# lxa9867/ControlVAR

Hardware: AMD Instinct MI355X
Metric: images/sec (256^2 autoregressive_infer_cfg, d24) (higher is better)
Workload: dtype bf16; 1 GPU; ControlVAR d24 autoregressive_infer_cfg 256^2 (control+image), CFG=4.0, top_k=900, top_p=0.96, incl. 2 VQVAE decodes; synthetic weights/labels; batch_per_gpu=512, global_batch=512, seq_len=1360, parallelism=dp1 (sample-sharded, no collective)

## Files before the change

### controlvar_amd/_lib.py

```python
from __future__ import annotations

import ctypes as C
import os
import threading

HERE = os.path.dirname(os.path.abspath(__file__))
LIB_PATH = os.environ.get('CVAR_LIB') or os.path.join(HERE, 'libcvar_hip.so')
ABI_VERSION = 21

CVAR_F32, CVAR_BF16 = 0, 1
ACT_NONE, ACT_GELU_TANH, ACT_GELU_GRAD = 0, 1, 2

c_p = C.c_void_p
c_i = C.c_int
c_l = C.c_int64
c_f = C.c_float


class GemmDesc(C.Structure):
    _fields_ = [
        ('M', c_i), ('N', c_i), ('K', c_i), ('dtype', c_i),
        ('A', c_p), ('lda', c_l), ('W', c_p), ('ldw', c_l),
        ('batch', c_i),
        ('strideA', c_l), ('strideW', c_l), ('strideC', c_l), ('strideR', c_l),
        ('conv', c_i), ('Hin', c_i), ('Win', c_i), ('Cin', c_i), ('Hout', c_i), ('Wout', c_i), ('stride', c_i), ('up', c_i),
        ('alpha', c_f), ('bias', c_p), ('act', c_i),
        ('gate', c_p), ('ldg', c_l), ('gate_rows', c_i),
        ('residual', c_p), ('res_dtype', c_i), ('ldr', c_l),
        ('C', c_p), ('out_dtype', c_i), ('ldc', c_l),
        ('remap_l', c_i), ('remap_L', c_i), ('remap_off', c_i),
        ('pre_act', c_p), ('aux', c_p), ('gate_scale', c_p),
        ('ws', c_p), ('ws_bytes', c_l), ('tile_cfg', c_i), ('stagger', c_i), ('group_m', c_i),
        ('C_split', c_p), ('split_n', c_i), ('ld_split', c_l), ('split_alpha', c_f),
        ('ln_out', c_p), ('ln_out_dtype', c_i), ('ln_scale', c_p), ('ln_shift', c_p), ('ld_ln', c_l), ('ln_rows', c_i), ('ln_eps', c_f),
        ('gn_part', c_p),
    ]


SIGNATURES = {
    'cvar_abi_version': (c_i, []),
    'cvar_status_str': (C.c_char_p, [c_i]),
    'cvar_gemm': (c_i, [C.POINTER(GemmDesc), c_p]),
    'cvar_resample_u8': (c_i, [c_p, c_i, c_i, c_i, c_i, c_i, c_p, c_p, c_i, c_p, c_p]),
    'cvar_crop_flip_normalize': (c_i, [c_p, c_i, c_i, c_i, c_i, c_i, c_i, c_i, c_i, c_p, c_p]),
    'cvar_sumsq_multi': (c_i, [c_p, c_i, c_p, c_p]),
    'cvar_adamw_multi': (c_i, [c_p, c_i, C.POINTER(c_f), C.POINTER(c_f), c_i, c_f, c_f, c_f, c_i, c_p, c_f, c_p]),
    'cvar_rle_paint': (c_i, [c_p, c_p, c_p, c_i, c_i, c_i, c_p, c_p]),
    'cvar_ignore_mask': (c_i, [c_p, c_i, c_i, c_i, C.POINTER(c_i), c_i, c_i, c_i, c_p, c_i, c_p]),
    'cvar_ln_modulate': (c_i, [c_p, c_p, c_p, c_l, c_i, c_p, c_i, c_i, c_i, c_f, c_p]),
    'cvar_silu_cast': (c_i, [c_p, c_p, c_i, c_l, c_p]),
    'cvar_attention': (c_i, [c_p, c_p, c_i, c_i, c_i, c_i, c_i, c_i, c_f, C.POINTER(c_i), c_i, C.POINTER(c_i), c_p, c_p, c_p]),
    'cvar_attention_rowwise': (c_i, [c_p, c_p, c_i, c_i, c_i, c_i, c_i, c_i, c_f, C.POINTER(c_i), c_i, C.POINTER(c_i), c_p, c_p, c_p]),
    'cvar_attention_v1': (c_i, [c_p, c_p, c_i, c_i, c_i, c_i, c_i, c_i, c_f, C.POINTER(c_i), c_i, C.POINTER(c_i), c_p, c_p, c_p]),
    'cvar_attention_prescaled': (c_i, [c_p, c_p, c_i, c_i, c_i, c_i, c_i, c_i, C.POINTER(c_i), c_i, C.POINTER(c_i), c_p, c_p, c_p]),
    'cvar_attention_bwd': (c_i, [c_p, c_i, c_p, c_p, c_p, c_i, c_i, c_i, c_i, c_i, c_f, C.POINTER(c_i), c_i, C.POINTER(c_i), c_p, c_p, c_p]),
    'cvar_attention_bwd_rowwise': (c_i, [c_p, c_i, c_p, c_p, c_p, c_i, c_i, c_i, c_i, c_i, c_f, C.POINTER(c_i), c_i, C.POINTER(c_i), c_p, c_p, c_p]),
    'cvar_cos_qk_norm': (c_i, [c_p, c_p, c_i, c_i, c_i, c_i, c_i, c_i, c_p, c_p, c_f, c_p]),
    'cvar_cos_qk_norm_bwd': (c_i, [c_p, c_p, c_i, c_i, c_i, c_i, c_i, c_p, c_p, c_p, c_p]),
    'cvar_cfg_sample': (c_i, [c_p, c_i, c_i, c_i, c_i, C.POINTER(c_f), c_i, c_f, C.c_uint64, c_p, c_i, c_i, c_p, c_p, c_p, c_p, c_i, c_p, c_i, c_f, c_f, c_p, c_p, c_p]),
    'cvar_ms_next_input': (c_i, [c_p, c_p, c_p, c_p, c_p, c_p, c_p, c_p, c_i, c_i, c_i, c_i, c_i, c_i, c_p]),
    'cvar_ms_encode': (c_i, [c_p, c_p, c_i, c_p, c_p, C.POINTER(c_i), C.POINTER(c_i), c_i, c_p, c_p, c_p, c_p, c_p, c_i, c_i, c_i, c_p]),
    'cvar_word_embed': (c_i, [c_p, c_p, c_p, c_p, c_p, c_i, c_i, c_i, c_i, c_i, c_i, c_i, c_p]),
    'cvar_first_tokens': (c_i, [c_p, c_p, c_p, c_p, c_p, c_p, c_p, c_p, c_i, c_i, c_i, c_i, c_p]),
    'cvar_groupnorm_ws_bytes': (c_l, [c_i, c_i, c_i]),
    'cvar_groupnorm_silu': (c_i, [c_p, c_i, c_p, c_p, c_p, c_i, c_i, c_i, c_i, c_f, c_i, c_p, c_p]),
    'cvar_groupnorm_silu_partials': (c_i, [c_p, c_i, c_p, c_p, c_p, c_i, c_i, c_i, c_i, c_f, c_i, c_p, c_i, c_i, c_p, c_p]),
    'cvar_split3': (c_i, [c_p, c_l, c_p, c_l, c_i, c_i, c_p]),
    'cvar_groupnorm_silu_split3': (c_i, [c_p, c_p, c_p, c_p, c_i, c_i, c_i, c_i, c_f, c_i, c_p, c_p]),
    'cvar_conv3x3_gn_partials': (c_i, [c_i, c_i, c_i, c_i, c_i, c_i, c_i, c_i, C.POINTER(c_i), C.POINTER(c_i)]),
    'cvar_softmax_rows': (c_i, [c_p, c_p, c_i, c_i, c_i, c_p]),
    'cvar_gemm_tn': (c_i, [c_p, c_l, c_p, c_l, c_p, c_l, c_i, c_i, c_i, c_p, c_l, c_p, c_p]),
    'cvar_embed_rows': (c_i, [c_p, c_p, c_i, c_p, c_l, c_i, c_p]),
    'cvar_resample_sep': (c_i, [c_p, c_p, c_p, c_p, c_i, c_i, c_i, c_i, c_i, c_i, c_p]),
    'cvar_transpose': (c_i, [c_p, c_p, c_i, c_i, c_i, c_i, c_l, c_l, c_p]),
    'cvar_nchw_to_nhwc': (c_i, [c_p, c_p, c_i, c_i, c_i, c_i, c_i, c_p]),
    'cvar_nhwc_to_nchw': (c_i, [c_p, c_i, c_l, c_p, c_i, c_i, c_i, c_f, c_f, c_f, c_f, c_p]),
    'cvar_gate_residual': (c_i, [c_p, c_p, c_i, c_p, c_l, c_i, c_p, c_l, c_i, c_p]),
    'cvar_train_ws_floats': (c_l, [c_l, c_i, c_i]),
    'cvar_gated_grad': (c_i, [c_p, c_p, c_i, c_p, c_l, c_p, c_p, c_p, c_l, c_i, c_i, c_i, c_p, c_l, c_p]),
    'cvar_gelu': (c_i, [c_p, c_p, c_i, c_l, c_p]),
    'cvar_gelu_bwd': (c_i, [c_p, c_p, c_i, c_l, c_p]),
    'cvar_ln_modulate_bwd': (c_i, [c_p, c_p, c_i, c_p, c_l, c_i, c_p, c_p, c_p, c_p, c_l, c_i, c_i, c_f, c_p, c_l, c_p]),
    'cvar_colsum': (c_i, [c_p, c_i, c_l, c_p, c_l, c_i, c_i, c_p, c_p]),
    'cvar_wordembed_grad_ws_bytes': (c_l, [c_l, c_i]),
    'cvar_wordembed_grad': (c_i, [c_p, c_l, c_i, c_i, c_p, c_i, c_i, c_i, c_i, c_p, c_p, c_p, c_p]),
    'cvar_rowsum': (c_i, [c_p, c_i, c_l, c_p, c_i, c_i, c_i, c_p]),
    'cvar_ce_fwd_bwd': (c_i, [c_p, c_p, c_p, c_f, c_p, c_p, c_i, c_l, c_i, c_p]),
    'cvar_scatter_add_rows': (c_i, [c_p, c_l, c_p, c_p, c_i, c_i, c_p]),
    'cvar_silu_bwd': (c_i, [c_p, c_p, c_p, c_l, c_p]),
    'cvar_adamw': (c_i, [c_p, c_p, c_p, c_p, c_l, c_f, c_f, c_f, c_f, c_f, c_i, c_p, c_f, c_p]),
    'cvar_sumsq': (c_i, [c_p, c_l, c_p, c_p]),
    'cvar_clip_coef': (c_i, [c_p, c_l, c_f, c_f, c_p, c_p]),
    'cvar_lora_down': (c_i, [c_p, c_l, c_p, c_l, c_p, c_l, c_p, c_l, c_i, c_i, c_i, c_i, c_f, c_f, C.c_uint64, C.c_uint32, c_p]),
    'cvar_lora_dx': (c_i, [c_p, c_l, c_i, c_p, c_l, c_p, c_l, c_p, c_l, c_i, c_i, c_i, c_i, c_f, c_f, C.c_uint64, C.c_uint32, c_p]),
    'cvar_lora_wgrad_ws_floats': (c_l, [c_i, c_i]),
    'cvar_lora_wgrad': (c_i, [c_p, c_l, c_p, c_l, c_i, c_i, c_i, c_i, c_f, c_f, C.c_uint64, C.c_uint32, c_p, c_l, c_p, c_l, c_l, c_p]),
    'cvar_lora_dropout_mask': (c_i, [c_p, c_i, c_i, c_f, C.c_uint64, C.c_uint32, c_p]),
    'cvar_probe_mfma_bf16': (c_i, [c_p, c_l, c_i, c_p, c_p]),
    'cvar_probe_mfma_bf16_32x32': (c_i, [c_p, c_l, c_i, c_p, c_p]),
    'cvar_probe_mfma_flops': (C.c_double, [c_i]),
}

_lib = None
_lock = threading.Lock()


class CvarError(RuntimeError):
    pass


def load(path: str = LIB_PATH) -> C.CDLL:
    global _lib
    with _lock:
        if _lib is not None:
            return _lib
        if not os.path.exists(path):
            raise CvarError(f'{path} not found - build it with `python -m controlvar_amd.build` (hipcc, gfx950); '
                            'there is no fallback path')
        try:
            import torch
        except Exception:
            pass
        lib = C.CDLL(path, mode=C.RTLD_GLOBAL)
        for name, (res, args) in SIGNATURES.items():
            fn = getattr(lib, name)
            fn.restype = res
            fn.argtypes = args
        v = lib.cvar_abi_version()
        if v != ABI_VERSION:
            raise CvarError(f'libcvar_hip.so ABI {v} != expected {ABI_VERSION}; rebuild')
        _lib = lib
        return lib


def check(status: int, what: str):
    if status != 0:
        msg = load().cvar_status_str(status).decode()
        raise CvarError(f'{what}: {msg} ({status})')
```

### controlvar_amd/csrc/conv_halo.hip

```cpp
#include "cvar_common.h"

typedef __attribute__((address_space(3))) void* lptr_t;

#ifndef CH_EPI_LDS
#define CH_EPI_LDS 1
#endif

struct ConvHaloParams {
    const bf16_t* X; const bf16_t* Wt; const float* bias; const bf16_t* res; void* out;
    int B, H, W, Cin, Cout, tiles_x, tiles_y, nchunk;
    int up, Hin, Win;
    float* gn_part;
};


template <int CH_NB, typename TO, int TW = 16>
__global__ __launch_bounds__(TW * 16, 2) void conv3x3_halo_bf16_kernel(const ConvHaloParams p) {
    constexpr int NW = TW / 4;
    constexpr int CH_HROW = TW + 4;
    constexpr int CH_HALO_PIECES = (18 * CH_HROW * 64 + 1023) / 1024;
    constexpr int CH_HALO_BYTES = CH_HALO_PIECES * 1024;
    constexpr int H_PER_WAVE = (CH_HALO_PIECES + NW - 1) / NW;
    constexpr int CH_W_BYTES = CH_NB * 2048;
    constexpr int W_PIECES = CH_NB * 2;
    constexpr int W_PER_WAVE = (W_PIECES + NW - 1) / NW;
    __shared__ __attribute__((aligned(1024))) char smem[2 * CH_HALO_BYTES + 3 * CH_W_BYTES];
    const int tid = threadIdx.x, lane = tid & 63;
    const int wave = __builtin_amdgcn_readfirstlane(tid >> 6);
    const int lrow = lane & 31, hi = lane >> 5;
    int t_ = blockIdx.x;
    const int tx = t_ % p.tiles_x; t_ /= p.tiles_x;
    const int ty = t_ % p.tiles_y;
    const int b = t_ / p.tiles_y;
    const int ty0 = ty * 16, tx0 = tx * TW;
    const int cout0 = blockIdx.y * (32 * CH_NB);
    const bf16_t* ximg = p.X + (long)b * p.Hin * p.Win * p.Cin;
    const __amdgpu_buffer_rsrc_t x_rsrc = __builtin_amdgcn_make_buffer_rsrc((void*)ximg, 0, p.Hin * p.Win * p.Cin * 2, 0x00020000);
    const __amdgpu_buffer_rsrc_t w_rsrc = __builtin_amdgcn_make_buffer_rsrc((void*)(p.Wt + (long)cout0 * 9 * p.Cin), 0, min(32 * CH_NB, p.Cout - cout0) * 9 * p.Cin * 2, 0x00020000);

    unsigned h_off[H_PER_WAVE], w_off[W_PER_WAVE];
#pragma unroll
    for (int jj = 0; jj < H_PER_WAVE; ++jj) {
        const int q = (wave + NW * jj) * 64 + lane;
        const int hp = q >> 2;
        const int hy = hp / CH_HROW, hx = hp - hy * CH_HROW;
        const int lc = (q & 3) ^ ((hx >> 2) & 3);
        const int gy = ty0 - 1 + hy, gx = tx0 - 1 + hx;
        const bool ok = hy < 18 && hx < TW + 2 && gy >= 0 && gy < p.H && gx >= 0 && gx < p.W;
        const int sy = p.up ? gy >> 1 : gy, sx = p.up ? gx >> 1 : gx;
        h_off[jj] = ok ? (unsigned)(((sy * p.Win + sx) * p.Cin + lc * 8) * 2) : 0x80000000u;
    }
#pragma unroll
    for (int jj = 0; jj < W_PER_WAVE; ++jj) {
        const int q = (wave + NW * jj) * 64 + lane;
        const int n = q >> 2, lc = (q & 3) ^ ((n >> 2) & 3);
        w_off[jj] = (n < 32 * CH_NB && cout0 + n < p.Cout) ? (unsigned)((n * 9 * p.Cin + lc * 8) * 2) : 0x80000000u;
    }
    auto issue_halo = [&](int c, int jj) -> int {
        const int j = wave + NW * jj;
        if (j >= CH_HALO_PIECES) return 0;
        __builtin_amdgcn_raw_ptr_buffer_load_lds(x_rsrc, (lptr_t)(smem + (c & 1) * CH_HALO_BYTES + j * 1024), 16, (int)h_off[jj], c * 64, 0, 0);
        return 1;
    };
    auto issue_w = [&](int c, int t) -> int {
        int n = 0;
#pragma unroll
        for (int jj = 0; jj < W_PER_WAVE; ++jj) {
            const int j = wave + NW * jj;
            if (j < W_PIECES) {
                __builtin_amdgcn_raw_ptr_buffer_load_lds(w_rsrc, (lptr_t)(smem + 2 * CH_HALO_BYTES + (t % 3) * CH_W_BYTES + j * 1024), 16,
                                                         (int)w_off[jj], (t * p.Cin + c * 32) * 2, 0, 0);
                ++n;
            }
        }
        return n;
    };
    auto wait_vm = [&](int n) {
        if (n >= 4) asm volatile("s_waitcnt vmcnt(4)" ::: "memory");
        else if (n == 3) asm volatile("s_waitcnt vmcnt(3)" ::: "memory");
        else if (n == 2) asm volatile("s_waitcnt vmcnt(2)" ::: "memory");
        else if (n == 1) asm volatile("s_waitcnt vmcnt(1)" ::: "memory");
        else asm volatile("s_waitcnt vmcnt(0)" ::: "memory");
    };

    constexpr int RPI = 32 / TW;
    const int px = lrow & (TW - 1), py0 = 2 * RPI * wave + lrow / TW;
    const int hpb = py0 * CH_HROW + px;
    const int swb = (lrow >> 2) & 3;
    const int b_lane = lrow * 64;

    f32x16_t acc[2][CH_NB];
#pragma unroll
    for (int i = 0; i < 2; ++i)
#pragma unroll
        for (int j = 0; j < CH_NB; ++j)
#pragma unroll
            for (int r = 0; r < 16; ++r) acc[i][j][r] = 0.f;

#pragma unroll
    for (int jj = 0; jj < H_PER_WAVE; ++jj) issue_halo(0, jj);
    issue_w(0, 0);
    issue_w(0, 1);
    asm volatile("s_waitcnt vmcnt(0)" ::: "memory");
    __builtin_amdgcn_s_barrier();

    bf16x8_t af[2][2][2];
    auto read_a = [&](int set, const char* hbuf, int d) {
        const int sw = ((px + d % CH_HROW) >> 2) & 3;
#pragma unroll
        for (int i = 0; i < 2; ++i) {
            const int hp = hpb + RPI * CH_HROW * i + d;
            const char* ap = hbuf + hp * 64;
#pragma unroll
            for (int ks = 0; ks < 2; ++ks) af[set][i][ks] = *(const bf16x8_t*)(ap + (((2 * ks + hi) ^ sw) << 4));
        }
    };
    read_a(0, smem, 0);
    for (int c = 0; c < p.nchunk; ++c) {
        const char* hb = smem + (c & 1) * CH_HALO_BYTES;
        const char* hb_next = smem + ((c + 1) & 1) * CH_HALO_BYTES;
#pragma unroll
        for (int t = 0; t < 9; ++t) {
            int issued = 0;
            if (t < H_PER_WAVE && c + 1 < p.nchunk) issued += issue_halo(c + 1, t);
            {
                const int c2 = t + 2 >= 9 ? c + 1 : c, t2 = t + 2 >= 9 ? t + 2 - 9 : t + 2;
                if (c2 < p.nchunk) issued += issue_w(c2, t2);
            }
            const char* wb = smem + 2 * CH_HALO_BYTES + (t % 3) * CH_W_BYTES + b_lane;
            bf16x8_t w[2][CH_NB];
#pragma unroll
            for (int ks = 0; ks < 2; ++ks)
#pragma unroll
                for (int j = 0; j < CH_NB; ++j) w[ks][j] = *(const bf16x8_t*)(wb + j * 2048 + (((2 * ks + hi) ^ swb) << 4));
            if (t < 8) read_a((t + 1) & 1, hb, ((t + 1) / 3) * CH_HROW + ((t + 1) % 3));
            else read_a(1, hb_next, 0);
#pragma unroll
            for (int ks = 0; ks < 2; ++ks)
#pragma unroll
                for (int j = 0; j < CH_NB; ++j)
#pragma unroll
                    for (int i = 0; i < 2; ++i) acc[i][j] = __builtin_amdgcn_mfma_f32_32x32x16_bf16(w[ks][j], af[t & 1][i][ks], acc[i][j], 0, 0, 0);
            wait_vm(issued);
            __builtin_amdgcn_s_barrier();
        }
#pragma unroll
        for (int i = 0; i < 2; ++i)
#pragma unroll
            for (int ks = 0; ks < 2; ++ks) af[0][i][ks] = af[1][i][ks];
    }

    float gs[8], gq[8], gpiv[8];
#pragma unroll
    for (int i = 0; i < 2; ++i) {
        const int yy = py0 + RPI * i, xx = px;
        const long gpix = ((long)b * p.H + ty0 + yy) * p.W + tx0 + xx;
        if constexpr (CH_NB == 1) {
            TO* op = (TO*)p.out + gpix * p.Cout + cout0;
#pragma unroll
            for (int g = 0; g < 4; ++g)
#pragma unroll
                for (int e = 0; e < 4; ++e) {
                    const int co = 8 * g + 4 * hi + e;
                    if (cout0 + co < p.Cout) {
                        const float v = acc[i][0][4 * g + e] + (p.bias ? p.bias[cout0 + co] : 0.f);
                        if constexpr (sizeof(TO) == 4) op[co] = v;
                        else op[co] = f32_to_bf16(v);
                    }
                }
        } else if constexpr (CH_NB == 5 && sizeof(TO) == 4) {
            float* op = (float*)p.out + gpix * p.Cout + cout0 + 4 * hi;
            const float* rp = p.res ? (const float*)p.res + gpix * p.Cout + cout0 + 4 * hi : nullptr;
            const float* bp = p.bias ? p.bias + cout0 + 4 * hi : nullptr;
#pragma unroll
            for (int j = 0; j < CH_NB; ++j) {
                f32x4_t rq[4];
                if (rp) {
#pragma unroll
                    for (int g = 0; g < 4; ++g) rq[g] = *(const f32x4_t*)(rp + 32 * j + 8 * g);
                }
#pragma unroll
                for (int g = 0; g < 4; ++g) {
                    const int co = 32 * j + 8 * g;
                    f32x4_t bq = {0.f, 0.f, 0.f, 0.f};
                    if (bp) bq = *(const f32x4_t*)(bp + co);
                    f32x4_t v;
#pragma unroll
                    for (int e = 0; e < 4; ++e) v[e] = acc[i][j][4 * g + e] + bq[e];
                    if (rp) {
#pragma unroll
                        for (int e = 0; e < 4; ++e) v[e] += rq[g][e];
                    }
                    *(f32x4_t*)(op + co) = v;
                }
            }
        } else if constexpr (CH_EPI_LDS != 0 && CH_NB == 5) {
            constexpr int PS = 336;
            constexpr int SLICE = (2 * CH_HALO_BYTES + 3 * CH_W_BYTES) / NW / 64 * 64;
            static_assert(32 * PS + 512 + 3 * 20 * 64 <= SLICE, "GroupNorm partials need the slack behind the staged rows");
            char* stg = smem + wave * SLICE;
            const float* bp = p.bias ? p.bias + cout0 + 4 * hi : nullptr;
            const long img = (long)b * p.H * p.W * p.Cout;
            auto chunk = [&](int k, int& go, int& lo) {
                const int q = k * 64 + lane, pq = q / 20, part = q - pq * 20;
                go = ((ty0 + 2 * RPI * wave + RPI * i + pq / TW) * p.W + tx0 + (pq & (TW - 1))) * p.Cout + cout0 + part * 8;
                lo = pq * PS + part * 16;
            };
            if (p.res) {
                const bf16_t* rimg = p.res + img;
#pragma unroll
                for (int h = 0; h < 2; ++h) {
                    bf16x8_t rr[5];
                    int lo[5];
#pragma unroll
                    for (int k = 0; k < 5; ++k) { int go; chunk(5 * h + k, go, lo[k]); rr[k] = *(const bf16x8_t*)(rimg + go); }
#pragma unroll
                    for (int k = 0; k < 5; ++k) *(bf16x8_t*)(stg + lo[k]) = rr[k];
                }
            }
            char* mine = stg + lrow * PS + 8 * hi;
#pragma unroll
            for (int j = 0; j < CH_NB; ++j)
#pragma unroll
                for (int g = 0; g < 4; ++g) {
                    const int co = 32 * j + 8 * g;
                    f32x4_t bq = {0.f, 0.f, 0.f, 0.f};
                    if (bp) bq = *(const f32x4_t*)(bp + co);
                    float v[4];
#pragma unroll
                    for (int e = 0; e < 4; ++e) v[e] = acc[i][j][4 * g + e] + bq[e];
                    if (p.res) {
                        const bf16x4_t rq = *(const bf16x4_t*)(mine + co * 2);
#pragma unroll
                        for (int e = 0; e < 4; ++e) v[e] += bf16_to_f32((bf16_t)rq[e]);
                    }
                    *(bf16x4_t*)(mine + co * 2) = pack_bf16x4(v);
                }
#pragma unroll
            for (int k = 0; k < 10; ++k) { int go, lo; chunk(k, go, lo); *(bf16x8_t*)((bf16_t*)p.out + img + go) = *(const bf16x8_t*)(stg + lo); }
            if (p.gn_part) {
                char* pv = smem + 32 * PS;
                if (i == 0) {
                    __builtin_amdgcn_wave_barrier();
                    if (wave == 0 && lane < 20) *(bf16x8_t*)(pv + lane * 16) = *(const bf16x8_t*)(stg + lane * 16);
                    __syncthreads();
                    if (lane < 60) {
                        const bf16x8_t pq8 = *(const bf16x8_t*)(pv + (lane % 20) * 16);
#pragma unroll
                        for (int e = 0; e < 8; ++e) { gpiv[e] = bf16_to_f32((bf16_t)pq8[e]); gs[e] = 0.f; gq[e] = 0.f; }
                    }
                }
                if (lane < 60) {
                    const int cc = lane % 20, pg = lane / 20;
#pragma unroll
                    for (int it = 0; it < 11; ++it) {
                        const int pp = pg + 3 * it;
                        if (pp < 32) {
                            const bf16x8_t y8 = *(const bf16x8_t*)(stg + pp * PS + cc * 16);
#pragma unroll
                            for (int e = 0; e < 8; ++e) { const float f = bf16_to_f32((bf16_t)y8[e]) - gpiv[e]; gs[e] += f; gq[e] = __builtin_fmaf(f, f, gq[e]); }
                        }
                    }
                }
                __builtin_amdgcn_wave_barrier();
            }
        } else {
            bf16_t* op = (bf16_t*)p.out + gpix * p.Cout + cout0 + 4 * hi;
            const bf16_t* rp = p.res ? p.res + gpix * p.Cout + cout0 + 4 * hi : nullptr;
            const float* bp = p.bias ? p.bias + cout0 + 4 * hi : nullptr;
            bf16x4_t rq[CH_NB][4];
            if (rp) {
#pragma unroll
                for (int j = 0; j < CH_NB; ++j)
#pragma unroll
                    for (int g = 0; g < 4; ++g) rq[j][g] = *(const bf16x4_t*)(rp + 32 * j + 8 * g);
            }
#pragma unroll
            for (int j = 0; j < CH_NB; ++j)
#pragma unroll
                for (int g = 0; g < 4; ++g) {
                    const int co = 32 * j + 8 * g;
                    f32x4_t bq = {0.f, 0.f, 0.f, 0.f};
                    if (bp) bq = *(const f32x4_t*)(bp + co);
                    float v[4];
#pragma unroll
                    for (int e = 0; e < 4; ++e) v[e] = acc[i][j][4 * g + e] + bq[e];
                    if (rp) {
#pragma unroll
                        for (int e = 0; e < 4; ++e) v[e] += bf16_to_f32((bf16_t)rq[j][g][e]);
                    }
                    *(bf16x4_t*)(op + co) = pack_bf16x4(v);
                }
        }
    }
    if constexpr (CH_NB == 5 && CH_EPI_LDS != 0 && sizeof(TO) == 2) {
        if (p.gn_part) {
            constexpr int PS = 336, SLICE = (2 * CH_HALO_BYTES + 3 * CH_W_BYTES) / NW / 64 * 64, RED = 32 * PS + 512;
            if (lane < 60) {
                float* rd = (float*)(smem + wave * SLICE + RED) + lane * 16;
#pragma unroll
                for (int e = 0; e < 8; e += 4) {
                    *(f32x4_t*)(rd + e) = f32x4_t{gs[e], gs[e + 1], gs[e + 2], gs[e + 3]};
                    *(f32x4_t*)(rd + 8 + e) = f32x4_t{gq[e], gq[e + 1], gq[e + 2], gq[e + 3]};
                }
            }
            __syncthreads();
            if (tid < 160) {
                const int cc = tid >> 3, e = tid & 7;
                float S = 0.f, Q = 0.f;
#pragma unroll
                for (int w = 0; w < NW; ++w)
#pragma unroll
                    for (int pg = 0; pg < 3; ++pg) {
                        const float* rd = (const float*)(smem + w * SLICE + RED) + (pg * 20 + cc) * 16;
                        S += rd[e]; Q += rd[8 + e];
                    }
                const float piv = bf16_to_f32(*(const bf16_t*)(smem + 32 * PS + tid * 2));
                float* gp = p.gn_part + ((((long)b * p.tiles_y + ty) * p.tiles_x + tx) * p.Cout + cout0 + tid) * 3;
                gp[0] = S; gp[1] = Q; gp[2] = piv;
            }
        }
    }
}

int cvar_conv3x3_halo_bf16(const void* X, const void* Wt, const float* bias, const void* residual, void* out, int out_f32, int B, int H, int W, int Cin,
                           int Cout, int up, float* gn_part, hipStream_t st) {
    ConvHaloParams p;
    p.X = (const bf16_t*)X; p.Wt = (const bf16_t*)Wt; p.bias = bias; p.res = (const bf16_t*)residual; p.out = out;
    p.B = B; p.H = H; p.W = W; p.Cin = Cin; p.Cout = Cout; p.tiles_x = W / 16; p.tiles_y = H / 16; p.nchunk = Cin / 32;
    p.up = up ? 1 : 0; p.Hin = up ? H / 2 : H; p.Win = up ? W / 2 : W;
    p.gn_part = gn_part;
    if (gn_part && !(Cout % 160 == 0 && !out_f32)) return CVAR_EUNSUPPORTED;
    const long tiles = (long)B * p.tiles_x * p.tiles_y;
    if (tiles <= 0 || tiles > 0x7fffffffL) return CVAR_EINVAL;
    if (Cout % 160 == 0 && out_f32) {
        if ((((uintptr_t)out | (uintptr_t)residual) & 15) != 0 || (long)H * W * Cout >= 0x7fffffffL) return CVAR_EUNSUPPORTED;
        hipLaunchKernelGGL((conv3x3_halo_bf16_kernel<5, float>), dim3((unsigned)tiles, Cout / 160), dim3(256), 0, st, p);
    } else if (Cout % 160 == 0 && !out_f32) {
        if ((((uintptr_t)out | (uintptr_t)residual) & 15) != 0 || (long)H * W * Cout >= 0x7fffffffL) return CVAR_EUNSUPPORTED;
        hipLaunchKernelGGL((conv3x3_halo_bf16_kernel<5, bf16_t>), dim3((unsigned)tiles, Cout / 160), dim3(256), 0, st, p);
    } else if (Cout <= 32 && !residual) {
        if (out_f32) hipLaunchKernelGGL((conv3x3_halo_bf16_kernel<1, float>), dim3((unsigned)tiles, 1), dim3(256), 0, st, p);
        else hipLaunchKernelGGL((conv3x3_halo_bf16_kernel<1, bf16_t>), dim3((unsigned)tiles, 1), dim3(256), 0, st, p);
    } else {
        return CVAR_EUNSUPPORTED;
    }
    CVAR_CHECK_LAUNCH();
    return CVAR_OK;
}
```

### controlvar_amd/csrc/cvar_common.h

```cpp
#pragma once
#include <hip/hip_runtime.h>
#include <stdint.h>
#include "../../include/cvar.h"

typedef __attribute__((ext_vector_type(8))) short bf16x8_t;
typedef __attribute__((ext_vector_type(4))) short bf16x4_t;
typedef __attribute__((ext_vector_type(4))) float f32x4_t;
typedef __attribute__((ext_vector_type(16))) float f32x16_t;
typedef unsigned short bf16_t;

#define CVAR_CHECK_LAUNCH()                                      \
    do {                                                         \
        hipError_t e__ = hipGetLastError();                      \
        if (e__ != hipSuccess) return CVAR_ELAUNCH;              \
    } while (0)

__device__ __forceinline__ float bf16_to_f32(bf16_t b) { return __uint_as_float(((unsigned)b) << 16); }

typedef __attribute__((ext_vector_type(2))) float f32x2_t;
typedef __attribute__((ext_vector_type(2))) __bf16 bf16x2n_t;
typedef __attribute__((ext_vector_type(4))) unsigned u32x4_t;
__device__ __forceinline__ bf16_t f32_to_bf16(float f) {
    const __bf16 b = (__bf16)f;
    return __builtin_bit_cast(unsigned short, b);
}
__device__ __forceinline__ unsigned pack_bf16x2(float lo, float hi) {
    const f32x2_t v = {lo, hi};
    const bf16x2n_t r = __builtin_convertvector(v, bf16x2n_t);
    return __builtin_bit_cast(unsigned, r);
}
__device__ __forceinline__ bf16x8_t pack_bf16x8(const float* v) {
    const u32x4_t u = {pack_bf16x2(v[0], v[1]), pack_bf16x2(v[2], v[3]), pack_bf16x2(v[4], v[5]), pack_bf16x2(v[6], v[7])};
    return __builtin_bit_cast(bf16x8_t, u);
}
__device__ __forceinline__ bf16x4_t pack_bf16x4(const float* v) {
    typedef __attribute__((ext_vector_type(2))) unsigned u32x2_t;
    const u32x2_t u = {pack_bf16x2(v[0], v[1]), pack_bf16x2(v[2], v[3])};
    return __builtin_bit_cast(bf16x4_t, u);
}

template <typename T> struct Elem;
template <> struct Elem<float> {
    static constexpr int kDtype = CVAR_F32;
    __device__ static __forceinline__ float ld(const float* p) { return *p; }
    __device__ static __forceinline__ void st(float* p, float v) { *p = v; }
};
template <> struct Elem<bf16_t> {
    static constexpr int kDtype = CVAR_BF16;
    __device__ static __forceinline__ float ld(const bf16_t* p) { return bf16_to_f32(*p); }
    __device__ static __forceinline__ void st(bf16_t* p, float v) { *p = f32_to_bf16(v); }
};

__device__ __forceinline__ float ld_any(const void* p, int dtype, int64_t i) {
    return dtype == CVAR_BF16 ? bf16_to_f32(((const bf16_t*)p)[i]) : ((const float*)p)[i];
}
__device__ __forceinline__ void st_any(void* p, int dtype, int64_t i, float v) {
    if (dtype == CVAR_BF16) ((bf16_t*)p)[i] = f32_to_bf16(v);
    else ((float*)p)[i] = v;
}

__device__ __forceinline__ float wave_sum(float v) {
#pragma unroll
    for (int o = 32; o > 0; o >>= 1) v += __shfl_xor(v, o, 64);
    return v;
}
__device__ __forceinline__ float wave_max(float v) {
#pragma unroll
    for (int o = 32; o > 0; o >>= 1) v = fmaxf(v, __shfl_xor(v, o, 64));
    return v;
}

__device__ __forceinline__ float gelu_tanh_f(float t) {
    const float k2 = 2.0f * 0.7978845608028654f;
    const float u2 = k2 * (t + 0.044715f * t * t * t);
    return t / (1.0f + __expf(-u2));
}

__device__ __forceinline__ float gelu_tanh_fast(float t) {
    const float c1 = -2.0f * 0.7978845608028654f * 1.4426950408889634f, c3 = c1 * 0.044715f;
    const float t2 = t * t;
    const float arg = t * (c1 + c3 * t2);
    return t * __builtin_amdgcn_rcpf(1.0f + __builtin_amdgcn_exp2f(arg));
}

__device__ __forceinline__ float gelu_tanh_grad(float t) {
    const float k2 = 2.0f * 0.7978845608028654f;
    const float u2 = k2 * (t + 0.044715f * t * t * t);
    const float sg = 1.0f / (1.0f + __expf(-u2));
    return sg + t * sg * (1.0f - sg) * k2 * (1.0f + 0.134145f * t * t);
}

static inline hipStream_t as_stream(void* s) { return (hipStream_t)s; }
static inline int cdiv(int64_t a, int64_t b) { return (int)((a + b - 1) / b); }

int cvar_conv3x3_halo_bf16(const void* X, const void* Wt, const float* bias, const void* residual, void* out, int out_f32, int B, int H, int W, int Cin,
                           int Cout, int up, float* gn_part, hipStream_t st);
int cvar_conv3x3_c8_bf16(const void* X, const void* Wt, const float* bias, void* out, int B, int H, int W, int Cout, float* gn_part, hipStream_t st);
```

### controlvar_amd/csrc/gemm.hip

```cpp
#include "cvar_common.h"
#include "gemm_params.h"
#if defined(CVAR_GEMM_CONV_TU)
#define CVAR_TU_CONV 1
#define CVAR_TU_PLAIN 0
#elif defined(CVAR_GEMM_F32_TU)
#define CVAR_TU_CONV 1
#define CVAR_TU_PLAIN 1
#else
#define CVAR_TU_CONV 0
#define CVAR_TU_PLAIN 1
#endif
#include <type_traits>

static __device__ __attribute__((aligned(16))) unsigned int cvar_zero_chunk[4] = {0u, 0u, 0u, 0u};
#if defined(CVAR_GEMM_TIMING) && defined(CVAR_GEMM_F32_TU)
#undef CVAR_GEMM_TIMING
#endif
#ifdef CVAR_GEMM_TIMING
__device__ unsigned long long cvar_gemm_dbg[64 * 8 * 8];
__device__ unsigned long long cvar_gemm_dbg_tot[8];
#define CVAR_DBG_WG_MAX 16384
__device__ unsigned long long cvar_gemm_dbg_wg[CVAR_DBG_WG_MAX * 5];
extern "C" int cvar_gemm_dbg_wg_read(unsigned long long* host, int n) { return (int)hipMemcpyFromSymbol(host, HIP_SYMBOL(cvar_gemm_dbg_wg), sizeof(unsigned long long) * 5 * (size_t)(n < CVAR_DBG_WG_MAX ? n : CVAR_DBG_WG_MAX)); }
extern "C" int cvar_gemm_dbg_tot_read(unsigned long long* host, int reset) { int rc = (int)hipMemcpyFromSymbol(host, HIP_SYMBOL(cvar_gemm_dbg_tot), 64); if (reset) { unsigned long long z[8] = {0}; rc |= (int)hipMemcpyToSymbol(HIP_SYMBOL(cvar_gemm_dbg_tot), z, 64); } return rc; }
// ... 788 lines not shown
            if (!lane_on || rr >= 16 || m >= p.M) continue;
            float v[8];
            {
                const float* sg = stg;
                const f32x4_t a0 = *(const f32x4_t*)(sg + (rr + srow_half * half) * EROW + ecol);
                const f32x4_t a1 = *(const f32x4_t*)(sg + (rr + srow_half * half) * EROW + ecol + 4);
#pragma unroll
                for (int e = 0; e < 4; ++e) { v[e] = a0[e] * p.alpha; v[4 + e] = a1[e] * p.alpha; }
            }
            long orow = m;
            if (p.remap_l > 0) {
                const int sq = fast_div(m, p.remap_magic, p.remap_shift);
                orow = (long)sq * p.remap_L + p.remap_off + (m - sq * p.remap_l);
            }
            const float* grow = p.gate ? p.gate + (long)fast_div(m, p.gate_magic, p.gate_shift) * p.ldg : nullptr;
            void* Cdst = Cb;
            long cbase = cz + orow * p.ldc + n;
            bool scale_split = false;
            if (p.split_n > 0) {
                if (n < p.split_n) { Cdst = p.Cs; cbase = (long)m * p.ld_split + n; scale_split = p.split_alpha != 1.0f; }
                else cbase -= p.split_n;
            }
            if (vec_ok) {
#pragma unroll
                for (int e = 0; e < 8; ++e) v[e] += bias8[e];
                if (p.C2) {
#pragma unroll
                    for (int e = 0; e < 8; ++e) st_any(p.C2, ES == 2 ? CVAR_BF16 : CVAR_F32, cz + (long)m * p.ldc + n + e, v[e]);
                }
                if (scale_split) {
#pragma unroll
                    for (int e = 0; e < 8; ++e) v[e] *= p.split_alpha;
                }
                if (p.act == CVAR_ACT_GELU_TANH) {
#pragma unroll
                    for (int e = 0; e < 8; ++e) v[e] = (ES == 2) ? gelu_tanh_fast(v[e]) : gelu_tanh_f(v[e]);
                } else if (p.act == CVAR_ACT_GELU_GRAD) {
#pragma unroll
                    for (int e = 0; e < 8; ++e) v[e] *= gelu_tanh_grad(ld_any(p.aux, p.out_dtype, cz + (long)m * p.ldc + n + e));
                }
                if (grow) {
                    const f32x4_t g0 = *(const f32x4_t*)(grow + n), g1 = *(const f32x4_t*)(grow + n + 4);
                    const float gs = p.gate_scale ? p.gate_scale[fast_div(m, p.gate_magic, p.gate_shift)] : 1.0f;
#pragma unroll
                    for (int e = 0; e < 4; ++e) { v[e] *= g0[e] * gs; v[4 + e] *= g1[e] * gs; }
                }
                if (p.residual) {
                    if (p.res_dtype == CVAR_BF16) {
                        const bf16x8_t rv = *(const bf16x8_t*)((const bf16_t*)p.residual + rz + (long)m * p.ldr + n);
#pragma unroll
                        for (int e = 0; e < 8; ++e) v[e] += bf16_to_f32((bf16_t)rv[e]);
                    } else {
                        const float* rp = (const float*)p.residual + rz + (long)m * p.ldr + n;
                        const f32x4_t r0 = *(const f32x4_t*)rp, r1 = *(const f32x4_t*)(rp + 4);
#pragma unroll
                        for (int e = 0; e < 4; ++e) { v[e] += r0[e]; v[4 + e] += r1[e]; }
                    }
                }
                if (p.out_dtype == CVAR_BF16) {
                    *(bf16x8_t*)((bf16_t*)Cdst + cbase) = pack_bf16x8(v);
                } else {
                    float* cp = (float*)Cdst + cbase;
                    const f32x4_t o0 = {v[0], v[1], v[2], v[3]}, o1 = {v[4], v[5], v[6], v[7]};
                    *(f32x4_t*)cp = o0; *(f32x4_t*)(cp + 4) = o1;
                }
            } else {
                for (int e = 0; e < 8; ++e) {
                    if (n + e >= p.N) break;
                    float x = v[e];
                    if (p.bias) x += p.bias[n + e];
                    if (p.C2) st_any(p.C2, ES == 2 ? CVAR_BF16 : CVAR_F32, cz + (long)m * p.ldc + n + e, x);
                    if (p.act == CVAR_ACT_GELU_TANH) x = gelu_tanh_f(x);
                    else if (p.act == CVAR_ACT_GELU_GRAD) x *= gelu_tanh_grad(ld_any(p.aux, p.out_dtype, cz + (long)m * p.ldc + n + e));
                    if (grow) x *= grow[n + e] * (p.gate_scale ? p.gate_scale[fast_div(m, p.gate_magic, p.gate_shift)] : 1.0f);
                    if (p.residual) x += ld_any(p.residual, p.res_dtype, rz + (long)m * p.ldr + n + e);
                    st_any(Cdst, p.out_dtype, cbase + e, x);
                }
            }
        }
    }
    }
#ifdef CVAR_GEMM_TIMING
    if (lane == 0 && wave == 0 && (int)blockIdx.x < CVAR_DBG_WG_MAX && blockIdx.y == 0 && blockIdx.z == 0) {
        asm volatile("s_waitcnt vmcnt(0)" ::: "memory");
        unsigned hwid, xcc;
        asm volatile("s_getreg_b32 %0, hwreg(HW_REG_HW_ID)" : "=s"(hwid));
        asm volatile("s_getreg_b32 %0, hwreg(HW_REG_XCC_ID)" : "=s"(xcc));
        unsigned long long* o = cvar_gemm_dbg_wg + (size_t)blockIdx.x * 5;
        o[0] = dbg_rt_entry; o[1] = dbg_rt_loop; o[2] = dbg_rt_loop_end; o[3] = __builtin_amdgcn_s_memrealtime(); o[4] = (unsigned long long)hwid | ((unsigned long long)xcc << 32);
    }
    if (lane == 0 && blockIdx.x < 64) {
        const unsigned long long dbg_t2 = __builtin_amdgcn_s_memtime();
        unsigned long long* o = cvar_gemm_dbg + (blockIdx.x * 8 + wave) * 8;
        o[0] = dbg_comp; o[1] = dbg_vm; o[2] = dbg_bar; o[3] = dbg_t1 - dbg_t0; o[4] = dbg_t2 - dbg_t1; o[5] = nk - kt_lo; o[6] = dbg_t0; o[7] = dbg_t2;
    }
    if (lane == 0 && wave == 0) {
        const unsigned long long dbg_t2 = __builtin_amdgcn_s_memtime();
        atomicAdd(&cvar_gemm_dbg_tot[0], dbg_t1 - dbg_t0); atomicAdd(&cvar_gemm_dbg_tot[1], dbg_t2 - dbg_t1); atomicAdd(&cvar_gemm_dbg_tot[2], 1ULL);
        atomicAdd(&cvar_gemm_dbg_tot[6], dbg_ew); atomicAdd(&cvar_gemm_dbg_tot[3], dbg_vm); atomicAdd(&cvar_gemm_dbg_tot[4], dbg_bar); atomicAdd(&cvar_gemm_dbg_tot[5], dbg_comp);
    }
#endif
}

template <typename T, int BM, int BN, int WM, int WN, bool CONV, int NSTAGE = 2, bool FAST = false, bool CUP = false>
__global__ __launch_bounds__(WM * WN * 64) void cvar_gemm_kernel(const GemmParams p) {
    cvar_gemm_tile<T, BM, BN, WM, WN, CONV, NSTAGE, FAST, CUP>(p, (int)blockIdx.x);
}

__device__ __forceinline__ void splitk_finish_quad(const GemmParams& p, const float* __restrict__ part, int nsplit, int m, int n) {
    f32x4_t v;
    const float* const q0 = part + (long)m * p.N + n;
    const long sstride = (long)p.M * p.N;
    {
        v = *(const f32x4_t*)q0;
        for (int s0 = 1; s0 < nsplit; s0 += 8) {
            f32x4_t w[8];
#pragma unroll
            for (int u = 0; u < 8; ++u)
                if (s0 + u < nsplit) w[u] = *(const f32x4_t*)(q0 + (long)(s0 + u) * sstride);
#pragma unroll
            for (int u = 0; u < 8; ++u)
                if (s0 + u < nsplit) {
#pragma unroll
                    for (int e = 0; e < 4; ++e) v[e] += w[u][e];
                }
        }
    }
    gemm_epilogue_quad(p, m, n, v);
}

template <typename K>
static void set_max_lds_once(K kfn, size_t lds, unsigned char* done) {
    int dev = 0;
    (void)hipGetDevice(&dev);
    if (dev < 0 || dev >= 64 || !done[dev]) {
        (void)hipFuncSetAttribute((const void*)kfn, hipFuncAttributeMaxDynamicSharedMemorySize, (int)lds);
        if (dev >= 0 && dev < 64) done[dev] = 1;
    }
}

template <typename T, int BM, int BN, int WM, int WN, int NSTAGE = 2, bool CONVFAST = false, bool CUP = false>
static int launch_cfg(const GemmParams& gp, int batch, hipStream_t st) {
    GemmParams p = gp;
    p.tiles_m = (p.M + BM - 1) / BM;
    p.tiles_n = (p.N + BN - 1) / BN;
    if (p.group_m <= 0) p.group_m = (!p.conv && ((long)p.K * (long)sizeof(T) >= 8192 || p.out_dtype == CVAR_F32)) ? 4 : 8;
    if (p.conv) { const int kt_e = 128 / (int)sizeof(T); p.cv_adv = kt_e / p.Cin; p.cv_rem = kt_e % p.Cin; }
    const size_t lds = NSTAGE * (BM + BN) * 128 + ((sizeof(T) == 2 && BM == 256 && BN == 256 && WM == 2 && WN == 4 && NSTAGE == 2 && !CONVFAST) ? 32768 : 0);
    const int nk_all = (p.K + (128 / (int)sizeof(T)) - 1) / (128 / (int)sizeof(T));
    const int splits = p.split_tiles > 0 ? (nk_all + p.split_tiles - 1) / p.split_tiles : 1;
    const bool plain_fast = !p.conv && p.K % (128 / (int)sizeof(T)) == 0 && (long)(BM - 1) * p.lda * (long)sizeof(T) + (long)p.K * (long)sizeof(T) < (1L << 31) &&
                            (long)(BN - 1) * p.ldw * (long)sizeof(T) + (long)p.K * (long)sizeof(T) < (1L << 31);
    dim3 grid((unsigned)(p.tiles_m * p.tiles_n), (unsigned)splits, (unsigned)batch), block(WM * WN * 64);
    constexpr bool WITH_CONV = CVAR_TU_CONV || sizeof(T) == 4, WITH_PLAIN = CVAR_TU_PLAIN || sizeof(T) == 4;
    if constexpr (CONVFAST) {
        if (!p.conv) return CVAR_EINVAL;
        if constexpr (WITH_CONV) {
            auto kfn = cvar_gemm_kernel<T, BM, BN, WM, WN, true, NSTAGE, true, CUP>;
            static unsigned char lds_set[64] = {0};
            set_max_lds_once(kfn, lds, lds_set);
            hipLaunchKernelGGL(kfn, grid, block, lds, st, p);
            CVAR_CHECK_LAUNCH();
            return CVAR_OK;
        } else return CVAR_EUNSUPPORTED;
    } else if (p.conv) {
        if constexpr (WITH_CONV) {
            auto kfn = cvar_gemm_kernel<T, BM, BN, WM, WN, true, NSTAGE>;
            static unsigned char lds_set[64] = {0};
            set_max_lds_once(kfn, lds, lds_set);
            hipLaunchKernelGGL(kfn, grid, block, lds, st, p);
        } else return CVAR_EUNSUPPORTED;
    } else if constexpr (!WITH_PLAIN) {
        return CVAR_EUNSUPPORTED;
    } else if (plain_fast) {
        auto kfn = cvar_gemm_kernel<T, BM, BN, WM, WN, false, NSTAGE, true>;
        static unsigned char lds_set[64] = {0};
        set_max_lds_once(kfn, lds, lds_set);
        hipLaunchKernelGGL(kfn, grid, block, lds, st, p);
    } else {
        auto kfn = cvar_gemm_kernel<T, BM, BN, WM, WN, false, NSTAGE>;
        static unsigned char lds_set[64] = {0};
        set_max_lds_once(kfn, lds, lds_set);
        hipLaunchKernelGGL(kfn, grid, block, lds, st, p);
    }
    CVAR_CHECK_LAUNCH();
    return CVAR_OK;
}

static int gemm_cfg_override(const GemmParams& p) {
    return p.tile_cfg == 1 ? 0 : (p.tile_cfg == 2 || p.tile_cfg == 7 || p.tile_cfg == 28) ? 1 : (p.tile_cfg == 3 || p.tile_cfg == 8) ? 3 : p.tile_cfg == 4 ? 4 : -1;
}

template <typename T>
static int launch_typed(const GemmParams& p, int batch, hipStream_t st) {
    if (p.M <= 64) return launch_cfg<T, 64, 128, 1, 4>(p, batch, st);
    auto launch_128 = [&](const GemmParams& q, int nb, hipStream_t s) -> int {
#if CVAR_TU_PLAIN && !CVAR_TU_CONV
        if constexpr (sizeof(T) == 2) {
            if (CVAR_GEMM_128_W8 && !q.conv && q.tile_cfg != 26) return launch_cfg<T, 128, 128, 2, 4>(q, nb, s);
        }
#endif
        return launch_cfg<T, 128, 128, 2, 2>(q, nb, s);
    };
    if constexpr (sizeof(T) == 2) {
        if (p.conv && p.N <= 32 && p.M >= 4096 && p.stride == 1 && !p.up && p.Cin % 32 == 0 && p.split_tiles == 0 && gemm_cfg_override(p) != 0) {
            const long in_bytes = (long)(p.M / (p.Hout * p.Wout)) * p.Hin * p.Win * p.Cin * (long)sizeof(T);
            if (in_bytes < (1L << 31)) {
                GemmParams q = p;
                q.conv_bytes = (unsigned)in_bytes;
                return launch_cfg<T, 256, 32, 4, 1, 2, true>(q, batch, st);
            }
        }
    }
    if (p.N % 160 == 0 && (p.N % 128 != 0 || p.conv) && p.M >= 4096) {
        const long in_bytes = p.conv ? (long)(p.M / (p.Hout * p.Wout)) * p.Hin * p.Win * p.Cin * (long)sizeof(T) : 0;
        if constexpr (sizeof(T) == 2) {
            if (p.conv && (p.stride == 1 || (p.stride == 2 && !p.up)) && p.Cin % 32 == 0 && p.split_tiles == 0 && in_bytes < (1L << 31) &&
                (long)159 * p.ldw * 2 + (long)p.K * 2 + 256 < (1L << 31) && gemm_cfg_override(p) != 0 &&
                (!p.up || (p.Hout == 2 * p.Hin && p.Wout == 2 * p.Win))) {
                GemmParams q = p;
                q.conv_bytes = (unsigned)in_bytes;
                const int ovc = gemm_cfg_override(p);
                if (!p.up && p.stride == 1 && ovc != 3 && (ovc == 4 || (long)p.K * (long)sizeof(T) <= 4096)) return launch_cfg<T, 256, 160, 8, 1, 2, true>(q, batch, st);
                return p.up ? launch_cfg<T, 256, 160, 4, 1, 2, true, true>(q, batch, st) : launch_cfg<T, 256, 160, 4, 1, 2, true>(q, batch, st);
            }
        }
        return launch_cfg<T, 128, 160, 4, 1>(p, batch, st);
    }
#if CVAR_TU_PLAIN && !CVAR_TU_CONV
    if constexpr (sizeof(T) == 2) {
        if (p.tile_cfg == 27 && !p.conv && p.split_tiles == 0) return launch_cfg<T, 256, 192, 4, 2>(p, batch, st);
    }
#endif
    const int ov = gemm_cfg_override(p);
    const bool n_ok = p.N % 256 == 0 || (p.N % 128 == 0 && p.N >= 1536);
    if (sizeof(T) == 2 && (ov == 3 || (ov != 0 && ov != 1 && p.split_tiles > 0)) && (p.M >= 2048 || (p.split_tiles > 0 && p.M > 1024)) && n_ok)
        return launch_cfg<T, 256, 256, 2, 2>(p, batch, st);
    if (ov == -1 && sizeof(T) == 2 && p.split_tiles == 0 && batch == 1 && n_ok && p.M >= 2048) {
        const long t256 = (long)((p.M + 255) / 256) * ((p.N + 255) / 256), t128 = (long)((p.M + 127) / 128) * ((p.N + 127) / 128);
        const double c256 = (double)((t256 + 255) / 256), c128 = CVAR_GEMM_C128 * (double)((t128 + 511) / 512);
#if CVAR_TU_PLAIN && !CVAR_TU_CONV
        if constexpr (sizeof(T) == 2) {
            if (CVAR_GEMM_T192 && !p.conv && p.N % 192 == 0) {
                const long t192 = (long)((p.M + 255) / 256) * (p.N / 192);
                const double c192 = CVAR_GEMM_C192 * (double)((t192 + 255) / 256);
                if (c192 < 0.95 * c256 && c192 < c128) return launch_cfg<T, 256, 192, 4, 2>(p, batch, st);
            }
        }
#endif
        if (c128 < 0.97 * c256) {
#if CVAR_TU_PLAIN && !CVAR_TU_CONV
            if constexpr (sizeof(T) == 2) {
                if (p.tile_cfg == 12 && !p.conv && t128 <= 256 && p.K >= 6 * 64) return launch_cfg<T, 128, 128, 2, 4, 3>(p, batch, st);
            }
#endif
            return launch_128(p, batch, st);
        }
    }
    if (ov != 0 && (p.M >= 2048 || (p.split_tiles > 0 && p.M > 1024)) && n_ok) return launch_cfg<T, 256, 256, 2, 4>(p, batch, st);
#if CVAR_TU_PLAIN && !CVAR_TU_CONV
    if constexpr (sizeof(T) == 2) {
        if (p.tile_cfg == 13 && !p.conv) return launch_cfg<T, 128, 128, 2, 4, 3>(p, batch, st);
        if (p.tile_cfg == 14 && !p.conv) return launch_cfg<T, 128, 128, 2, 2, 4>(p, batch, st);
        if (p.tile_cfg == 12 && !p.conv && batch == 1 && p.split_tiles == 0 && p.K >= 6 * 64 &&
            (long)((p.M + 127) / 128) * ((p.N + 127) / 128) <= 256) return launch_cfg<T, 128, 128, 2, 4, 3>(p, batch, st);
    }
#endif
    return launch_128(p, batch, st);
}

int cvar_gemm_skinny_plan(int M, int N, int K, long lda, long ldw, int want_rowfin, int have_ws, int* mt, int* nt, int* slices);
int cvar_gemm_skinny_launch(const GemmParams& p, int mt, int nt, int slices, hipStream_t st);
int cvar_splitk_rowfin_ok(const GemmParams& p, const cvar_gemm_desc* d);
int cvar_splitk_rowfin_launch(const float* part, int nsplit, const GemmParams& p, const cvar_gemm_desc* d, hipStream_t st);
int cvar_gemm_launch_f32(const GemmParams& p, int batch, hipStream_t st);
int cvar_gemm_launch_conv_bf16(const GemmParams& p, int batch, hipStream_t st);
#if defined(CVAR_GEMM_F32_TU)
int cvar_gemm_launch_f32(const GemmParams& p, int batch, hipStream_t st) { return launch_typed<float>(p, batch, st); }
#elif defined(CVAR_GEMM_CONV_TU)
int cvar_gemm_launch_conv_bf16(const GemmParams& p, int batch, hipStream_t st) { return launch_typed<bf16_t>(p, batch, st); }
#else

__global__ __launch_bounds__(256) void cvar_splitk_epilogue_kernel(const float* __restrict__ part, int nsplit, const GemmParams p) {
    const long nvec = (long)p.M * (p.N / 4);
    for (long i = (long)blockIdx.x * 256 + threadIdx.x; i < nvec; i += (long)gridDim.x * 256)
        splitk_finish_quad(p, part, nsplit, (int)(i / (p.N / 4)), (int)(i % (p.N / 4)) * 4);
}


extern "C" int cvar_conv3x3_gn_partials(int dtype, int stride, int Cin, int Cout, int Hin, int Win, int Hout, int Wout, int* tiles_per_image, int* pixels_per_tile) {
#ifndef CVAR_NO_CONV_C8
    const bool c8 = Cin == 8 && Hin == Hout && Win == Wout;
#else
    const bool c8 = false;
#endif
    const bool ok = dtype == CVAR_BF16 && stride == 1 && Cin > 0 && (Cin % 32 == 0 || c8) && Cout > 0 && Cout % 160 == 0 && Hout > 0 && Wout > 0 && Hout % 16 == 0 && Wout % 16 == 0 &&
                    (long)Hin * Win * Cin * 2 < 0x7fffffffL && (long)Hout * Wout * Cout < 0x7fffffffL;
    if (!ok) return 0;
    if (tiles_per_image) *tiles_per_image = (Hout / 16) * (Wout / 16);
    if (pixels_per_tile) *pixels_per_tile = 256;
    return 1;
}

extern "C" int cvar_gemm(const cvar_gemm_desc* d, void* stream) {
    if (!d || !d->A || !d->W || !d->C) return CVAR_EINVAL;
    if (d->M <= 0 || d->N <= 0 || d->K <= 0 || d->batch < 1) return CVAR_EINVAL;
    if (d->dtype != CVAR_F32 && d->dtype != CVAR_BF16) return CVAR_EUNSUPPORTED;
    const int es = d->dtype == CVAR_BF16 ? 2 : 4, kch = 16 / es;
    if (d->K % kch) return CVAR_EUNSUPPORTED;
    if (((uintptr_t)d->A & 15) || ((uintptr_t)d->W & 15)) return CVAR_EINVAL;
    if ((d->ldw % kch) || (d->strideW % kch) || (d->strideA % kch)) return CVAR_EUNSUPPORTED;
    if (d->conv) {
        if (d->Cin % kch || d->K != 9 * d->Cin) return CVAR_EUNSUPPORTED;
        if (d->stride != 1 && d->stride != 2) return CVAR_EUNSUPPORTED;
        if (d->stride == 2 && d->up) return CVAR_EUNSUPPORTED;
        if (d->stride == 1 && (d->Hout != (d->up ? 2 : 1) * d->Hin || d->Wout != (d->up ? 2 : 1) * d->Win)) return CVAR_EINVAL;
        if (d->stride == 2 && (d->Hout != d->Hin / 2 || d->Wout != d->Win / 2)) return CVAR_EINVAL;
        if (d->M % (d->Hout * d->Wout)) return CVAR_EINVAL;
    } else if (d->lda % kch) {
        return CVAR_EUNSUPPORTED;
    }
    if (d->gn_part && !d->conv) return CVAR_EINVAL;
    if (d->gate && d->gate_rows <= 0) return CVAR_EINVAL;
    if (d->act == CVAR_ACT_GELU_GRAD && !d->aux) return CVAR_EINVAL;
    if (d->pre_act && d->act == CVAR_ACT_GELU_GRAD) return CVAR_EINVAL;
    if (d->gate_scale && !d->gate) return CVAR_EINVAL;
    if ((d->pre_act || d->aux) && d->remap_l > 0) return CVAR_EUNSUPPORTED;
    if (d->split_n < 0 || d->split_n >= d->N) return CVAR_EINVAL;
    if (d->split_n > 0) {
        if (!d->C_split || d->ld_split < d->split_n) return CVAR_EINVAL;
        if (d->remap_l <= 0 || d->conv || d->batch != 1 || d->residual || d->gate || d->act != CVAR_ACT_NONE) return CVAR_EUNSUPPORTED;
        if ((d->split_n & 7) || (d->N & 7) || (d->ld_split & 7) || (d->ldc & 7) || ((uintptr_t)d->C_split & 15) || ((uintptr_t)d->C & 15)) return CVAR_EUNSUPPORTED;
    }
    GemmParams p;
    p.M = d->M; p.N = d->N; p.K = d->K;
    p.A = (const char*)d->A; p.lda = d->lda; p.W = (const char*)d->W; p.ldw = d->ldw;
    p.strideA = d->strideA; p.strideW = d->strideW; p.strideC = d->strideC; p.strideR = d->strideR;
    p.conv = d->conv; p.Hin = d->Hin; p.Win = d->Win; p.Cin = d->Cin; p.Hout = d->Hout; p.Wout = d->Wout;
    p.stride = d->stride; p.up = d->up;
    p.alpha = d->alpha; p.bias = d->bias; p.act = d->act;
    p.gate = d->gate; p.ldg = d->ldg; p.gate_rows = d->gate_rows;
    p.residual = d->residual; p.res_dtype = d->res_dtype; p.ldr = d->ldr;
    p.C = d->C; p.out_dtype = d->out_dtype; p.ldc = d->ldc;
    p.C2 = d->pre_act; p.aux = d->aux; p.gate_scale = d->gate_scale; p.in_dtype = d->dtype;
    p.remap_l = d->remap_l; p.remap_L = d->remap_L; p.remap_off = d->remap_off;
    p.Cs = d->C_split; p.split_n = d->split_n; p.ld_split = d->ld_split; p.split_alpha = d->split_alpha == 0.0f ? 1.0f : d->split_alpha;
    p.tiles_m = p.tiles_n = 0;
    p.cv_adv = p.cv_rem = 0; p.conv_bytes = 0;
    make_fast_div(p.remap_l, &p.remap_magic, &p.remap_shift);
    make_fast_div(p.gate ? p.gate_rows : 1, &p.gate_magic, &p.gate_shift);
    p.split_tiles = 0; p.split_stride = 0;
    p.tile_cfg = d->tile_cfg; p.stagger = d->stagger > 0 ? d->stagger : 0; p.group_m = d->group_m > 0 ? d->group_m : 0;
    p.nt = ((long)d->M * d->N * (d->out_dtype == CVAR_F32 ? 4 : 2) >= (128L << 20)) ? 1 : 0;
    float* const g_splitk_ws = (d->ws && d->ws_bytes > 0 && (((uintptr_t)d->ws & 15) == 0)) ? (float*)d->ws : nullptr;
    const size_t g_splitk_ws_bytes = g_splitk_ws ? (size_t)d->ws_bytes : 0;
    hipStream_t st = as_stream(stream);
    if (d->ln_out) {
        if (!d->ln_scale || !d->ln_shift || d->ln_rows <= 0 || (d->N % 4) || d->N > 2048 || (d->ld_ln % 4) || d->out_dtype != CVAR_F32 || d->ldc != d->N ||
            d->remap_l > 0 || d->split_n > 0 || d->conv || d->batch != 1 || (d->ln_out_dtype != CVAR_BF16 && d->ln_out_dtype != CVAR_F32)) return CVAR_EUNSUPPORTED;
    }
    auto ln_after = [&](int rc) -> int {
        if (rc != CVAR_OK || !d->ln_out) return rc;
        return cvar_ln_modulate((const float*)d->C, d->ln_scale, d->ln_shift, d->ld_ln, d->ln_rows, d->ln_out, d->ln_out_dtype, d->M, d->N, d->ln_eps, stream);
    };
    const bool rowfin = g_splitk_ws && cvar_splitk_rowfin_ok(p, d);
    auto finish_slices = [&](int splits) -> int {
        if (rowfin) return cvar_splitk_rowfin_launch(g_splitk_ws, splits, p, d, st);
        const long nvec = (long)d->M * (d->N / 4);
        hipLaunchKernelGGL(cvar_splitk_epilogue_kernel, dim3((unsigned)min((long)2048, (nvec + 255) / 256)), dim3(256), 0, st, g_splitk_ws, splits, p);
        CVAR_CHECK_LAUNCH();
        return ln_after(CVAR_OK);
    };
    if (!d->conv && d->batch == 1 && d->dtype == CVAR_BF16 && d->tile_cfg == 12 && !d->pre_act && !d->aux) {
        int mt = 0, nt = 0, sl = 0;
        if (cvar_gemm_skinny_plan(d->M, d->N, d->K, d->lda, d->ldw, rowfin ? 1 : 0, g_splitk_ws ? 1 : 0, &mt, &nt, &sl)) {
            if (sl > 1 && (size_t)sl * d->M * d->N * sizeof(float) <= g_splitk_ws_bytes) {
                GemmParams ps = p;
                ps.C = g_splitk_ws; ps.out_dtype = CVAR_F32; ps.ldc = d->N;
                ps.split_tiles = (d->K >> 5) / sl; ps.split_stride = (long)d->M * d->N;
                const int rc = cvar_gemm_skinny_launch(ps, mt, nt, sl, st);
                if (rc != CVAR_OK) return rc;
                return finish_slices(sl);
            }
            if (sl == 1) return ln_after(cvar_gemm_skinny_launch(p, mt, nt, 1, st));
        }
    }
    const int kt_elems = 128 / es;
    const int nk_all = (d->K + kt_elems - 1) / kt_elems;
    const int tm = d->M <= 64 ? (d->M + 63) / 64 : (d->M + 127) / 128, tn = (d->N + 127) / 128;
    int long_k_splits = 0;
    const int t256 = ((d->M + 255) / 256) * ((d->N + 255) / 256);
    if (!d->conv && d->batch == 1 && d->dtype == CVAR_BF16 && d->M > 1024 && d->M % 128 == 0 && d->N % 128 == 0 && d->N >= 1536 && g_splitk_ws &&
        (nk_all >= 128 || (nk_all >= 24 && t256 <= 64 && !d->remap_l))) {
        const int tiles = t256;
        if (tiles < 256) {
            double best = 1e30;
            for (int sp = 1; sp <= 8; ++sp) {
                const double cost = (double)((tiles * sp + 255) / 256) / sp + 0.01 * sp;
                if (nk_all / sp < 6) break;
                if (cost < best && (size_t)sp * d->M * d->N * sizeof(float) <= g_splitk_ws_bytes) { best = cost; long_k_splits = sp; }
            }
            if (long_k_splits < 2) long_k_splits = 0;
        }
    }
    const bool three = d->tile_cfg == 12 && !d->conv && d->batch == 1 && d->dtype == CVAR_BF16 && d->M > 64 && d->M <= 1024 && (d->N % 4) == 0 && tm * tn <= 256 &&
                       nk_all >= 6 && !d->pre_act && !d->aux;
    int three_splits = 1;
    if (three && g_splitk_ws) {
        three_splits = min(16, max(1, 256 / (tm * tn)));
        while (three_splits > 1 && nk_all / three_splits < 4) --three_splits;
    }
    if (three) p.tile_cfg = 13;
    if (long_k_splits || (three && three_splits > 1) ||
        (!three && !d->conv && d->batch == 1 && d->M <= 1024 && (d->N % 4) == 0 && tm * tn < 128 && nk_all >= 8 && g_splitk_ws)) {
        int splits = long_k_splits ? long_k_splits : three ? three_splits : min(16, max(2, 320 / (tm * tn)));
        int per = (nk_all + splits - 1) / splits;
        if (per < 2) per = 2;
        splits = (nk_all + per - 1) / per;
        const size_t need = (size_t)splits * d->M * d->N * sizeof(float);
        if (splits > 1 && need <= g_splitk_ws_bytes) {
            GemmParams ps = p;
            ps.alpha = 1.0f; ps.bias = nullptr; ps.act = CVAR_ACT_NONE; ps.gate = nullptr; ps.residual = nullptr; ps.C2 = nullptr; ps.aux = nullptr; ps.gate_scale = nullptr;
            ps.C = g_splitk_ws; ps.out_dtype = CVAR_F32; ps.ldc = d->N; ps.remap_l = 0; ps.split_n = 0; ps.Cs = nullptr; ps.strideC = 0;
            ps.split_tiles = per; ps.split_stride = (long)d->M * d->N;
            const int rc = d->dtype == CVAR_BF16 ? launch_typed<bf16_t>(ps, 1, st) : cvar_gemm_launch_f32(ps, 1, st);
            if (rc != CVAR_OK) return rc;
            return finish_slices(splits);
        }
    }
#ifndef CVAR_NO_CONV_C8
    if (d->conv && d->dtype == CVAR_BF16 && d->stride == 1 && !d->up && d->batch == 1 && (d->tile_cfg == 0 || d->tile_cfg == 6) && d->Cin == 8 && d->N % 160 == 0 &&
        d->Hout % 16 == 0 && d->Wout % 16 == 0 && d->act == CVAR_ACT_NONE && !d->gate && d->alpha == 1.0f && !d->residual && !d->pre_act && !d->aux && !d->gate_scale &&
        d->remap_l == 0 && d->split_n == 0 && d->strideC == 0 && d->ldc == d->N && d->ldw == d->K && d->out_dtype == CVAR_BF16 &&
        ((((uintptr_t)d->C | (uintptr_t)d->bias) & 15) == 0) && (long)d->Hout * d->Wout * d->N < 0x7fffffffL)
        return cvar_conv3x3_c8_bf16(d->A, d->W, d->bias, d->C, d->M / (d->Hout * d->Wout), d->Hout, d->Wout, d->N, d->gn_part, st);
#endif
    if (d->conv && d->dtype == CVAR_BF16 && d->stride == 1 && d->batch == 1 && (d->tile_cfg == 0 || d->tile_cfg == 6 || d->tile_cfg == 9 || d->tile_cfg == 10) &&
        d->Cin % 32 == 0 && d->Hout % 16 == 0 && d->Wout % 16 == 0 && d->act == CVAR_ACT_NONE && !d->gate && d->alpha == 1.0f &&
        !d->pre_act && !d->aux && !d->gate_scale && d->remap_l == 0 && d->split_n == 0 && d->strideC == 0 && d->ldc == d->N &&
        d->ldw == d->K &&
        (!d->bias || (((uintptr_t)d->bias & 15) == 0)) && (long)d->Hin * d->Win * d->Cin * 2 < 0x7fffffffL) {
        const bool wide = d->N % 160 == 0 && d->out_dtype == CVAR_BF16 && (((uintptr_t)d->C & 15) == 0) &&
                          (!d->residual || (d->res_dtype == CVAR_BF16 && d->ldr == d->N && (((uintptr_t)d->residual & 15) == 0))) &&
                          (long)d->Hout * d->Wout * d->N < 0x7fffffffL;
        const bool narrow = d->N <= 32 && !d->residual && (d->out_dtype == CVAR_BF16 || d->out_dtype == CVAR_F32) && ((long)d->Hout * d->Wout >= 65536 || d->tile_cfg == 6);
        if (d->gn_part && !wide) return CVAR_EUNSUPPORTED;
        const bool wide32 = d->N % 160 == 0 && d->out_dtype == CVAR_F32 && (((uintptr_t)d->C & 15) == 0) && !d->up &&
                            (!d->residual || (d->res_dtype == CVAR_F32 && d->ldr == d->N && (((uintptr_t)d->residual & 15) == 0))) &&
                            (long)d->Hout * d->Wout * d->N < 0x7fffffffL;
        if (wide || narrow || wide32)
            return cvar_conv3x3_halo_bf16(d->A, d->W, d->bias, d->residual, d->C, d->out_dtype == CVAR_F32, d->M / (d->Hout * d->Wout), d->Hout, d->Wout, d->Cin,
                                          d->N, d->up, d->gn_part, st);
    }
    if (d->gn_part) return CVAR_EUNSUPPORTED;
    if (d->dtype == CVAR_BF16) return d->conv ? cvar_gemm_launch_conv_bf16(p, d->batch, st) : ln_after(launch_typed<bf16_t>(p, d->batch, st));
    return ln_after(cvar_gemm_launch_f32(p, d->batch, st));
}
#endif
```

### controlvar_amd/csrc/ops.hip

```cpp
#include "cvar_common.h"

template <typename TO, int NV, bool TAIL>
__global__ __launch_bounds__(256) void ln_modulate_kernel(const float* __restrict__ x, const float* __restrict__ scale,
                                                         const float* __restrict__ shift, long ld_ada, int rows_per,
                                                         TO* __restrict__ out, int M, int C, float eps) {
    const int lane = threadIdx.x & 63;
    const int row = blockIdx.x * 4 + (threadIdx.x >> 6);
    if (row >= M) return;
    const float* xr = x + (long)row * C;
    const long g = row / rows_per;
    const float* sc = scale + g * ld_ada;
    const float* sh = shift + g * ld_ada;
    f32x4_t v[NV], a[NV], b[NV];
    const f32x4_t zero4 = {0.f, 0.f, 0.f, 0.f};
#pragma unroll
    for (int i = 0; i < NV; ++i) {
        const int c = (i * 64 + lane) * 4;
        const bool ok = !(TAIL && i == NV - 1) || c < C;
        v[i] = ok ? *(const f32x4_t*)(xr + c) : zero4;
        a[i] = ok ? *(const f32x4_t*)(sc + c) : zero4;
        b[i] = ok ? *(const f32x4_t*)(sh + c) : zero4;
    }
    float s = 0.f;
#pragma unroll
// ... 42 lines not shown
        case 1: ln_launch<TO, 1>(tail, grid, st, x, scale, shift, ld_ada, rows_per, out, M, C, eps); break;
        case 2: ln_launch<TO, 2>(tail, grid, st, x, scale, shift, ld_ada, rows_per, out, M, C, eps); break;
        case 3: ln_launch<TO, 3>(tail, grid, st, x, scale, shift, ld_ada, rows_per, out, M, C, eps); break;
        case 4: ln_launch<TO, 4>(tail, grid, st, x, scale, shift, ld_ada, rows_per, out, M, C, eps); break;
        case 5: ln_launch<TO, 5>(tail, grid, st, x, scale, shift, ld_ada, rows_per, out, M, C, eps); break;
        case 6: ln_launch<TO, 6>(tail, grid, st, x, scale, shift, ld_ada, rows_per, out, M, C, eps); break;
        case 7: ln_launch<TO, 7>(tail, grid, st, x, scale, shift, ld_ada, rows_per, out, M, C, eps); break;
        case 8: ln_launch<TO, 8>(tail, grid, st, x, scale, shift, ld_ada, rows_per, out, M, C, eps); break;
        default: return CVAR_EUNSUPPORTED;
    }
    CVAR_CHECK_LAUNCH();
    return CVAR_OK;
}

extern "C" int cvar_ln_modulate(const float* x, const float* scale, const float* shift, int64_t ld_ada, int rows_per,
                                void* out, int out_dtype, int M, int C, float eps, void* stream) {
    if (!x || !scale || !shift || !out || M <= 0 || rows_per <= 0) return CVAR_EINVAL;
    if (C % 4 || C > 2048 || ld_ada % 4) return CVAR_EUNSUPPORTED;
    if (out_dtype == CVAR_BF16) return ln_dispatch<bf16_t>(x, scale, shift, (long)ld_ada, rows_per, (bf16_t*)out, M, C, eps, as_stream(stream));
    if (out_dtype == CVAR_F32) return ln_dispatch<float>(x, scale, shift, (long)ld_ada, rows_per, (float*)out, M, C, eps, as_stream(stream));
    return CVAR_EUNSUPPORTED;
}

template <typename TO>
__global__ void silu_cast_kernel(const float* __restrict__ x, TO* __restrict__ out, long n) {
    long i = (long)blockIdx.x * blockDim.x + threadIdx.x;
    const long stride = (long)gridDim.x * blockDim.x;
    for (; i < n; i += stride) {
        const float v = x[i];
        Elem<TO>::st(out + i, v / (1.0f + __expf(-v)));
    }
}

extern "C" int cvar_silu_cast(const float* x, void* out, int out_dtype, int64_t n, void* stream) {
    if (!x || !out || n <= 0) return CVAR_EINVAL;
    dim3 grid((unsigned)min((int64_t)2048, (n + 255) / 256)), block(256);
    if (out_dtype == CVAR_BF16) hipLaunchKernelGGL(silu_cast_kernel<bf16_t>, grid, block, 0, as_stream(stream), x, (bf16_t*)out, (long)n);
    else if (out_dtype == CVAR_F32) hipLaunchKernelGGL(silu_cast_kernel<float>, grid, block, 0, as_stream(stream), x, (float*)out, (long)n);
    else return CVAR_EUNSUPPORTED;
    CVAR_CHECK_LAUNCH();
    return CVAR_OK;
}

template <typename T>
__global__ __launch_bounds__(256) void cos_qk_norm_kernel(T* __restrict__ qkv, T* __restrict__ qs, int R, int H, int Lmax, int q_off, int l,
                                                         const float* __restrict__ scale_mul, float* __restrict__ norms, float q_mul) {
    const int lane = threadIdx.x & 63;
    const long item = (long)blockIdx.x * 4 + (threadIdx.x >> 6);
    const long total = (long)R * l * H * 2;
    if (item >= total) return;
    const int which = (int)(item & 1);
    const int h = (int)((item >> 1) % H);
    const long rt = (item >> 1) / H;
    const int t = (int)(rt % l);
    const long r = rt / l;
    T* p;
    if (qs) p = (which == 0 ? qs + (r * l + t) * (long)(H * 64) : qkv + (r * Lmax + q_off + t) * 2 * (long)(H * 64)) + h * 64 + lane;
    else p = qkv + ((r * Lmax + q_off + t) * 3 + which) * (long)(H * 64) + h * 64 + lane;
    const float v = Elem<T>::ld(p);
    const float nrm = fmaxf(sqrtf(wave_sum(v * v)), 1e-12f);
    float o = v / nrm;
    if (which == 0) o *= __expf(fminf(scale_mul[h], 4.605170185988092f)) * q_mul;
    Elem<T>::st(p, o);
    if (norms && lane == 0) norms[item] = nrm;
}

extern "C" int cvar_cos_qk_norm(void* qkv, void* q, int dtype, int R, int H, int Lmax, int q_off, int l, const float* scale_mul,
                                float* norms, float q_mul, void* stream) {
    if (!qkv || !scale_mul || R <= 0 || H <= 0 || l <= 0) return CVAR_EINVAL;
    const long total = (long)R * l * H * 2;
    dim3 grid(cdiv(total, 4)), block(256);
    if (dtype == CVAR_BF16) hipLaunchKernelGGL(cos_qk_norm_kernel<bf16_t>, grid, block, 0, as_stream(stream), (bf16_t*)qkv, (bf16_t*)q, R, H, Lmax, q_off, l, scale_mul, norms, q_mul);
    else if (dtype == CVAR_F32) hipLaunchKernelGGL(cos_qk_norm_kernel<float>, grid, block, 0, as_stream(stream), (float*)qkv, (float*)q, R, H, Lmax, q_off, l, scale_mul, norms, q_mul);
    else return CVAR_EUNSUPPORTED;
    CVAR_CHECK_LAUNCH();
    return CVAR_OK;
}

template <typename T>
__global__ __launch_bounds__(256) void cos_qk_norm_bwd_kernel(const T* __restrict__ qkv, T* __restrict__ dqkv, int R, int H, int Lmax, int l,
                                                             const float* __restrict__ scale_mul, const float* __restrict__ norms,
                                                             float* __restrict__ dsm_tok ) {
    const int lane = threadIdx.x & 63;
    const long item = (long)blockIdx.x * 4 + (threadIdx.x >> 6);
    const long total = (long)R * l * H * 2;
    if (item >= total) return;
    const int which = (int)(item & 1);
    const int h = (int)((item >> 1) % H);
    const long rt = (item >> 1) / H;
    const int t = (int)(rt % l);
    const long r = rt / l;
    const long off = ((r * Lmax + t) * 3 + which) * (long)(H * 64) + h * 64 + lane;
    const float sm = __expf(fminf(scale_mul[h], 4.605170185988092f));
    const float xh = Elem<T>::ld(qkv + off);
    const float g = Elem<T>::ld(dqkv + off);
    const float nrm = norms[item];
    const float xt = which == 0 ? xh / sm : xh;
    const float gp = which == 0 ? g * sm : g;
    const float dot = wave_sum(xt * gp);
    Elem<T>::st(dqkv + off, (gp - xt * dot) / nrm);
    if (which == 0) {
        const float ds = wave_sum(g * xt);
        if (lane == 0) dsm_tok[rt * H + h] = scale_mul[h] < 4.605170185988092f ? ds * sm : 0.f;
    }
}

extern "C" int cvar_cos_qk_norm_bwd(const void* qkv, void* dqkv, int dtype, int R, int H, int Lmax, int l, const float* scale_mul,
                                    const float* norms, float* dsm_tok, void* stream) {
    if (!qkv || !dqkv || !scale_mul || !norms || !dsm_tok || R <= 0 || H <= 0 || l <= 0) return CVAR_EINVAL;
    const long total = (long)R * l * H * 2;
    dim3 grid(cdiv(total, 4)), block(256);
    if (dtype == CVAR_BF16) hipLaunchKernelGGL(cos_qk_norm_bwd_kernel<bf16_t>, grid, block, 0, as_stream(stream), (const bf16_t*)qkv, (bf16_t*)dqkv, R, H, Lmax, l, scale_mul, norms, dsm_tok);
    else if (dtype == CVAR_F32) hipLaunchKernelGGL(cos_qk_norm_bwd_kernel<float>, grid, block, 0, as_stream(stream), (const float*)qkv, (float*)dqkv, R, H, Lmax, l, scale_mul, norms, dsm_tok);
    else return CVAR_EUNSUPPORTED;
    CVAR_CHECK_LAUNCH();
    return CVAR_OK;
}

constexpr int WE_TOK = 64;
__global__ __launch_bounds__(256) void word_embed_kernel(const float* __restrict__ tok, const float* __restrict__ W,
                                                        const float* __restrict__ bias, const float* __restrict__ lvl_pos,
                                                        float* __restrict__ x, int nb, int nrep, int l, int Cvae, int C,
                                                        int x_rows, int x_off, int tpb) {
    __shared__ __attribute__((aligned(16))) float tk[WE_TOK * 64];
    const long ntok = (long)nb * l;
    const long bt0 = (long)blockIdx.x * tpb;
    const int nt = (int)min((long)tpb, ntok - bt0);
    for (int i = threadIdx.x; i < nt * Cvae; i += 256) tk[i] = tok[bt0 * Cvae + i];
    __syncthreads();
    const int c = blockIdx.y * 256 + threadIdx.x;
    if (c >= C) return;
    f32x4_t wv[16];
#pragma unroll
    for (int k4 = 0; k4 < 16; ++k4) {
        const f32x4_t z = {0.f, 0.f, 0.f, 0.f};
        wv[k4] = 4 * k4 < Cvae ? *(const f32x4_t*)(W + (long)c * Cvae + 4 * k4) : z;
    }
    const float bc = bias[c];
    for (int i = 0; i < nt; ++i) {
        const long bt = bt0 + i;
        const int t = (int)(bt % l);
        const long b = bt / l;
        const float* tv = tk + i * Cvae;
        float acc = 0.f;
#pragma unroll
        for (int k4 = 0; k4 < 16; ++k4) {
            if (4 * k4 < Cvae) {
                const f32x4_t q = *(const f32x4_t*)(tv + 4 * k4);
                acc = fmaf(q[0], wv[k4][0], acc); acc = fmaf(q[1], wv[k4][1], acc);
                acc = fmaf(q[2], wv[k4][2], acc); acc = fmaf(q[3], wv[k4][3], acc);
            }
        }
        const float v = (acc + bc) + lvl_pos[(long)t * C + c];
        for (int rep = 0; rep < nrep; ++rep) x[(((long)rep * nb + b) * x_rows + x_off + t) * C + c] = v;
    }
}

extern "C" int cvar_word_embed(const float* tok, const float* W, const float* bias, const float* lvl_pos, float* x,
                               int nb, int nrep, int l, int Cvae, int C, int x_rows, int x_off, void* stream) {
    if (!tok || !W || !bias || !lvl_pos || !x || nb <= 0 || nrep <= 0 || l <= 0) return CVAR_EINVAL;
    if (x_rows < x_off + l || x_off < 0) return CVAR_EINVAL;
    if (Cvae > 64 || Cvae % 4) return CVAR_EUNSUPPORTED;
    const long ntok = (long)nb * l;
    int tpb = WE_TOK;
    while (tpb > 4 && ((ntok + tpb - 1) / tpb) * cdiv(C, 256) < 512) tpb >>= 1;
    hipLaunchKernelGGL(word_embed_kernel, dim3((unsigned)((ntok + tpb - 1) / tpb), (unsigned)cdiv(C, 256)), dim3(256), 0, as_stream(stream), tok, W,
                       bias, lvl_pos, x, nb, nrep, l, Cvae, C, x_rows, x_off, tpb);
    CVAR_CHECK_LAUNCH();
    return CVAR_OK;
}

__global__ void first_tokens_kernel(const float* __restrict__ class_emb, const float* __restrict__ cond_embed,
                                    const int* __restrict__ labels, const int* __restrict__ types,
                                    const float* __restrict__ pos_start, const float* __restrict__ lvl_pos,
                                    float* __restrict__ x, float* __restrict__ cond, int R, int first_l, int C, int x_rows) {
    const int r = blockIdx.x;
    const float* ce = class_emb + (long)labels[r] * C;
    for (int c = threadIdx.x; c < C; c += blockDim.x) {
        const float cls = ce[c];
        cond[(long)r * C + c] = cls;
        if (first_l == 2) {
            const float ct = cond_embed[(long)types[r] * C + c];
            x[((long)r * x_rows + 0) * C + c] = (ct + pos_start[c]) + lvl_pos[c];
            x[((long)r * x_rows + 1) * C + c] = (cls + pos_start[C + c]) + lvl_pos[C + c];
        } else {
            x[(long)r * x_rows * C + c] = (cls + pos_start[c]) + lvl_pos[c];
        }
    }
}

extern "C" int cvar_first_tokens(const float* class_emb, const float* cond_embed, const int32_t* labels, const int32_t* types,
                                 const float* pos_start, const float* lvl_pos, float* x, float* cond, int R, int first_l,
                                 int C, int x_rows, void* stream) {
    if (!class_emb || !labels || !pos_start || !lvl_pos || !x || !cond || R <= 0) return CVAR_EINVAL;
    if (first_l != 1 && first_l != 2) return CVAR_EUNSUPPORTED;
    if (x_rows < first_l) return CVAR_EINVAL;
    if (first_l == 2 && (!cond_embed || !types)) return CVAR_EINVAL;
    hipLaunchKernelGGL(first_tokens_kernel, dim3(R), dim3(256), 0, as_stream(stream), class_emb, cond_embed, labels, types, pos_start, lvl_pos, x, cond, R, first_l, C, x_rows);
    CVAR_CHECK_LAUNCH();
    return CVAR_OK;
}

template <typename T>
__global__ __launch_bounds__(256) void gn_stats_kernel(const T* __restrict__ x, float* __restrict__ partial, int HW, int C, int pix_per_block) {
    constexpr int VEC = 16 / sizeof(T);
    extern __shared__ float sred[];
    const int b = blockIdx.y, chunk = blockIdx.x, nchunk = gridDim.x;
    const int ncg = C / VEC;
    const int PL = 256 / ncg;
    const int pl = threadIdx.x / ncg, cg = threadIdx.x % ncg;
    if (pl < PL) {
        float s[VEC], q[VEC];
#pragma unroll
        for (int e = 0; e < VEC; ++e) { s[e] = 0.f; q[e] = 0.f; }
        const int p0 = chunk * pix_per_block;
        const int p1 = min(p0 + pix_per_block, HW);
        float piv[VEC];
        {
            const T* src = x + (long)b * HW * C + cg * VEC;
            if constexpr (sizeof(T) == 2) {
                const bf16x8_t v = *(const bf16x8_t*)src;
#pragma unroll
                for (int e = 0; e < VEC; ++e) piv[e] = bf16_to_f32((bf16_t)v[e]);
            } else {
                const f32x4_t v = *(const f32x4_t*)src;
#pragma unroll
                for (int e = 0; e < VEC; ++e) piv[e] = v[e];
            }
        }
#pragma unroll 4
        for (int p = p0 + pl; p < p1; p += PL) {
            const T* src = x + ((long)b * HW + p) * C + cg * VEC;
            if constexpr (sizeof(T) == 2) {
                const bf16x8_t v = *(const bf16x8_t*)src;
#pragma unroll
                for (int e = 0; e < VEC; ++e) { const float f = bf16_to_f32((bf16_t)v[e]) - piv[e]; s[e] += f; q[e] += f * f; }
            } else {
                const f32x4_t v = *(const f32x4_t*)src;
#pragma unroll
                for (int e = 0; e < VEC; ++e) { const float f = v[e] - piv[e]; s[e] += f; q[e] += f * f; }
            }
        }
#pragma unroll
        for (int e = 0; e < VEC; ++e) {
            float2 sq; sq.x = s[e]; sq.y = q[e];
            *(float2*)(sred + ((long)(e * PL + pl) * ncg + cg) * 2) = sq;
        }
    }
    __syncthreads();
    for (int i = threadIdx.x; i < 2 * C; i += 256) {
        const int c = i >> 1, which = i & 1, cg2 = c / VEC, e = c % VEC;
        float a = 0.f;
        for (int k = 0; k < PL; ++k) a += sred[((long)(e * PL + k) * ncg + cg2) * 2 + which];
        partial[(((long)b * nchunk + chunk) * C) * 2 + i] = a;
    }
}

template <typename T>
__global__ __launch_bounds__(64) void gn_finalize_kernel(const float* __restrict__ partial, int nchunk, const T* __restrict__ x, const float* __restrict__ weight,
                                                        const float* __restrict__ bias, float* __restrict__ coef, int HW, int C, int groups, float eps) {
    const int b = blockIdx.y, g = blockIdx.x, lane = threadIdx.x;
    const int cpg = C / groups;
    double s = 0.0;
    const int items = cpg * nchunk;
    for (int it = lane; it < items; it += 64) {
        const int k = it / cpg, cc = g * cpg + it % cpg;
        s += (double)partial[(((long)b * nchunk + k) * C + cc) * 2];
    }
    for (int cc = g * cpg + lane; cc < (g + 1) * cpg; cc += 64) s += (double)HW * (double)Elem<T>::ld(x + (long)b * HW * C + cc);
#pragma unroll
    for (int o = 32; o > 0; o >>= 1) s += __shfl_xor(s, o, 64);
    const double n = (double)HW * cpg;
    const double mean = s / n;
    double q = 0.0;
    for (int it = lane; it < items; it += 64) {
        const int k = it / cpg, cc = g * cpg + it % cpg;
        const double d = (double)Elem<T>::ld(x + (long)b * HW * C + cc) - mean;
        q += (double)partial[(((long)b * nchunk + k) * C + cc) * 2 + 1] + 2.0 * d * (double)partial[(((long)b * nchunk + k) * C + cc) * 2];
    }
    for (int cc = g * cpg + lane; cc < (g + 1) * cpg; cc += 64) {
        const double d = (double)Elem<T>::ld(x + (long)b * HW * C + cc) - mean;
        q += (double)HW * d * d;
    }
#pragma unroll
    for (int o = 32; o > 0; o >>= 1) q += __shfl_xor(q, o, 64);
    double var = q / n;
    if (var < 0.0) var = 0.0;
    const float rstd = (float)(1.0 / sqrt(var + (double)eps));
    for (int cc = g * cpg + lane; cc < (g + 1) * cpg; cc += 64) {
        const float a = rstd * weight[cc];
        coef[((long)b * C + cc) * 2] = a;
        coef[((long)b * C + cc) * 2 + 1] = bias[cc] - (float)mean * a;
    }
}

template <typename T>
__global__ __launch_bounds__(256) void gn_apply_kernel(const T* __restrict__ x, const float* __restrict__ coef, T* __restrict__ out,
                                                      int HW, int C, int ppb, int silu) {
    constexpr int VEC = 16 / sizeof(T);
    const int ncg = C / VEC, PL = 256 / ncg;
    const int b = blockIdx.y, chunk = blockIdx.x;
    const int cg = threadIdx.x % ncg, pl = threadIdx.x / ncg;
    if (pl >= PL) return;
    float a[VEC], d[VEC];
    {
        const float* cf = coef + ((long)b * C + cg * VEC) * 2;
#pragma unroll
        for (int e = 0; e < VEC; ++e) { a[e] = cf[2 * e]; d[e] = cf[2 * e + 1]; }
    }
    const int p0 = chunk * ppb, p1 = min(HW, p0 + ppb);
    const long base = (long)b * HW * C + cg * VEC;
#pragma unroll 4
    for (int p = p0 + pl; p < p1; p += PL) {
        const long off = base + (long)p * C;
        float y[VEC];
        if constexpr (sizeof(T) == 2) {
            const bf16x8_t v = *(const bf16x8_t*)(x + off);
#pragma unroll
            for (int e = 0; e < VEC; ++e) y[e] = bf16_to_f32((bf16_t)v[e]) * a[e] + d[e];
        } else {
            const f32x4_t v = *(const f32x4_t*)(x + off);
#pragma unroll
            for (int e = 0; e < VEC; ++e) y[e] = v[e] * a[e] + d[e];
        }
        if (silu) {
#pragma unroll
            for (int e = 0; e < VEC; ++e) {
                if constexpr (sizeof(T) == 2) y[e] = y[e] * __builtin_amdgcn_rcpf(1.0f + __builtin_amdgcn_exp2f(-1.4426950408889634f * y[e]));
                else y[e] = y[e] / (1.0f + __expf(-y[e]));
            }
        }
        if constexpr (sizeof(T) == 2) {
            *(bf16x8_t*)(out + off) = pack_bf16x8(y);
        } else {
            f32x4_t o = {y[0], y[1], y[2], y[3]};
            *(f32x4_t*)(out + off) = o;
        }
    }
}

__global__ __launch_bounds__(64) void gn_finalize_tiles_kernel(const float* __restrict__ part, int ntile, int npix, const float* __restrict__ weight,
                                                              const float* __restrict__ bias, float* __restrict__ coef, int HW, int C, int groups, float eps) {
    const int b = blockIdx.y, g = blockIdx.x, lane = threadIdx.x;
    const int cpg = C / groups;
    const int items = cpg * ntile;
    const double n = (double)npix;
    double s = 0.0;
    for (int it = lane; it < items; it += 64) {
        const int k = it / cpg, cc = g * cpg + it % cpg;
        const float* q = part + (((long)b * ntile + k) * C + cc) * 3;
        s += n * (double)q[2] + (double)q[0];
    }
#pragma unroll
    for (int o = 32; o > 0; o >>= 1) s += __shfl_xor(s, o, 64);
    const double cnt = (double)HW * cpg;
    const double mean = s / cnt;
    double v = 0.0;
    for (int it = lane; it < items; it += 64) {
        const int k = it / cpg, cc = g * cpg + it % cpg;
        const float* q = part + (((long)b * ntile + k) * C + cc) * 3;
        const double d = (double)q[2] - mean;
        v += (double)q[1] + 2.0 * d * (double)q[0] + n * d * d;
    }
#pragma unroll
    for (int o = 32; o > 0; o >>= 1) v += __shfl_xor(v, o, 64);
    double var = v / cnt;
    if (var < 0.0) var = 0.0;
    const float rstd = (float)(1.0 / sqrt(var + (double)eps));
    for (int cc = g * cpg + lane; cc < (g + 1) * cpg; cc += 64) {
        const float a = rstd * weight[cc];
        coef[((long)b * C + cc) * 2] = a;
        coef[((long)b * C + cc) * 2 + 1] = bias[cc] - (float)mean * a;
    }
}

static inline int gn_pix_per_block(int HW) { return HW >= 16384 ? 512 : (HW >= 1024 ? 128 : 32); }

extern "C" int64_t cvar_groupnorm_ws_bytes(int B, int HW, int C) {
    const int64_t nchunk = cdiv(HW, gn_pix_per_block(HW));
    return ((int64_t)B * nchunk * C * 2 + (int64_t)B * C * 2) * (int64_t)sizeof(float);
}

template <typename T>
static int groupnorm_typed(const T* x, const float* weight, const float* bias, T* out, int B, int HW, int C, int groups,
                           float eps, int silu, void* ws, hipStream_t st) {
    constexpr int VEC = 16 / sizeof(T);
    if (C % VEC || C % groups || C / VEC > 256) return CVAR_EUNSUPPORTED;
    const int ppb = gn_pix_per_block(HW);
    const int nchunk = cdiv(HW, ppb);
    float* partial = (float*)ws;
    float* coef = partial + (size_t)B * nchunk * C * 2;
    const int PL = 256 / (C / VEC);
    hipLaunchKernelGGL(gn_stats_kernel<T>, dim3(nchunk, B), dim3(256), (size_t)PL * C * 2 * sizeof(float), st, x, partial, HW, C, ppb);
    hipLaunchKernelGGL(gn_finalize_kernel<T>, dim3(groups, B), dim3(64), 0, st, partial, nchunk, x, weight, bias, coef, HW, C, groups, eps);
    hipLaunchKernelGGL(gn_apply_kernel<T>, dim3(nchunk, B), dim3(256), 0, st, x, coef, out, HW, C, ppb, silu);
    CVAR_CHECK_LAUNCH();
    return CVAR_OK;
}

extern "C" int cvar_groupnorm_silu_partials(const void* x, int dtype, const float* weight, const float* bias, void* out, int B, int HW, int C, int groups, float eps,
                                            int silu, const float* gn_part, int tiles_per_image, int pixels_per_tile, void* ws, void* stream) {
    if (!x || !weight || !bias || !out || !ws || !gn_part || B <= 0 || HW <= 0 || C <= 0 || groups <= 0 || tiles_per_image <= 0 || pixels_per_tile <= 0) return CVAR_EINVAL;
    if ((long)tiles_per_image * pixels_per_tile != HW) return CVAR_EINVAL;
    if (dtype != CVAR_BF16) return CVAR_EUNSUPPORTED;
    constexpr int VEC = 8;
    if (C % VEC || C % groups || C / VEC > 256) return CVAR_EUNSUPPORTED;
    hipStream_t st = as_stream(stream);
    const int ppb = gn_pix_per_block(HW);
    const int nchunk = cdiv(HW, ppb);
    float* coef = (float*)ws + (size_t)B * nchunk * C * 2;
    hipLaunchKernelGGL(gn_finalize_tiles_kernel, dim3(groups, B), dim3(64), 0, st, gn_part, tiles_per_image, pixels_per_tile, weight, bias, coef, HW, C, groups, eps);
    hipLaunchKernelGGL(gn_apply_kernel<bf16_t>, dim3(nchunk, B), dim3(256), 0, st, (const bf16_t*)x, coef, (bf16_t*)out, HW, C, ppb, silu);
    CVAR_CHECK_LAUNCH();
    return CVAR_OK;
}

extern "C" int cvar_groupnorm_silu(const void* x, int dtype, const float* weight, const float* bias, void* out,
                                   int B, int HW, int C, int groups, float eps, int silu, void* ws, void* stream) {
    if (!x || !weight || !bias || !out || !ws || B <= 0 || HW <= 0 || C <= 0 || groups <= 0) return CVAR_EINVAL;
    if (dtype == CVAR_BF16) return groupnorm_typed<bf16_t>((const bf16_t*)x, weight, bias, (bf16_t*)out, B, HW, C, groups, eps, silu, ws, as_stream(stream));
    if (dtype == CVAR_F32) return groupnorm_typed<float>((const float*)x, weight, bias, (float*)out, B, HW, C, groups, eps, silu, ws, as_stream(stream));
    return CVAR_EUNSUPPORTED;
}

__device__ __forceinline__ void split3_store(bf16_t* __restrict__ o, const float* y, int C) {
    float hi[4], lo[4];
#pragma unroll
    for (int e = 0; e < 4; ++e) { const bf16_t h = f32_to_bf16(y[e]); hi[e] = bf16_to_f32(h); lo[e] = y[e] - hi[e]; }
    const bf16x4_t H = pack_bf16x4(hi), L = pack_bf16x4(lo);
    *(bf16x4_t*)(o) = H;
    *(bf16x4_t*)(o + C) = L;
    *(bf16x4_t*)(o + 2 * C) = H;
}

__global__ __launch_bounds__(256) void split3_kernel(const float* __restrict__ x, long ldx, bf16_t* __restrict__ out, long M, int C, int Cpad) {
    const int nq = C / 4, npad = (Cpad - 3 * C) / 4;
    const long total = M * (nq + npad);
    for (long i = (long)blockIdx.x * 256 + threadIdx.x; i < total; i += (long)gridDim.x * 256) {
        const long m = i / (nq + npad);
        const int q = (int)(i % (nq + npad));
        if (q < nq) {
            const f32x4_t v = *(const f32x4_t*)(x + m * ldx + q * 4);
            const float y[4] = {v[0], v[1], v[2], v[3]};
            split3_store(out + m * Cpad + q * 4, y, C);
        } else {
            const bf16x4_t z = {0, 0, 0, 0};
            *(bf16x4_t*)(out + m * Cpad + 3 * C + (q - nq) * 4) = z;
        }
    }
}

extern "C" int cvar_split3(const float* x, int64_t ldx, void* out, int64_t M, int C, int Cpad, void* stream) {
    if (!x || !out || M <= 0 || C <= 0) return CVAR_EINVAL;
    if (C % 4 || ldx % 4 || Cpad < 3 * C || Cpad % 4 || (((uintptr_t)x | (uintptr_t)out) & 15)) return CVAR_EUNSUPPORTED;
    const long total = M * (long)(Cpad - 2 * C) / 4;
    const int blocks = (int)std::min<long>(cdiv(total, 256L), 256L * 32);
    hipLaunchKernelGGL(split3_kernel, dim3(blocks), dim3(256), 0, as_stream(stream), x, (long)ldx, (bf16_t*)out, (long)M, C, Cpad);
    CVAR_CHECK_LAUNCH();
    return CVAR_OK;
}

__global__ __launch_bounds__(256) void gn_apply_split3_kernel(const float* __restrict__ x, const float* __restrict__ coef, bf16_t* __restrict__ out,
                                                             int HW, int C, int ppb, int silu) {
    const int ncg = C / 4, PL = 256 / ncg;
    const int b = blockIdx.y, chunk = blockIdx.x;
    const int cg = threadIdx.x % ncg, pl = threadIdx.x / ncg;
    if (pl >= PL) return;
    float a[4], d[4];
    {
        const float* cf = coef + ((long)b * C + cg * 4) * 2;
#pragma unroll
        for (int e = 0; e < 4; ++e) { a[e] = cf[2 * e]; d[e] = cf[2 * e + 1]; }
    }
    const int p0 = chunk * ppb, p1 = min(HW, p0 + ppb);
#pragma unroll 4
    for (int p = p0 + pl; p < p1; p += PL) {
        const long row = (long)b * HW + p;
        const f32x4_t v = *(const f32x4_t*)(x + row * C + cg * 4);
        float y[4];
#pragma unroll
        for (int e = 0; e < 4; ++e) y[e] = v[e] * a[e] + d[e];
        if (silu) {
#pragma unroll
            for (int e = 0; e < 4; ++e) y[e] = y[e] / (1.0f + __expf(-y[e]));
        }
        split3_store(out + row * 3 * C + cg * 4, y, C);
    }
}

extern "C" int cvar_groupnorm_silu_split3(const float* x, const float* weight, const float* bias, void* out, int B, int HW, int C, int groups, float eps, int silu,
                                          void* ws, void* stream) {
    if (!x || !weight || !bias || !out || !ws || B <= 0 || HW <= 0 || C <= 0 || groups <= 0) return CVAR_EINVAL;
    if (C % 4 || C % groups || C / 4 > 256 || (((uintptr_t)x | (uintptr_t)out) & 15)) return CVAR_EUNSUPPORTED;
    hipStream_t st = as_stream(stream);
    const int ppb = gn_pix_per_block(HW);
    const int nchunk = cdiv(HW, ppb);
    float* partial = (float*)ws;
    float* coef = partial + (size_t)B * nchunk * C * 2;
    const int PL = 256 / (C / 4);
    hipLaunchKernelGGL(gn_stats_kernel<float>, dim3(nchunk, B), dim3(256), (size_t)PL * C * 2 * sizeof(float), st, x, partial, HW, C, ppb);
    hipLaunchKernelGGL(gn_finalize_kernel<float>, dim3(groups, B), dim3(64), 0, st, partial, nchunk, x, weight, bias, coef, HW, C, groups, eps);
    hipLaunchKernelGGL(gn_apply_split3_kernel, dim3(nchunk, B), dim3(256), 0, st, x, coef, (bf16_t*)out, HW, C, ppb, silu);
    CVAR_CHECK_LAUNCH();
    return CVAR_OK;
}

template <typename TO>
__global__ __launch_bounds__(256) void softmax_rows_kernel(const float* __restrict__ s, TO* __restrict__ p, int rows, int cols) {
    const int lane = threadIdx.x & 63;
    const long row = (long)blockIdx.x * 4 + (threadIdx.x >> 6);
    if (row >= rows) return;
    const float* sr = s + row * cols;
    float v[16];
    float mx = -INFINITY;
#pragma unroll
    for (int i = 0; i < 16; ++i) {
        const int c = i * 64 + lane;
        v[i] = c < cols ? sr[c] : -INFINITY;
        mx = fmaxf(mx, v[i]);
    }
    mx = wave_max(mx);
    float sum = 0.f;
#pragma unroll
    for (int i = 0; i < 16; ++i) { v[i] = __expf(v[i] - mx); sum += v[i]; }
    sum = wave_sum(sum);
    const float inv = 1.0f / sum;
#pragma unroll
    for (int i = 0; i < 16; ++i) {
        const int c = i * 64 + lane;
        if (c < cols) Elem<TO>::st(p + row * cols + c, v[i] * inv);
    }
}

extern "C" int cvar_softmax_rows(const float* s, void* p, int out_dtype, int rows, int cols, void* stream) {
    if (!s || !p || rows <= 0 || cols <= 0) return CVAR_EINVAL;
    if (cols > 1024) return CVAR_EUNSUPPORTED;
    dim3 grid(cdiv(rows, 4)), block(256);
    if (out_dtype == CVAR_BF16) hipLaunchKernelGGL(softmax_rows_kernel<bf16_t>, grid, block, 0, as_stream(stream), s, (bf16_t*)p, rows, cols);
    else if (out_dtype == CVAR_F32) hipLaunchKernelGGL(softmax_rows_kernel<float>, grid, block, 0, as_stream(stream), s, (float*)p, rows, cols);
    else return CVAR_EUNSUPPORTED;
    CVAR_CHECK_LAUNCH();
    return CVAR_OK;
}

template <typename T>
__global__ __launch_bounds__(256) void transpose_kernel(const T* __restrict__ in, T* __restrict__ out, int n, int c, long ld_in, long ld_out) {
    constexpr int VEC = 16 / sizeof(T);
    constexpr int TS = 64;
    constexpr int TPR = TS / VEC;
    constexpr int RPP = 256 / TPR;
    __shared__ T tile[TS][TS + 2 * VEC / VEC + (sizeof(T) == 2 ? 2 : 1)];
    const long b = blockIdx.z;
    const int n0 = blockIdx.x * TS, c0 = blockIdx.y * TS;
    const int tr = threadIdx.x / TPR, tv = (threadIdx.x % TPR) * VEC;
    const bool vec_in = ((ld_in % VEC) == 0) && ((((uintptr_t)in) & 15) == 0);
    const bool vec_out = ((ld_out % VEC) == 0) && ((((uintptr_t)out) & 15) == 0);
    for (int r = tr; r < TS; r += RPP) {
        const int nn = n0 + r, cc = c0 + tv;
        if (nn < n) {
            const T* src = in + (b * n + nn) * ld_in + cc;
            if (vec_in && cc + VEC <= c) {
                T tmp[VEC];
                *(u32x4_t*)tmp = *(const u32x4_t*)src;
#pragma unroll
                for (int e = 0; e < VEC; ++e) tile[r][tv + e] = tmp[e];
            } else {
                for (int e = 0; e < VEC; ++e) if (cc + e < c) tile[r][tv + e] = src[e];
            }
        }
    }
    __syncthreads();
    for (int r = tr; r < TS; r += RPP) {
        const int cidx = c0 + r, nn = n0 + tv;
        if (cidx < c) {
            T* dst = out + (b * c + cidx) * ld_out + nn;
            if (vec_out && nn + VEC <= n) {
                T tmp[VEC];
#pragma unroll
                for (int e = 0; e < VEC; ++e) tmp[e] = tile[tv + e][r];
                *(u32x4_t*)dst = *(const u32x4_t*)tmp;
            } else {
                for (int e = 0; e < VEC; ++e) if (nn + e < n) dst[e] = tile[tv + e][r];
            }
        }
    }
}

extern "C" int cvar_transpose(const void* in, void* out, int dtype, int B, int n, int c, int64_t ld_in, int64_t ld_out, void* stream) {
    if (!in || !out || B <= 0 || n <= 0 || c <= 0 || ld_out < n) return CVAR_EINVAL;
    dim3 grid(cdiv(n, 64), cdiv(c, 64), B), block(256);
    if (dtype == CVAR_BF16) hipLaunchKernelGGL(transpose_kernel<bf16_t>, grid, block, 0, as_stream(stream), (const bf16_t*)in, (bf16_t*)out, n, c, (long)ld_in, (long)ld_out);
    else if (dtype == CVAR_F32) hipLaunchKernelGGL(transpose_kernel<float>, grid, block, 0, as_stream(stream), (const float*)in, (float*)out, n, c, (long)ld_in, (long)ld_out);
    else return CVAR_EUNSUPPORTED;
    CVAR_CHECK_LAUNCH();
    return CVAR_OK;
}

template <typename T>
__global__ __launch_bounds__(256) void rowsum_kernel(const T* __restrict__ A, long lda, float* __restrict__ out, int nrows, int ncols, int accumulate) {
    constexpr int VEC = 16 / sizeof(T);
    const int lane = threadIdx.x & 63;
    const int row = blockIdx.x * 4 + (threadIdx.x >> 6);
    if (row >= nrows) return;
    const T* ar = A + (long)row * lda;
    float acc = 0.f;
    const int nv = ncols / VEC;
    for (int i = lane; i < nv; i += 64) {
        T tmp[VEC];
        *(u32x4_t*)tmp = *(const u32x4_t*)(ar + (long)i * VEC);
#pragma unroll
        for (int e = 0; e < VEC; ++e) acc += Elem<T>::ld(tmp + e);
    }
    for (int j = nv * VEC + lane; j < ncols; j += 64) acc += Elem<T>::ld(ar + j);
    acc = wave_sum(acc);
    if (lane == 0) out[row] = accumulate ? out[row] + acc : acc;
}
extern "C" int cvar_rowsum(const void* A, int dtype, int64_t lda, float* out, int nrows, int ncols, int accumulate, void* stream) {
    if (!A || !out || nrows <= 0 || ncols <= 0) return CVAR_EINVAL;
    const int es = dtype == CVAR_BF16 ? 2 : 4;
    if ((lda * es) % 16 || ((uintptr_t)A & 15)) return CVAR_EUNSUPPORTED;
    dim3 grid(cdiv(nrows, 4)), block(256);
    if (dtype == CVAR_BF16) hipLaunchKernelGGL(rowsum_kernel<bf16_t>, grid, block, 0, as_stream(stream), (const bf16_t*)A, (long)lda, out, nrows, ncols, accumulate);
    else if (dtype == CVAR_F32) hipLaunchKernelGGL(rowsum_kernel<float>, grid, block, 0, as_stream(stream), (const float*)A, (long)lda, out, nrows, ncols, accumulate);
    else return CVAR_EUNSUPPORTED;
    CVAR_CHECK_LAUNCH();
    return CVAR_OK;
}

template <typename TO>
__global__ void nchw_to_nhwc_kernel(const float* __restrict__ in, TO* __restrict__ out, int C, int HW, int Cpad, long total) {
    long i = (long)blockIdx.x * blockDim.x + threadIdx.x;
    const long stride = (long)gridDim.x * blockDim.x;
    for (; i < total; i += stride) {
        const int c = (int)(i % Cpad);
        const long bp = i / Cpad;
        const long p = bp % HW, b = bp / HW;
        Elem<TO>::st(out + i, c < C ? in[(b * C + c) * HW + p] : 0.f);
    }
}

extern "C" int cvar_nchw_to_nhwc(const float* in, void* out, int dtype, int B, int C, int HW, int Cpad, void* stream) {
    if (!in || !out || B <= 0 || C <= 0 || HW <= 0 || Cpad < C) return CVAR_EINVAL;
    const long total = (long)B * HW * Cpad;
    dim3 grid((unsigned)min((long)4096, (total + 255) / 256)), block(256);
    if (dtype == CVAR_BF16) hipLaunchKernelGGL(nchw_to_nhwc_kernel<bf16_t>, grid, block, 0, as_stream(stream), in, (bf16_t*)out, C, HW, Cpad, total);
    else if (dtype == CVAR_F32) hipLaunchKernelGGL(nchw_to_nhwc_kernel<float>, grid, block, 0, as_stream(stream), in, (float*)out, C, HW, Cpad, total);
    else return CVAR_EUNSUPPORTED;
    CVAR_CHECK_LAUNCH();
    return CVAR_OK;
}

template <typename TI>
__global__ void nhwc_to_nchw_kernel(const TI* __restrict__ in, long ld_in, float* __restrict__ out, int C, int HW, long total,
                                    float lo, float hi, float mul, float add) {
    long i = (long)blockIdx.x * blockDim.x + threadIdx.x;
    const long stride = (long)gridDim.x * blockDim.x;
    for (; i < total; i += stride) {
        const long p = i % HW;
        const long bc = i / HW;
        const int c = (int)(bc % C);
        const long b = bc / C;
        float v = Elem<TI>::ld(in + (b * HW + p) * ld_in + c);
        v = fminf(fmaxf(v, lo), hi);
        out[i] = v * mul + add;
    }
}

extern "C" int cvar_nhwc_to_nchw(const void* in, int dtype, int64_t ld_in, float* out, int B, int C, int HW,
                                 float lo, float hi, float mul, float add, void* stream) {
    if (!in || !out || B <= 0 || C <= 0 || HW <= 0) return CVAR_EINVAL;
    const long total = (long)B * C * HW;
    dim3 grid((unsigned)min((long)4096, (total + 255) / 256)), block(256);
    if (dtype == CVAR_BF16) hipLaunchKernelGGL(nhwc_to_nchw_kernel<bf16_t>, grid, block, 0, as_stream(stream), (const bf16_t*)in, (long)ld_in, out, C, HW, total, lo, hi, mul, add);
    else if (dtype == CVAR_F32) hipLaunchKernelGGL(nhwc_to_nchw_kernel<float>, grid, block, 0, as_stream(stream), (const float*)in, (long)ld_in, out, C, HW, total, lo, hi, mul, add);
    else return CVAR_EUNSUPPORTED;
    CVAR_CHECK_LAUNCH();
    return CVAR_OK;
}

extern "C" int cvar_abi_version(void) { return 21; }
extern "C" const char* cvar_status_str(int status) {
    switch (status) {
        case CVAR_OK: return "ok";
        case CVAR_EINVAL: return "invalid argument";
        case CVAR_EUNSUPPORTED: return "unsupported shape or dtype";
        case CVAR_ELAUNCH: return "kernel launch failed";
        default: return "unknown status";
    }
}
```

### controlvar_amd/models.py

```python
from __future__ import annotations

import math
from typing import Any, Dict, List, Optional, Sequence, Tuple, Union

import numpy as np
import torch
import torch.nn as nn

from . import ops
from ._lib import CvarError
from ._lib import ACT_GELU_TANH
from .pyramid import packed_tables
from .spec import DEFAULT_PATCH_NUMS, VaeConfig, VarConfig, attention_levels, vae_state_shapes, var_state_shapes
from .synth import synth_vae_state, synth_var_state


class _Tree(nn.Module):
    """plain container so that dotted state_dict keys map onto nested attributes"""


def _register_tree(root: nn.Module, shapes, values: Dict[str, torch.Tensor], requires_grad: bool):
    for key, (shape, kind) in shapes.items():
        parts = key.split('.')
        m = root
        for p in parts[:-1]:
            if p not in m._modules:
                m.add_module(p, _Tree())
            m = m._modules[p]
        t = values[key]
        assert tuple(t.shape) == tuple(shape), key
        if kind == 'param':
            m.register_parameter(parts[-1], nn.Parameter(t, requires_grad=requires_grad and t.is_floating_point()))
        else:
            m.register_buffer(parts[-1], t)


def _tensor_sig(module: nn.Module):
    return tuple((t.data_ptr(), t._version) for t in list(module.parameters(recurse=True)) + list(module.buffers(recurse=True)))


def _check_index_range(t: torch.Tensor, lo: int, hi: int, what: str):
    if t.numel() == 0:
        return
    if t.is_cuda and torch.cuda.is_current_stream_capturing():
        return
    mn, mx = (int(v) for v in torch.stack((t.min(), t.max())).tolist())
    if mn < lo or mx > hi:
        raise IndexError(f'{what}: index out of range (got [{mn}, {mx}], valid [{lo}, {hi}])')


def _compute_dtype(d) -> torch.dtype:
    if isinstance(d, torch.dtype):
        return d
    return {'bf16': torch.bfloat16, 'bfloat16': torch.bfloat16, 'fp32': torch.float32, 'f32': torch.float32, 'float32': torch.float32}[d]


class VQVAE(nn.Module):

    def __init__(self, vocab_size=4096, z_channels=32, ch=128, dropout=0.0, beta=0.25, using_znorm=False, quant_conv_ks=3,
                 quant_resi=0.5, share_quant_resi=4, default_qresi_counts=0, v_patch_nums=DEFAULT_PATCH_NUMS, test_mode=True,
                 compute_dtype=torch.bfloat16, init_seed: int = 0, decode_chunk: int = 128, encoder_precision: Optional[str] = None):
        super().__init__()
        if using_znorm or quant_conv_ks != 3 or abs(quant_resi - 0.5) > 1e-9 or share_quant_resi != 4 or dropout != 0.0:
            raise NotImplementedError('only the shipped VQVAE configuration (vqvae.py:18-27 defaults, share_quant_resi=4) is built')
        self.cfg = VaeConfig(vocab=vocab_size, z_channels=z_channels, ch=ch, share_quant_resi=share_quant_resi,
                             patch_nums=tuple(v_patch_nums))
        self.test_mode = test_mode
        self.V = self.vocab_size = vocab_size
        self.Cvae = z_channels
        self.downsample = 2 ** (len(self.cfg.ch_mult) - 1)
        self.compute_dtype = _compute_dtype(compute_dtype)
        ep = encoder_precision or ('bf16' if self.compute_dtype == torch.bfloat16 else 'fp32')
        if ep not in ('bf16', 'bf16x3', 'fp32') or (self.compute_dtype == torch.float32 and ep != 'fp32'):
            raise ValueError(f'encoder_precision={encoder_precision!r}: one of bf16 / bf16x3 / fp32 (an fp32 model encodes in fp32)')
        self.encoder_precision = ep
        self.decode_chunk = decode_chunk
        _register_tree(self, vae_state_shapes(self.cfg), synth_vae_state(self.cfg, init_seed), requires_grad=not test_mode)
        self._packed = None
        if test_mode:
            self.eval()

    def load_state_dict(self, state_dict: Dict[str, Any], strict=True, assign=False):
        key = 'quantize.ema_vocab_hit_SV'
        if key in state_dict and state_dict[key].shape[0] != self.quantize.ema_vocab_hit_SV.shape[0]:
            state_dict = dict(state_dict)
            state_dict[key] = self.quantize.ema_vocab_hit_SV
        self._packed = None
        return super().load_state_dict(state_dict, strict=strict, assign=assign)

    def _apply(self, fn, *a, **k):
        self._packed = None
        return super()._apply(fn, *a, **k)

    @property
    def device(self):
        return self.quant_conv.weight.device

    def _state_sig(self):
        return _tensor_sig(self)

    def _pack(self, check: bool = False):
        if self._packed is not None and (not check or self._packed_sig == self._state_sig()):
            return self._packed
        dev, T = self.device, self.compute_dtype
        if dev.type != 'cuda':
            raise RuntimeError('controlvar_amd.VQVAE computes on the GPU only; call .to("cuda") first')
        kch = 8 if T == torch.bfloat16 else 4
        sd = {k: v.detach() for k, v in self.state_dict().items()}
        P: Dict[str, Any] = {'conv': {}, 'norm': {}}
        for k, v in sd.items():
            if k.endswith('.weight') and v.dim() == 4 and not k.startswith('quantize.'):
                name = k[:-len('.weight')]
                fp32_only = name in ('quant_conv', 'post_quant_conv')
                Tw = torch.float32 if fp32_only else T
                kc = 4 if fp32_only else kch
                cout, cin, ks, _ = v.shape
                if ks == 3:
                    cin_p = (cin + kc - 1) // kc * kc
                    w = torch.zeros(cout, 3, 3, cin_p, device=dev, dtype=torch.float32)
                    w[..., :cin] = v.permute(0, 2, 3, 1)
                    w = w.reshape(cout, 9 * cin_p)
                else:
                    cin_p = cin
                    w = v.reshape(cout, cin)
                P['conv'][name] = dict(w=w.to(Tw).contiguous(), b=sd[name + '.bias'].float().contiguous(), cin=cin_p, cout=cout, ks=ks)
                if name.startswith('encoder.') and T == torch.bfloat16 and self.encoder_precision != 'bf16':
                    P.setdefault('enc', {})[name] = self._pack_encoder_conv(v, sd[name + '.bias'], dev)
            elif '.norm' in k and k.endswith('.weight'):
                name = k[:-len('.weight')]
                P['norm'][name] = (v.float().contiguous(), sd[name + '.bias'].float().contiguous())
        P['E'] = sd['quantize.embedding.weight'].float().contiguous()
        nphi = self.cfg.share_quant_resi
        pw = torch.stack([sd[f'quantize.quant_resi.qresi_ls.{k}.weight'] for k in range(nphi)])
        P['phi_w'] = pw.permute(0, 2, 3, 4, 1).reshape(nphi, self.Cvae, 9, self.Cvae).float().contiguous()
        P['phi_b'] = torch.stack([sd[f'quantize.quant_resi.qresi_ls.{k}.bias'] for k in range(nphi)]).float().contiguous()
        r = float(self.cfg.quant_resi)
        pf = pw.float() * r
        pf[:, torch.arange(self.Cvae), torch.arange(self.Cvae), 1, 1] += 1.0 - r
        P['phi_fold_w'] = pf.permute(0, 1, 3, 4, 2).reshape(nphi, self.Cvae, 9 * self.Cvae).contiguous()
        P['phi_fold_b'] = (P['phi_b'] * r).contiguous()
        up, down, offs = packed_tables(self.cfg.patch_nums)
        P['up'] = torch.from_numpy(up).to(dev)
        P['down'] = torch.from_numpy(down).to(dev)
        P['tab_off'] = [int(o) for o in offs]
        P['phi_map'] = self.cfg.phi_map
        self._packed = P
        self._packed_sig = self._state_sig()
        return P

    def _pack_encoder_conv(self, v, bias, dev):
        cout, cin, ks, _ = v.shape
        cin_p = (cin + 3) // 4 * 4
        w = torch.zeros(cout, ks, ks, cin_p, device=dev, dtype=torch.float32)
        w[..., :cin] = v.permute(0, 2, 3, 1).float()
        b = bias.float().contiguous()
        if self.encoder_precision == 'fp32':
            return dict(w=w.reshape(cout, ks * ks * cin_p).contiguous(), b=b, cin=cin_p, cout=cout, ks=ks)
        hi = w.to(torch.bfloat16)
        lo = (w - hi.float()).to(torch.bfloat16)
        cin3 = (3 * cin_p + 7) // 8 * 8
        w3 = torch.zeros(cout, ks, ks, cin3, device=dev, dtype=torch.bfloat16)
        w3[..., :cin_p], w3[..., cin_p:2 * cin_p], w3[..., 2 * cin_p:3 * cin_p] = hi, hi, lo
        return dict(w=w3.reshape(cout, ks * ks * cin3).contiguous(), b=b, cin=cin_p, cin3=cin3, cout=cout, ks=ks)

    GN_FROM_CONV = True

    def _conv(self, x, name, B, Hin, Win, *, stride=1, up=0, residual=None, out_dtype=None):
        c = self._pack()['conv'][name]
        T = c['w'].dtype
        if c['ks'] == 1:
            M = B * Hin * Win
            out = torch.empty(M, c['cout'], device=x.device, dtype=out_dtype or T)
            ops.gemm(x, c['w'], out, M=M, N=c['cout'], K=c['cin'], bias=c['b'], residual=residual, split_k=False)
            return out, Hin, Win
        Hout = Hin * 2 if up else (Hin // 2 if stride == 2 else Hin)
        Wout = Win * 2 if up else (Win // 2 if stride == 2 else Win)
        M = B * Hout * Wout
        out = torch.empty(M, c['cout'], device=x.device, dtype=out_dtype or T)
        geo = ops.conv_gn_partials(T, stride, c['cin'], c['cout'], Hin, Win, Hout, Wout) if (self.GN_FROM_CONV and out.dtype == T) else None
        part = torch.empty(B, geo[0], c['cout'], 3, device=x.device, dtype=torch.float32) if geo else None
        cv = dict(Hin=Hin, Win=Win, Cin=c['cin'], Hout=Hout, Wout=Wout, stride=stride, up=up)
        try:
            ops.gemm(x, c['w'], out, M=M, N=c['cout'], K=9 * c['cin'], bias=c['b'], residual=residual, conv=cv, gn_part=part)
        except CvarError as e:
            if part is None or 'unsupported' not in str(e).lower():
                raise
            geo, part = None, None
            ops.gemm(x, c['w'], out, M=M, N=c['cout'], K=9 * c['cin'], bias=c['b'], residual=residual, conv=cv)
        if geo:
            out._gn_part = (part, geo[0], geo[1])
        return out, Hout, Wout

    def _gn(self, x, name, B, HW, C, silu=True):
        w, b = self._pack()['norm'][name]
        ws = torch.empty(ops.groupnorm_ws_bytes(B, HW, C), device=x.device, dtype=torch.uint8)
        out = torch.empty_like(x)
        gp = getattr(x, '_gn_part', None)
        if gp is not None and gp[0].shape[0] == B and gp[0].shape[2] == C and gp[1] * gp[2] == HW:
            return ops.groupnorm_silu_partials(x, w, b, out, B, HW, C, self.cfg.gn_groups, self.cfg.gn_eps, silu, gp[0], gp[1], gp[2], ws)
        return ops.groupnorm_silu(x, w, b, out, B, HW, C, self.cfg.gn_groups, self.cfg.gn_eps, silu, ws)

    def _resblock(self, x, name, B, H, W, cin, cout):
        h = self._gn(x, name + '.norm1', B, H * W, cin)
        h, _, _ = self._conv(h, name + '.conv1', B, H, W)
        h = self._gn(h, name + '.norm2', B, H * W, cout)
        if cin != cout:
            x, _, _ = self._conv(x, name + '.nin_shortcut', B, H, W)
        h, _, _ = self._conv(h, name + '.conv2', B, H, W, residual=x)
        return h

    def _attnblock(self, x, name, B, HW, C):
        T = x.dtype
        n = self._gn(x, name + '.norm', B, HW, C, silu=False)
        qkv, _, _ = self._conv(n, name + '.qkv', B, HW, 1)
        kch = 16 // x.element_size()
        HWp = -(-HW // kch) * kch
        vT = torch.empty(B, C, HW, device=x.device, dtype=T) if HWp == HW else torch.zeros(B, C, HWp, device=x.device, dtype=T)
        ops.transpose(qkv, vT, B, HW, C, 3 * C, in_off=2 * C, ld_out=HWp)
        s = torch.empty(B, HW, HW, device=x.device, dtype=torch.float32)
        ops.gemm(qkv, qkv, s, M=HW, N=HW, K=C, lda=3 * C, ldw=3 * C, w_off=C, alpha=float(int(C) ** -0.5), batch=B,
                 strideA=HW * 3 * C, strideW=HW * 3 * C, strideC=HW * HW)
        p = torch.empty(B, HW, HW, device=x.device, dtype=T)
        ops.softmax_rows(s, p, B * HW, HW)
        if HWp != HW:
            pp = torch.zeros(B, HW, HWp, device=x.device, dtype=T)
            pp[:, :, :HW] = p
            p = pp
        o = torch.empty(B * HW, C, device=x.device, dtype=T)
        ops.gemm(p, vT, o, M=HW, N=C, K=HWp, batch=B, strideA=HW * HWp, strideW=C * HWp, strideC=HW * C)
        y, _, _ = self._conv(o, name + '.proj_out', B, HW, 1, residual=x)
        return y

    def _encode_f(self, img: torch.Tensor) -> torch.Tensor:
        P = self._pack()
        if self.encoder_precision != ('bf16' if self.compute_dtype == torch.bfloat16 else 'fp32'):
            return self._encode_f_hiprec(img)
        B, _, H, W = img.shape
        T = self.compute_dtype
        cfg = self.cfg
        cin_p = P['conv']['encoder.conv_in']['cin']
        x = torch.empty(B * H * W, cin_p, device=img.device, dtype=T)
        ops.nchw_to_nhwc(img.contiguous().float(), x, B, 3, H * W, cin_p)
        h, H, W = self._conv(x, 'encoder.conv_in', B, H, W)
        nlev = len(cfg.ch_mult)
        in_mult = (1,) + tuple(cfg.ch_mult)
        cur = cfg.ch
        for lv in range(nlev):
            cout = cfg.ch * cfg.ch_mult[lv]
            for b in range(cfg.num_res_blocks):
                h = self._resblock(h, f'encoder.down.{lv}.block.{b}', B, H, W, cur, cout)
                cur = cout
                if lv == nlev - 1:
                    h = self._attnblock(h, f'encoder.down.{lv}.attn.{b}', B, H * W, cur)
            if lv != nlev - 1:
                h, H, W = self._conv(h, f'encoder.down.{lv}.downsample.conv', B, H, W, stride=2)
        h = self._resblock(h, 'encoder.mid.block_1', B, H, W, cur, cur)
        h = self._attnblock(h, 'encoder.mid.attn_1', B, H * W, cur)
        h = self._resblock(h, 'encoder.mid.block_2', B, H, W, cur, cur)
        h = self._gn(h, 'encoder.norm_out', B, H * W, cur)
        z, _, _ = self._conv(h, 'encoder.conv_out', B, H, W, out_dtype=torch.float32)
        f, _, _ = self._conv(z, 'quant_conv', B, H, W)
        out = torch.empty(B, self.Cvae, H, W, device=img.device, dtype=torch.float32)
        ops.nhwc_to_nchw(f, self.Cvae, out, B, self.Cvae, H * W)
        return out

    def _hp_conv(self, x, name, B, Hin, Win, *, stride=1, residual=None, pre_split=False):
        c = self._pack()['enc'][name]
        x3mode = self.encoder_precision == 'bf16x3'
        ks = c['ks']
        Hout, Wout = (Hin // 2, Win // 2) if stride == 2 else (Hin, Win)
        M = B * Hout * Wout
        if x3mode and not pre_split:
            xs = torch.empty(B * Hin * Win, c['cin3'], device=x.device, dtype=torch.bfloat16)
            ops.split3(x, xs, B * Hin * Win, c['cin'], c['cin3'])
            x = xs
        cin = c['cin3'] if x3mode else c['cin']
        out = torch.empty(M, c['cout'], device=x.device, dtype=torch.float32)
        if ks == 1:
            ops.gemm(x, c['w'], out, M=M, N=c['cout'], K=cin, bias=c['b'], residual=residual, split_k=False)
        else:
            ops.gemm(x, c['w'], out, M=M, N=c['cout'], K=9 * cin, bias=c['b'], residual=residual,
                     conv=dict(Hin=Hin, Win=Win, Cin=cin, Hout=Hout, Wout=Wout, stride=stride, up=0))
        return out, Hout, Wout

    def _hp_gn(self, x, name, B, HW, C, silu=True):
        w, b = self._pack()['norm'][name]
        ws = torch.empty(ops.groupnorm_ws_bytes(B, HW, C), device=x.device, dtype=torch.uint8)
        if self.encoder_precision == 'bf16x3':
            out = torch.empty(B * HW, 3 * C, device=x.device, dtype=torch.bfloat16)
            return ops.groupnorm_silu_split3(x, w, b, out, B, HW, C, self.cfg.gn_groups, self.cfg.gn_eps, silu, ws)
        return ops.groupnorm_silu(x, w, b, torch.empty_like(x), B, HW, C, self.cfg.gn_groups, self.cfg.gn_eps, silu, ws)

    def _hp_resblock(self, x, name, B, H, W, cin, cout):
        h = self._hp_gn(x, name + '.norm1', B, H * W, cin)
        h, _, _ = self._hp_conv(h, name + '.conv1', B, H, W, pre_split=True)
        h = self._hp_gn(h, name + '.norm2', B, H * W, cout)
        if cin != cout:
            x, _, _ = self._hp_conv(x, name + '.nin_shortcut', B, H, W)
        h, _, _ = self._hp_conv(h, name + '.conv2', B, H, W, residual=x, pre_split=True)
        return h

    def _hp_attnblock(self, x, name, B, HW, C):
        F32 = torch.float32
        n = self._hp_gn(x, name + '.norm', B, HW, C, silu=False)
        qkv, _, _ = self._hp_conv(n, name + '.qkv', B, HW, 1, pre_split=True)
        HWp = -(-HW // 4) * 4
        vT = torch.empty(B, C, HW, device=x.device, dtype=F32) if HWp == HW else torch.zeros(B, C, HWp, device=x.device, dtype=F32)
        ops.transpose(qkv, vT, B, HW, C, 3 * C, in_off=2 * C, ld_out=HWp)
        s = torch.empty(B, HW, HW, device=x.device, dtype=F32)
        ops.gemm(qkv, qkv, s, M=HW, N=HW, K=C, lda=3 * C, ldw=3 * C, w_off=C, alpha=float(int(C) ** -0.5), batch=B,
                 strideA=HW * 3 * C, strideW=HW * 3 * C, strideC=HW * HW)
        p = torch.empty(B, HW, HW, device=x.device, dtype=F32)
        ops.softmax_rows(s, p, B * HW, HW)
        if HWp != HW:
            pp = torch.zeros(B, HW, HWp, device=x.device, dtype=F32)
            pp[:, :, :HW] = p
            p = pp
        o = torch.empty(B * HW, C, device=x.device, dtype=F32)
        ops.gemm(p, vT, o, M=HW, N=C, K=HWp, batch=B, strideA=HW * HWp, strideW=C * HWp, strideC=HW * C)
        y, _, _ = self._hp_conv(o, name + '.proj_out', B, HW, 1, residual=x)
        return y

    def _encode_f_hiprec(self, img: torch.Tensor) -> torch.Tensor:
        P = self._pack()
        B, _, H, W = img.shape
        cfg = self.cfg
        cin_p = P['enc']['encoder.conv_in']['cin']
        x = torch.empty(B * H * W, cin_p, device=img.device, dtype=torch.float32)
        ops.nchw_to_nhwc(img.contiguous().float(), x, B, 3, H * W, cin_p)
        h, H, W = self._hp_conv(x, 'encoder.conv_in', B, H, W)
        nlev = len(cfg.ch_mult)
        cur = cfg.ch
        for lv in range(nlev):
            cout = cfg.ch * cfg.ch_mult[lv]
            for b in range(cfg.num_res_blocks):
                h = self._hp_resblock(h, f'encoder.down.{lv}.block.{b}', B, H, W, cur, cout)
                cur = cout
                if lv == nlev - 1:
                    h = self._hp_attnblock(h, f'encoder.down.{lv}.attn.{b}', B, H * W, cur)
            if lv != nlev - 1:
                h, H, W = self._hp_conv(h, f'encoder.down.{lv}.downsample.conv', B, H, W, stride=2)
        h = self._hp_resblock(h, 'encoder.mid.block_1', B, H, W, cur, cur)
        h = self._hp_attnblock(h, 'encoder.mid.attn_1', B, H * W, cur)
        h = self._hp_resblock(h, 'encoder.mid.block_2', B, H, W, cur, cur)
        h = self._hp_gn(h, 'encoder.norm_out', B, H * W, cur)
        z, _, _ = self._hp_conv(h, 'encoder.conv_out', B, H, W, pre_split=True)
        f, _, _ = self._conv(z, 'quant_conv', B, H, W)
        out = torch.empty(B, self.Cvae, H, W, device=img.device, dtype=torch.float32)
        ops.nhwc_to_nchw(f, self.Cvae, out, B, self.Cvae, H * W)
        return out

    def _decode(self, f_hat: torch.Tensor, lo=-1.0, hi=1.0, mul=1.0, add=0.0) -> torch.Tensor:
        P = self._pack()
        outs = []
        for s in range(0, f_hat.shape[0], self.decode_chunk):
            outs.append(self._decode_chunk(f_hat[s:s + self.decode_chunk].contiguous(), lo, hi, mul, add))
        return outs[0] if len(outs) == 1 else torch.cat(outs, dim=0)

    def _decode_chunk(self, f_hat, lo, hi, mul, add):
        cfg = self.cfg
        T = self.compute_dtype
        B, Cv, H, W = f_hat.shape
        x = torch.empty(B * H * W, Cv, device=f_hat.device, dtype=torch.float32)
        ops.nchw_to_nhwc(f_hat.float(), x, B, Cv, H * W, Cv)
        z, _, _ = self._conv(x, 'post_quant_conv', B, H, W, out_dtype=T)
        nlev = len(cfg.ch_mult)
        cur = cfg.ch * cfg.ch_mult[-1]
        h, _, _ = self._conv(z, 'decoder.conv_in', B, H, W)
        h = self._resblock(h, 'decoder.mid.block_1', B, H, W, cur, cur)
        h = self._attnblock(h, 'decoder.mid.attn_1', B, H * W, cur)
        h = self._resblock(h, 'decoder.mid.block_2', B, H, W, cur, cur)
        for lv in reversed(range(nlev)):
            cout = cfg.ch * cfg.ch_mult[lv]
            for b in range(cfg.num_res_blocks + 1):
                h = self._resblock(h, f'decoder.up.{lv}.block.{b}', B, H, W, cur, cout)
                cur = cout
                if lv == nlev - 1:
                    h = self._attnblock(h, f'decoder.up.{lv}.attn.{b}', B, H * W, cur)
            if lv != 0:
                h, H, W = self._conv(h, f'decoder.up.{lv}.upsample.conv', B, H, W, up=1)
        h = self._gn(h, 'decoder.norm_out', B, H * W, cur)
        y, _, _ = self._conv(h, 'decoder.conv_out', B, H, W, out_dtype=torch.float32)
        out = torch.empty(B, 3, H, W, device=f_hat.device, dtype=torch.float32)
        ops.nhwc_to_nchw(y, 3, out, B, 3, H * W, lo, hi, mul, add)
        return out

    def _split(self, flat: torch.Tensor, mf: int = 1) -> List[torch.Tensor]:
        outs, o = [], 0
        for pn in self.cfg.patch_nums:
            n = mf * pn * pn
            outs.append(flat[:, o:o + n])
            o += n
        return outs

    def _scale_tables(self, v_patch_nums):
        P = self._pack()
        pns = tuple(int(p[0] if isinstance(p, (tuple, list)) else p) for p in v_patch_nums)
        if any(isinstance(p, (tuple, list)) and p[0] != p[1] for p in v_patch_nums):
            raise NotImplementedError('non-square scales (ph != pw) are not built')
        if pns == tuple(self.cfg.patch_nums):
            return pns, P['up'], P['down'], P['phi_map']
        if pns[-1] != self.cfg.patch_nums[-1]:
            raise AssertionError(f'patch_hws[-1]={pns[-1]} != latent size {self.cfg.patch_nums[-1]}')
        if len(pns) > 16:
            raise NotImplementedError('at most 16 scales')
        cache = P.setdefault('alt_tables', {})
        if pns not in cache:
            from .spec import phi_index_map
            up, down, _ = packed_tables(pns)
            cache[pns] = (torch.from_numpy(up).to(self.device), torch.from_numpy(down).to(self.device), phi_index_map(len(pns), self.cfg.share_quant_resi))
        up, down, pm = cache[pns]
        return pns, up, down, pm

    def _ms_encode(self, f: torch.Tensor, want_fhat=False, want_margin=False, v_patch_nums=None):
        P = self._pack()
        B = f.shape[0]
        pns, up, down, phi_map = self._scale_tables(v_patch_nums) if v_patch_nums is not None else (self.cfg.patch_nums, P['up'], P['down'], P['phi_map'])
        Ltot = sum(p * p for p in pns)
        idx = torch.empty(B, Ltot, device=f.device, dtype=torch.int32)
        fh = torch.empty_like(f) if want_fhat else None
        mg = torch.empty(B, Ltot, device=f.device, dtype=torch.float32) if want_margin else None
        ops.ms_encode(f.contiguous(), P['E'], self.V, P['phi_w'], P['phi_b'], phi_map, list(pns), up, down, idx, fh, mg,
                      B, pns[-1], self.Cvae)
        return idx, fh, mg

    def _next_input(self, si: int, idx: torch.Tensor, f_hat: torch.Tensor, nb: int, nmaps: int, want_tok: bool, soft: Optional[torch.Tensor] = None,
                    pn_next: Optional[int] = None):
        P = self._pack()
        pns = self.cfg.patch_nums
        pn = pns[si]
        last = si == len(pns) - 1
        explicit = pn_next is not None
        if not explicit:
            pn_next = pns[si + 1] if not last else pn
        codebook = P['E']
        if soft is not None:
            codebook = soft.reshape(-1, self.Cvae).float().contiguous()
            idx = torch.arange(codebook.shape[0], device=f_hat.device, dtype=torch.int32).view(nb, -1)
        make_tok = want_tok and (explicit or not last)
        tok = torch.empty(nb, nmaps * pn_next * pn_next, self.Cvae, device=f_hat.device, dtype=torch.float32) if make_tok else None
        down_off = P['tab_off'][pns.index(pn_next)] if make_tok else 0
        ops.ms_next_input(idx, codebook, P['phi_w'], P['phi_b'], P['up'], P['down'], f_hat, tok, nb, nmaps, pn, pn_next, pns[-1], self.Cvae,
                          P['phi_map'][si], P['tab_off'][si], down_off)
        return tok

    @torch.no_grad()
    def img_to_idxBl(self, inp_img_no_grad: torch.Tensor, v_patch_nums=None) -> List[torch.Tensor]:
        self._pack(check=True)
        idx, _, _ = self._ms_encode(self._encode_f(inp_img_no_grad), v_patch_nums=v_patch_nums)
        pns = self._scale_tables(v_patch_nums)[0] if v_patch_nums is not None else self.cfg.patch_nums
        outs, o = [], 0
        for pn in pns:
            outs.append(idx[:, o:o + pn * pn].long())
            o += pn * pn
        return outs

    @torch.no_grad()
    def idxBl_to_h(self, gt_ms_idx_Bl: List[torch.Tensor]) -> List[torch.Tensor]:
        self._pack(check=True)
        B = gt_ms_idx_Bl[0].shape[0]
        dev = gt_ms_idx_Bl[0].device
        S = self.cfg.patch_nums[-1]
        f_hat = torch.zeros(B, 1, self.Cvae, S, S, device=dev, dtype=torch.float32)
        outs = []
        for si in range(len(self.cfg.patch_nums) - 1):
            outs.append(self._next_input(si, gt_ms_idx_Bl[si].to(torch.int32).contiguous(), f_hat, B, 1, True))
        return outs

    def _idx_to_fhat(self, ms_idx_Bl: List[torch.Tensor]) -> torch.Tensor:
        B = ms_idx_Bl[0].shape[0]
        S = self.cfg.patch_nums[-1]
        f_hat = torch.zeros(B, 1, self.Cvae, S, S, device=ms_idx_Bl[0].device, dtype=torch.float32)
        for si in range(len(self.cfg.patch_nums)):
            self._next_input(si, ms_idx_Bl[si].to(torch.int32).contiguous(), f_hat, B, 1, False)
        return f_hat[:, 0]

    @torch.no_grad()
    def fhat_to_img(self, f_hat: torch.Tensor) -> torch.Tensor:
        self._pack(check=True)
        return self._decode(f_hat)

    @torch.no_grad()
    def idxBl_to_img(self, ms_idx_Bl: List[torch.Tensor], same_shape: bool = True, last_one: bool = False):
        self._pack(check=True)
        if not same_shape:
            rows = [self._embed(idx) for idx in ms_idx_Bl]
            fh = self._lowres_fhats(rows, ms_idx_Bl[0].shape[0], last_one)
            return self._decode(fh) if last_one else [self._decode(f) for f in fh]
        if last_one:
            return self._decode(self._idx_to_fhat(ms_idx_Bl))
        B = ms_idx_Bl[0].shape[0]
        S = self.cfg.patch_nums[-1]
        f_hat = torch.zeros(B, 1, self.Cvae, S, S, device=ms_idx_Bl[0].device, dtype=torch.float32)
        outs = []
        for si in range(len(self.cfg.patch_nums)):
            self._next_input(si, ms_idx_Bl[si].to(torch.int32).contiguous(), f_hat, B, 1, False)
            outs.append(self._decode(f_hat[:, 0]))
        return outs

    def _embed(self, idx_Bl: torch.Tensor) -> torch.Tensor:
        P = self._pack()
# ... 725 lines not shown
```

### controlvar_amd/ops.py

```python
from __future__ import annotations

import ctypes as C
from typing import Optional, Sequence

import torch

from . import _lib
from ._lib import ACT_GELU_TANH, ACT_NONE, CVAR_BF16, CVAR_F32, GemmDesc, check

_DT = {torch.float32: CVAR_F32, torch.bfloat16: CVAR_BF16}

GEMM_PROFILE = None


def dt(t_or_dtype) -> int:
    d = t_or_dtype.dtype if isinstance(t_or_dtype, torch.Tensor) else t_or_dtype
    try:
        return _DT[d]
    except KeyError:
        raise TypeError(f'unsupported dtype {d}') from None


def _stream() -> int:
    return torch.cuda.current_stream().cuda_stream


def _ptr(t: Optional[torch.Tensor]) -> Optional[int]:
    if t is None:
        return None
    if not t.is_cuda:
        raise _lib.CvarError('controlvar_amd ops need device tensors (no CPU fallback)')
    return t.data_ptr()


_SPLITK_WS = {}
GEMM_TILE_CFG = 0
GEMM_STAGGER = 0
GEMM_GROUP_M = 0
SMALL_M_KERNEL = True


def ensure_splitk_workspace(device, nbytes: int = 256 << 20) -> torch.Tensor:
    dev = torch.device(device)
    if dev.index is None:
        dev = torch.device('cuda', torch.cuda.current_device())
    key = (dev.index, torch.cuda.current_stream(dev).cuda_stream)
    ws = _SPLITK_WS.get(key)
    if ws is None or ws.numel() < nbytes:
        ws = _SPLITK_WS[key] = torch.empty(nbytes, device=dev, dtype=torch.uint8)
    return ws


def splitk_workspace_keys() -> set:
    return set(_SPLITK_WS)


def take_splitk_workspace(key) -> Optional[torch.Tensor]:
    return _SPLITK_WS.pop(key, None)


def release_splitk_workspace(device=None, stream_handle: Optional[int] = None):
    dev = torch.device(device) if device is not None else torch.device('cuda', torch.cuda.current_device())
    idx = dev.index if dev.index is not None else torch.cuda.current_device()
    if stream_handle is not None:
        _SPLITK_WS.pop((idx, stream_handle), None)
        return
    cur = torch.cuda.current_stream(dev).cuda_stream
    for k in [k for k in _SPLITK_WS if k[0] == idx and k[1] != cur]:
        del _SPLITK_WS[k]


def gemm(A: torch.Tensor, W: torch.Tensor, out: torch.Tensor, *, M: int, N: int, K: int, lda: int = 0, ldw: int = 0, ldc: int = 0,
         bias: Optional[torch.Tensor] = None, act: int = ACT_NONE, alpha: float = 1.0,
         gate: Optional[torch.Tensor] = None, ldg: int = 0, gate_rows: int = 1, gate_off: int = 0,
         residual: Optional[torch.Tensor] = None, ldr: int = 0,
         remap: Optional[Sequence[int]] = None, batch: int = 1, strideA: int = 0, strideW: int = 0, strideC: int = 0, strideR: int = 0,
         conv: Optional[dict] = None, a_off: int = 0, w_off: int = 0, c_off: int = 0,
         pre_act: Optional[torch.Tensor] = None, aux: Optional[torch.Tensor] = None, gate_scale: Optional[torch.Tensor] = None,
         split: Optional[tuple] = None, split_alpha: float = 1.0, ln: Optional[tuple] = None, small_m: bool = False, split_k: bool = True,
         gn_part: Optional[torch.Tensor] = None):
    d = GemmDesc()
    d.M, d.N, d.K, d.dtype = M, N, K, dt(A)
    if W.dtype != A.dtype:
        raise TypeError('A and W must share a dtype')
    d.A = _ptr(A) + a_off * A.element_size()
    d.W = _ptr(W) + w_off * W.element_size()
    d.lda, d.ldw = lda or K, ldw or K
    d.batch, d.strideA, d.strideW, d.strideC, d.strideR = batch, strideA, strideW, strideC, strideR
    if conv:
        d.conv = 1
        d.Hin, d.Win, d.Cin, d.Hout, d.Wout = conv['Hin'], conv['Win'], conv['Cin'], conv['Hout'], conv['Wout']
        d.stride, d.up = conv.get('stride', 1), conv.get('up', 0)
    d.alpha = alpha
    d.bias = _ptr(bias)
    d.act = act
    if gate is not None:
        d.gate = _ptr(gate) + gate_off * 4
        d.ldg, d.gate_rows = ldg, gate_rows
    if residual is not None:
        d.residual, d.res_dtype, d.ldr = _ptr(residual), dt(residual), ldr or N
    d.C = _ptr(out) + c_off * out.element_size()
    d.out_dtype, d.ldc = dt(out), ldc or N
    if remap is not None:
        d.remap_l, d.remap_L, d.remap_off = remap
    d.pre_act, d.aux, d.gate_scale = _ptr(pre_act), _ptr(aux), _ptr(gate_scale)
    if split is not None:
        st, d.split_n, d.ld_split = split
        if st.dtype != out.dtype:
            raise TypeError('split target and out must share a dtype')
        d.C_split = _ptr(st)
        d.split_alpha = float(split_alpha)
    if ln is not None:
        lo, ada, sc_off, sh_off, ld_ada, rows_per, eps = ln
        d.ln_out, d.ln_out_dtype = _ptr(lo), dt(lo)
        d.ln_scale, d.ln_shift = _ptr(ada) + 4 * sc_off, _ptr(ada) + 4 * sh_off
        d.ld_ln, d.ln_rows, d.ln_eps = ld_ada, rows_per, eps
    d.gn_part = _ptr(gn_part)
    ws = _SPLITK_WS.get((A.device.index, _stream()))
    if ws is None:
        ws = ensure_splitk_workspace(A.device)
    if split_k:
        d.ws, d.ws_bytes = ws.data_ptr(), ws.numel()
    d.tile_cfg, d.stagger, d.group_m = (12 if (small_m and GEMM_TILE_CFG == 0 and SMALL_M_KERNEL) else GEMM_TILE_CFG), GEMM_STAGGER, GEMM_GROUP_M
    if GEMM_PROFILE is None:
        check(_lib.load().cvar_gemm(C.byref(d), _stream()), 'cvar_gemm')
    else:
        e0, e1 = torch.cuda.Event(enable_timing=True), torch.cuda.Event(enable_timing=True)
        e0.record()
        check(_lib.load().cvar_gemm(C.byref(d), _stream()), 'cvar_gemm')
        e1.record()
        tag = ('conv' if conv else 'gemm', M, N, K, batch, 'gate' if gate is not None else ('res' if residual is not None else ('act' if act else ('remap' if remap is not None else 'plain'))), str(out.dtype)[6:])
        GEMM_PROFILE.append((e0, e1, 2.0 * M * N * K * batch, tag))
    return out


def gemm_tn(A: torch.Tensor, B: torch.Tensor, out: torch.Tensor, *, T: int, Nn: int, Kk: int, lda: int = 0, ldb: int = 0, ldc: int = 0, c_off: int = 0,
            colsum: Optional[torch.Tensor] = None, colsum_off: int = 0):
    ws = _SPLITK_WS.get((A.device.index, _stream()))
    if ws is None:
        ws = ensure_splitk_workspace(A.device)
    cs = (_ptr(colsum) + 4 * colsum_off) if colsum is not None else None
    check(_lib.load().cvar_gemm_tn(_ptr(A), lda or Nn, _ptr(B), ldb or Kk, _ptr(out) + 4 * c_off, ldc or Kk, T, Nn, Kk, ws.data_ptr(), ws.numel(), cs, _stream()),
          'cvar_gemm_tn')
    return out


def ln_modulate(x: torch.Tensor, ada: torch.Tensor, scale_off: int, shift_off: int, ld_ada: int, rows_per: int,
                out: torch.Tensor, M: int, Cdim: int, eps: float):
    base = _ptr(ada)
    check(_lib.load().cvar_ln_modulate(_ptr(x), base + 4 * scale_off, base + 4 * shift_off, ld_ada, rows_per,
                                       _ptr(out), dt(out), M, Cdim, eps, _stream()), 'cvar_ln_modulate')
    return out


def silu_cast(x: torch.Tensor, out: torch.Tensor):
    check(_lib.load().cvar_silu_cast(_ptr(x), _ptr(out), dt(out), x.numel(), _stream()), 'cvar_silu_cast')
    return out


def _level_arrays(lvl_end, holes):
    n = len(lvl_end) if lvl_end else 0
    arr = (C.c_int * max(n, 1))(*(lvl_end or [0]))
    harr = None
    if holes:
        if len(holes) != n:
            raise ValueError('one (lo, hi) hole per level')
        harr = (C.c_int * (2 * n))(*[int(v) for h in holes for v in h])
    return n, arr, harr


def attention(qkv: torch.Tensor, out: torch.Tensor, R: int, H: int, Lmax: int, q_off: int, l: int, scale: float,
              lvl_end: Optional[Sequence[int]] = None, qkv_off: int = 0, rowwise: bool = False, lse: Optional[torch.Tensor] = None,
              holes: Optional[Sequence[Sequence[int]]] = None, q: Optional[torch.Tensor] = None, prescaled: bool = False, v1: bool = False):
    n, arr, harr = _level_arrays(lvl_end, holes)
    if q is not None and (q.dtype != qkv.dtype or q.numel() < R * l * H * 64):
        raise ValueError('q must hold R*l rows of H*64 elements in the arena dtype')
    if prescaled:
        if rowwise or q is None:
            raise ValueError('prescaled queries: K/V-arena form of the MFMA kernel only')
        check(_lib.load().cvar_attention_prescaled(_ptr(qkv) + qkv_off * qkv.element_size(), _ptr(q), dt(qkv), R, H, Lmax, q_off, l,
                                                   arr, n, harr, _ptr(out), _ptr(lse), _stream()), 'cvar_attention_prescaled')
        return out
    fn = _lib.load().cvar_attention_rowwise if rowwise else (_lib.load().cvar_attention_v1 if v1 else _lib.load().cvar_attention)
    check(fn(_ptr(qkv) + qkv_off * qkv.element_size(), _ptr(q), dt(qkv), R, H, Lmax, q_off, l, scale,
                                     arr, n, harr, _ptr(out), _ptr(lse), _stream()), 'cvar_attention')
    return out


def attention_bwd(qkv, o, dout, lse, dqkv, ws, R, H, Lmax, l, scale, lvl_end=None, qkv_off: int = 0, rowwise: bool = False, holes=None):
    n, arr, harr = _level_arrays(lvl_end, holes)
    fn = _lib.load().cvar_attention_bwd_rowwise if rowwise else _lib.load().cvar_attention_bwd
    check(fn(_ptr(qkv) + qkv_off * qkv.element_size(), dt(qkv), _ptr(o), _ptr(dout), _ptr(lse), R, H, Lmax, 0, l, scale,
                                         arr, n, harr, _ptr(dqkv), _ptr(ws), _stream()), 'cvar_attention_bwd')
    return dqkv


def cos_qk_norm(qkv: torch.Tensor, R: int, H: int, Lmax: int, q_off: int, l: int, scale_mul: torch.Tensor,
                qkv_off: int = 0, sm_off: int = 0, norms: Optional[torch.Tensor] = None, q: Optional[torch.Tensor] = None, q_mul: float = 1.0):
    check(_lib.load().cvar_cos_qk_norm(_ptr(qkv) + qkv_off * qkv.element_size(), _ptr(q), dt(qkv), R, H, Lmax, q_off, l,
                                       _ptr(scale_mul) + 4 * sm_off, _ptr(norms), float(q_mul), _stream()), 'cvar_cos_qk_norm')


def cos_qk_norm_bwd(qkv, dqkv, R, H, Lmax, l, scale_mul, norms, dsm_tok, sm_off: int = 0):
    check(_lib.load().cvar_cos_qk_norm_bwd(_ptr(qkv), _ptr(dqkv), dt(qkv), R, H, Lmax, l, _ptr(scale_mul) + 4 * sm_off, _ptr(norms), _ptr(dsm_tok),
                                           _stream()), 'cvar_cos_qk_norm_bwd')


def cfg_sample(logits: torch.Tensor, B: int, nrep: int, l: int, V: int, coef: Sequence[float], top_k: int, top_p: float,
               seed: int, stage: int, n_draw: int, idx_out: torch.Tensor, combined: Optional[torch.Tensor] = None,
               margin: Optional[torch.Tensor] = None, kept: Optional[torch.Tensor] = None, seed_dev: Optional[torch.Tensor] = None,
               ldv: int = 0, codebook: Optional[torch.Tensor] = None, smooth_mul: float = 1.0, smooth_tau: float = 1.0,
               gumbel: Optional[torch.Tensor] = None, soft_out: Optional[torch.Tensor] = None):
    arr = (C.c_float * 4)(*(list(coef) + [0.0] * (4 - len(coef))))
    check(_lib.load().cvar_cfg_sample(_ptr(logits), B, nrep, l, V, arr, top_k, float(top_p), int(seed) & (2 ** 64 - 1), _ptr(seed_dev), stage, n_draw,
                                      _ptr(idx_out), _ptr(combined), _ptr(margin), _ptr(kept), int(ldv), _ptr(codebook),
                                      codebook.shape[1] if codebook is not None else 0, float(smooth_mul), float(smooth_tau), _ptr(gumbel), _ptr(soft_out),
                                      _stream()), 'cvar_cfg_sample')
    return idx_out


def ms_next_input(idx: torch.Tensor, codebook, phi_w, phi_b, up, down, f_hat, tok_out, nb, nmaps, pn, pn_next, S, Cvae,
                  phi_k: int, up_off: int, down_off: int):
    lib = _lib.load()
    pw = _ptr(phi_w) + 4 * phi_k * Cvae * 9 * Cvae
    pb = _ptr(phi_b) + 4 * phi_k * Cvae
    check(lib.cvar_ms_next_input(_ptr(idx), _ptr(codebook), pw, pb, _ptr(up) + 4 * up_off, _ptr(down) + 4 * down_off,
                                 _ptr(f_hat), _ptr(tok_out), nb, nmaps, pn, pn_next, S, Cvae, _stream()), 'cvar_ms_next_input')


def ms_encode(f, codebook, V, phi_w, phi_b, phi_map, patch_nums, up, down, idx_out, f_hat_out, margin_out, B, S, Cvae):
    n = len(patch_nums)
    pm = (C.c_int * n)(*phi_map)
    pn = (C.c_int * n)(*patch_nums)
    check(_lib.load().cvar_ms_encode(_ptr(f), _ptr(codebook), V, _ptr(phi_w), _ptr(phi_b), pm, pn, n, _ptr(up), _ptr(down),
                                     _ptr(idx_out), _ptr(f_hat_out), _ptr(margin_out), B, S, Cvae, _stream()), 'cvar_ms_encode')


def word_embed(tok, W, bias, lvl_pos, x, nb, nrep, l, Cvae, Cdim, x_rows, x_off, lvl_off: int = 0):
    check(_lib.load().cvar_word_embed(_ptr(tok), _ptr(W), _ptr(bias), _ptr(lvl_pos) + 4 * lvl_off * Cdim, _ptr(x), nb, nrep, l, Cvae, Cdim,
                                      x_rows, x_off, _stream()), 'cvar_word_embed')


def first_tokens(class_emb, cond_embed, labels, types, pos_start, lvl_pos, x, cond, R, first_l, Cdim, x_rows):
    check(_lib.load().cvar_first_tokens(_ptr(class_emb), _ptr(cond_embed), _ptr(labels), _ptr(types), _ptr(pos_start), _ptr(lvl_pos),
                                        _ptr(x), _ptr(cond), R, first_l, Cdim, x_rows, _stream()), 'cvar_first_tokens')


def groupnorm_ws_bytes(B, HW, Cdim) -> int:
    return int(_lib.load().cvar_groupnorm_ws_bytes(B, HW, Cdim))


def groupnorm_silu(x, weight, bias, out, B, HW, Cdim, groups, eps, silu, ws):
    check(_lib.load().cvar_groupnorm_silu(_ptr(x), dt(x), _ptr(weight), _ptr(bias), _ptr(out), B, HW, Cdim, groups, eps, int(silu),
                                          _ptr(ws), _stream()), 'cvar_groupnorm_silu')
    return out


def split3(x, out, M, Cdim, Cpad=0, ldx=0):
    check(_lib.load().cvar_split3(_ptr(x), ldx or Cdim, _ptr(out), M, Cdim, Cpad or 3 * Cdim, _stream()), 'cvar_split3')
    return out


def groupnorm_silu_split3(x, weight, bias, out, B, HW, Cdim, groups, eps, silu, ws):
    check(_lib.load().cvar_groupnorm_silu_split3(_ptr(x), _ptr(weight), _ptr(bias), _ptr(out), B, HW, Cdim, groups, eps, int(silu), _ptr(ws), _stream()),
          'cvar_groupnorm_silu_split3')
    return out


def conv_gn_partials(dtype: torch.dtype, stride: int, Cin: int, Cout: int, Hin: int, Win: int, Hout: int, Wout: int):
    if GEMM_TILE_CFG not in (0, 6):
        return None
    nt, pp = C.c_int(0), C.c_int(0)
    if dtype not in _DT:
        return None
    ok = _lib.load().cvar_conv3x3_gn_partials(_DT[dtype], stride, Cin, Cout, Hin, Win, Hout, Wout, C.byref(nt), C.byref(pp))
    return (nt.value, pp.value) if ok else None


def groupnorm_silu_partials(x, weight, bias, out, B, HW, Cdim, groups, eps, silu, gn_part, tiles, tile_pixels, ws):
    check(_lib.load().cvar_groupnorm_silu_partials(_ptr(x), dt(x), _ptr(weight), _ptr(bias), _ptr(out), B, HW, Cdim, groups, eps, int(silu),
                                                   _ptr(gn_part), tiles, tile_pixels, _ptr(ws), _stream()), 'cvar_groupnorm_silu_partials')
    return out


def softmax_rows(s, p, rows, cols):
    check(_lib.load().cvar_softmax_rows(_ptr(s), _ptr(p), dt(p), rows, cols, _stream()), 'cvar_softmax_rows')
    return p


def transpose(inp, out, B, n, c, ld_in, in_off: int = 0, ld_out: int = 0):
    check(_lib.load().cvar_transpose(_ptr(inp) + in_off * inp.element_size(), _ptr(out), dt(inp), B, n, c, ld_in, ld_out or n, _stream()), 'cvar_transpose')
    return out


def nchw_to_nhwc(inp, out, B, Cdim, HW, Cpad):
    check(_lib.load().cvar_nchw_to_nhwc(_ptr(inp), _ptr(out), dt(out), B, Cdim, HW, Cpad, _stream()), 'cvar_nchw_to_nhwc')
    return out


def nhwc_to_nchw(inp, ld_in, out, B, Cdim, HW, lo=-3.0e38, hi=3.0e38, mul=1.0, add=0.0):
    check(_lib.load().cvar_nhwc_to_nchw(_ptr(inp), dt(inp), ld_in, _ptr(out), B, Cdim, HW, lo, hi, mul, add, _stream()), 'cvar_nhwc_to_nchw')
    return out


def embed_rows(idx: torch.Tensor, codebook: torch.Tensor, out: torch.Tensor):
    check(_lib.load().cvar_embed_rows(_ptr(idx), _ptr(codebook), codebook.shape[0], _ptr(out), idx.numel(), codebook.shape[1], _stream()), 'cvar_embed_rows')
    return out


def resample_sep(inp: torch.Tensor, wy: torch.Tensor, wx: torch.Tensor, out: torch.Tensor, B: int, h: int, w: int, H: int, W: int, Cdim: int):
    check(_lib.load().cvar_resample_sep(_ptr(inp), _ptr(wy), _ptr(wx), _ptr(out), B, h, w, H, W, Cdim, _stream()), 'cvar_resample_sep')
    return out


def gate_residual(x, f, gate, gate_off, ldg, gate_rows, rowscale, M, Cdim):
    check(_lib.load().cvar_gate_residual(_ptr(x), _ptr(f), dt(f), _ptr(gate) + 4 * gate_off, ldg, gate_rows, _ptr(rowscale), M, Cdim, _stream()), 'cvar_gate_residual')


def train_ws_floats(M: int, R: int, Cdim: int) -> int:
    return int(_lib.load().cvar_train_ws_floats(M, R, Cdim))


def gated_grad(dx, f, gate, gate_off, ldg, rowscale, df, dgate, dgate_off, ldo, R, l, Cdim, ws):
    check(_lib.load().cvar_gated_grad(_ptr(dx), _ptr(f), dt(f), _ptr(gate) + 4 * gate_off, ldg, _ptr(rowscale), _ptr(df), _ptr(dgate) + 4 * dgate_off, ldo,
                                      R, l, Cdim, _ptr(ws), ws.numel(), _stream()), 'cvar_gated_grad')


def gelu(a, h):
    check(_lib.load().cvar_gelu(_ptr(a), _ptr(h), dt(a), a.numel(), _stream()), 'cvar_gelu')
    return h


def gelu_bwd(a, dh):
    check(_lib.load().cvar_gelu_bwd(_ptr(a), _ptr(dh), dt(a), a.numel(), _stream()), 'cvar_gelu_bwd')
    return dh


def ln_modulate_bwd(x, dy, ada, scale_off, ld_ada, rows_per, dx_in, dx_out, dada, dscale_off, dshift_off, ldo, M, Cdim, eps, ws):
    check(_lib.load().cvar_ln_modulate_bwd(_ptr(x), _ptr(dy), dt(dy), _ptr(ada) + 4 * scale_off, ld_ada, rows_per, _ptr(dx_in), _ptr(dx_out),
                                           _ptr(dada) + 4 * dscale_off, _ptr(dada) + 4 * dshift_off, ldo, M, Cdim, eps, _ptr(ws), ws.numel(), _stream()), 'cvar_ln_modulate_bwd')


def colsum(A, lda, out, M, N, ws, accumulate=False, a_off: int = 0, out_off: int = 0):
    check(_lib.load().cvar_colsum(_ptr(A) + a_off * A.element_size(), dt(A), lda, _ptr(out) + 4 * out_off, M, N, int(accumulate), _ptr(ws), _stream()), 'cvar_colsum')


def wordembed_grad(dx, ldx: int, rows_per_sample: int, skip: int, tok, n_per_sample: int, B: int, Cdim: int, Cvae: int, out, w_off: int, b_off: int,
                   dx_off: int = 0):
    lib = _lib.load()
    nb = lib.cvar_wordembed_grad_ws_bytes(B * n_per_sample, Cdim)
    ws = torch.empty(nb, device=dx.device, dtype=torch.uint8)
    check(lib.cvar_wordembed_grad(_ptr(dx) + 4 * dx_off, ldx, rows_per_sample, skip, _ptr(tok), n_per_sample, B, Cdim, Cvae,
                                  _ptr(out) + 4 * w_off, _ptr(out) + 4 * b_off, _ptr(ws), _stream()), 'cvar_wordembed_grad')


def rowsum(A, lda, out, nrows, ncols, accumulate=False, out_off: int = 0):
    check(_lib.load().cvar_rowsum(_ptr(A), dt(A), lda, _ptr(out) + 4 * out_off, nrows, ncols, int(accumulate), _stream()), 'cvar_rowsum')


def ce_fwd_bwd(logits, target, weight, gscale, loss_tok, dlogits, M, V):
    check(_lib.load().cvar_ce_fwd_bwd(_ptr(logits), _ptr(target), _ptr(weight), float(gscale), _ptr(loss_tok), _ptr(dlogits),
                                      dt(dlogits) if dlogits is not None else CVAR_F32, M, V, _stream()), 'cvar_ce_fwd_bwd')


def scatter_add_rows(src, ld_src, idx, dst, n, Cdim, src_off: int = 0):
    check(_lib.load().cvar_scatter_add_rows(_ptr(src) + 4 * src_off, ld_src, _ptr(idx), _ptr(dst), n, Cdim, _stream()), 'cvar_scatter_add_rows')


def silu_bwd(cond, dsilu, dcond):
    check(_lib.load().cvar_silu_bwd(_ptr(cond), _ptr(dsilu), _ptr(dcond), cond.numel(), _stream()), 'cvar_silu_bwd')


def adamw(p, g, m, v, lr, b1, b2, eps, wd, step, gscale_dev=None, gscale=1.0):
    check(_lib.load().cvar_adamw(_ptr(p), _ptr(g), _ptr(m), _ptr(v), p.numel(), lr, b1, b2, eps, wd, step, _ptr(gscale_dev), gscale, _stream()), 'cvar_adamw')


def sumsq(x, partial, slot):
    check(_lib.load().cvar_sumsq(_ptr(x), x.numel(), _ptr(partial) + 8 * 256 * slot, _stream()), 'cvar_sumsq')


def adam_table(entries, device) -> torch.Tensor:
    rows = []
    for (p, g, m, v, group, *rest) in entries:
        w16 = rest[0] if rest else None
        if w16 is not None and (w16.dtype != torch.bfloat16 or w16.numel() != p.numel() or not w16.is_contiguous()):
            raise ValueError('adam_table: the bf16 copy must be a contiguous bfloat16 tensor of the size of the parameter')
        rows.append([p.data_ptr(), g.data_ptr(), m.data_ptr(), v.data_ptr(), p.numel(), int(group) & 0xffffffff, w16.data_ptr() if w16 is not None else 0])
    return torch.tensor(rows, dtype=torch.int64).to(device)


def sumsq_multi(table: torch.Tensor, n: int, partial: torch.Tensor):
    check(_lib.load().cvar_sumsq_multi(_ptr(table), n, _ptr(partial), _stream()), 'cvar_sumsq_multi')


def adamw_multi(table: torch.Tensor, n: int, lrs: Sequence[float], wds: Sequence[float], b1, b2, eps, step, gscale_dev=None, gscale=1.0):
    la = (C.c_float * len(lrs))(*lrs)
    wa = (C.c_float * len(wds))(*wds)
    check(_lib.load().cvar_adamw_multi(_ptr(table), n, la, wa, len(lrs), b1, b2, eps, step, _ptr(gscale_dev), gscale, _stream()), 'cvar_adamw_multi')


def clip_coef(partial, count, pre_scale, max_norm, out2):
    check(_lib.load().cvar_clip_coef(_ptr(partial), count, pre_scale, max_norm, _ptr(out2), _stream()), 'cvar_clip_coef')


def resample_u8(src: torch.Tensor, src_h: int, src_w: int, channels: int, axis: int, dst_extent: int, bounds: torch.Tensor,
                coeffs: torch.Tensor, ksize: int, dst: torch.Tensor):
    check(_lib.load().cvar_resample_u8(_ptr(src), src_h, src_w, channels, axis, dst_extent, _ptr(bounds), _ptr(coeffs), ksize, _ptr(dst),
                                       _stream()), 'cvar_resample_u8')
    return dst


def crop_flip_normalize(src: torch.Tensor, src_h: int, src_w: int, channels: int, top: int, left: int, out_h: int, out_w: int,
                        flip: bool, dst: torch.Tensor):
    check(_lib.load().cvar_crop_flip_normalize(_ptr(src), src_h, src_w, channels, top, left, out_h, out_w, int(flip), _ptr(dst),
                                               _stream()), 'cvar_crop_flip_normalize')
    return dst


def ignore_mask(cond: torch.Tensor, B: int, H: int, W: int, patch_nums: Sequence[int], first_masked_scale: int, image_first: int,
                out: torch.Tensor, L: int):
    arr = (C.c_int * len(patch_nums))(*patch_nums)
    check(_lib.load().cvar_ignore_mask(_ptr(cond), B, H, W, arr, len(patch_nums), first_masked_scale, image_first, _ptr(out), L,
                                       _stream()), 'cvar_ignore_mask')
    return out


def rle_paint(run_ends: torch.Tensor, ann_offsets: torch.Tensor, colours: torch.Tensor, n_ann: int, H: int, W: int, out: torch.Tensor):
    check(_lib.load().cvar_rle_paint(_ptr(run_ends), _ptr(ann_offsets), _ptr(colours), n_ann, H, W, _ptr(out), _stream()), 'cvar_rle_paint')
    return out


def lora_down(x, A, u, *, M: int, K: int, r: int, scale: float, p: float = 0.0, seed: int = 0, tag: int = 0, ldx: int = 0, lda: int = 0,
              ldu: int = 0, x_off: int = 0, u_off: int = 0, x_copy=None, ld_copy: int = 0):
    if A.dtype != x.dtype or u.dtype != x.dtype:
        raise TypeError('lora_down: x, A and u must share a dtype')
    es = x.element_size()
    check(_lib.load().cvar_lora_down(_ptr(x) + x_off * es, ldx or K, _ptr(A), lda or K, _ptr(u) + u_off * es, ldu or r, _ptr(x_copy), ld_copy or K,
                                     M, K, r, dt(x), float(scale), float(p), int(seed) & (2 ** 64 - 1), int(tag) & 0xffffffff, _stream()),
          'cvar_lora_down')
    return u


def lora_dx(dx, du, A, *, M: int, K: int, r: int, scale: float, p: float = 0.0, seed: int = 0, tag: int = 0, lddx: int = 0, lddu: int = 0,
            lda: int = 0, du_off: int = 0, aux=None, ldaux: int = 0):
    if A.dtype != du.dtype or (aux is not None and aux.dtype != du.dtype):
        raise TypeError('lora_dx: du, A and aux must share a dtype')
    check(_lib.load().cvar_lora_dx(_ptr(dx), lddx or K, dt(dx), _ptr(du) + du_off * du.element_size(), lddu or 16, _ptr(A), lda or K, _ptr(aux),
                                   ldaux or K, M, K, r, dt(du), float(scale), float(p), int(seed) & (2 ** 64 - 1), int(tag) & 0xffffffff, _stream()),
          'cvar_lora_dx')
    return dx


def lora_wgrad_ws_floats(M: int, N: int) -> int:
    return int(_lib.load().cvar_lora_wgrad_ws_floats(M, N))


def lora_wgrad(Y, Z, out, ws, *, M: int, N: int, r: int, scale: float = 1.0, p: float = 0.0, seed: int = 0, tag: int = 0, ldy: int = 0,
               ldz: int = 0, y_off: int = 0, z_off: int = 0, out_off: int = 0, os_n: int = 0, os_j: int = 1):
    if Y.dtype != Z.dtype:
        raise TypeError('lora_wgrad: Y and Z must share a dtype')
    if out.dtype != torch.float32 or ws.dtype != torch.float32:
        raise TypeError('lora_wgrad: out and ws are fp32')
    es = Y.element_size()
    check(_lib.load().cvar_lora_wgrad(_ptr(Y) + y_off * es, ldy or N, _ptr(Z) + z_off * es, ldz or r, M, N, r, dt(Y), float(scale), float(p),
                                      int(seed) & (2 ** 64 - 1), int(tag) & 0xffffffff, _ptr(ws), ws.numel(), _ptr(out) + 4 * out_off,
                                      os_n or r, os_j, _stream()), 'cvar_lora_wgrad')
    return out


def lora_dropout_mask(M: int, K: int, p: float, seed: int, tag: int, device=None) -> torch.Tensor:
    dev = torch.device(device) if device is not None else torch.device('cuda', torch.cuda.current_device())
    out = torch.empty(M, K, device=dev, dtype=torch.float32)
    check(_lib.load().cvar_lora_dropout_mask(_ptr(out), M, K, float(p), int(seed) & (2 ** 64 - 1), int(tag) & 0xffffffff, _stream()),
          'cvar_lora_dropout_mask')
    return out
```

### include/cvar.h

```cpp
#ifndef CVAR_H
#define CVAR_H

#include <stdint.h>

#ifdef __cplusplus
extern "C" {
#endif

typedef enum { CVAR_OK = 0, CVAR_EINVAL = -1, CVAR_EUNSUPPORTED = -2, CVAR_ELAUNCH = -3 } cvar_status;
typedef enum { CVAR_F32 = 0, CVAR_BF16 = 1 } cvar_dtype;
typedef enum { CVAR_ACT_NONE = 0, CVAR_ACT_GELU_TANH = 1, CVAR_ACT_GELU_GRAD = 2 } cvar_act;

int cvar_abi_version(void);
const char* cvar_status_str(int status);

typedef struct {
    int M, N, K;
    int dtype;
    const void* A; int64_t lda;
    const void* W; int64_t ldw;
    int batch;
    int64_t strideA, strideW, strideC, strideR;
    int conv;
    int Hin, Win, Cin, Hout, Wout, stride, up;
    float alpha;
    const float* bias;
    int act;
    const float* gate; int64_t ldg; int gate_rows;
    const void* residual; int res_dtype; int64_t ldr;
    void* C; int out_dtype; int64_t ldc;
    int remap_l, remap_L, remap_off;
    void* pre_act;
    const void* aux;
    const float* gate_scale;
    void* ws; int64_t ws_bytes;
    int tile_cfg;
    int stagger;
    int group_m;
    void* C_split; int split_n; int64_t ld_split;
    float split_alpha;
    void* ln_out; int ln_out_dtype;
    const float* ln_scale; const float* ln_shift; int64_t ld_ln; int ln_rows; float ln_eps;
    float* gn_part;
} cvar_gemm_desc;
int cvar_gemm(const cvar_gemm_desc* d, void* stream);
int cvar_conv3x3_gn_partials(int dtype, int stride, int Cin, int Cout, int Hin, int Win, int Hout, int Wout, int* tiles_per_image, int* pixels_per_tile);

int cvar_gemm_tn(const void* A, int64_t lda, const void* B, int64_t ldb, float* C, int64_t ldc, int T, int Nn, int Kk,
                 float* ws, int64_t ws_bytes, float* colsum_a, void* stream);

int cvar_ln_modulate(const float* x, const float* scale, const float* shift, int64_t ld_ada, int rows_per,
                     void* out, int out_dtype, int M, int C, float eps, void* stream);

int cvar_silu_cast(const float* x, void* out, int out_dtype, int64_t n, void* stream);

int cvar_attention(const void* qkv, const void* q, int dtype, int R, int H, int Lmax, int q_off, int l, float scale,
                   const int* lvl_end_host, int n_lvl, const int* hole_host, void* out,
                   float* lse , void* stream);
int cvar_attention_rowwise(const void* qkv, const void* q, int dtype, int R, int H, int Lmax, int q_off, int l, float scale,
                           const int* lvl_end_host, int n_lvl, const int* hole_host, void* out, float* lse, void* stream);
int cvar_attention_prescaled(const void* kv, const void* q, int dtype, int R, int H, int Lmax, int q_off, int l,
                             const int* lvl_end_host, int n_lvl, const int* hole_host, void* out, float* lse, void* stream);
int cvar_attention_v1(const void* qkv, const void* q, int dtype, int R, int H, int Lmax, int q_off, int l, float scale,
                      const int* lvl_end_host, int n_lvl, const int* hole_host, void* out, float* lse, void* stream);
int cvar_attention_bwd(const void* qkv, int dtype, const void* o, const void* dout, const float* lse, int R, int H, int Lmax,
                       int q_off, int l, float scale, const int* lvl_end_host, int n_lvl, const int* hole_host, void* dqkv, float* ws, void* stream);
int cvar_attention_bwd_rowwise(const void* qkv, int dtype, const void* o, const void* dout, const float* lse, int R, int H, int Lmax,
                               int q_off, int l, float scale, const int* lvl_end_host, int n_lvl, const int* hole_host, void* dqkv, float* ws,
                               void* stream);

int cvar_cos_qk_norm(void* qkv, void* q, int dtype, int R, int H, int Lmax, int q_off, int l, const float* scale_mul,
                     float* norms ,
                     float q_mul , void* stream);
int cvar_cos_qk_norm_bwd(const void* qkv, void* dqkv, int dtype, int R, int H, int Lmax, int l, const float* scale_mul,
                         const float* norms, float* dsm_tok, void* stream);

int cvar_cfg_sample(const float* logits, int B, int nrep, int l, int V, const float* coef_host,
                    int top_k, float top_p, uint64_t seed, const uint64_t* seed_dev , int stage, int n_draw,
                    int32_t* idx_out, float* combined, float* margin, int32_t* kept, int ldv,
                    const float* codebook , int Cvae, float smooth_mul, float smooth_tau, const float* gumbel, float* soft_out,
                    void* stream);

int cvar_ms_next_input(const int32_t* idx, const float* codebook, const float* phi_w, const float* phi_b,
                       const float* up_mat, const float* down_mat, float* f_hat, float* tok_out,
                       int nb, int nmaps, int pn, int pn_next, int S, int Cvae, void* stream);

int cvar_ms_encode(const float* f, const float* codebook, int V, const float* phi_w, const float* phi_b,
                   const int* phi_map_host, const int* patch_nums_host, int nscale, const float* up_mats,
                   const float* down_mats, int32_t* idx_out, float* f_hat_out, float* margin_out,
                   int B, int S, int Cvae, void* stream);

int cvar_word_embed(const float* tok, const float* W, const float* bias, const float* lvl_pos, float* x,
                    int nb, int nrep, int l, int Cvae, int C, int x_rows, int x_off, void* stream);

int cvar_first_tokens(const float* class_emb, const float* cond_embed, const int32_t* labels, const int32_t* types,
                      const float* pos_start, const float* lvl_pos, float* x, float* cond, int R, int first_l,
                      int C, int x_rows, void* stream);

int64_t cvar_groupnorm_ws_bytes(int B, int HW, int C);
int cvar_groupnorm_silu(const void* x, int dtype, const float* weight, const float* bias, void* out,
                        int B, int HW, int C, int groups, float eps, int silu, void* ws, void* stream);
int cvar_groupnorm_silu_partials(const void* x, int dtype, const float* weight, const float* bias, void* out, int B, int HW, int C, int groups, float eps,
                                 int silu, const float* gn_part, int tiles_per_image, int pixels_per_tile, void* ws, void* stream);
int cvar_split3(const float* x, int64_t ldx, void* out_bf16, int64_t M, int C, int Cpad, void* stream);
int cvar_groupnorm_silu_split3(const float* x, const float* weight, const float* bias, void* out_bf16, int B, int HW, int C, int groups, float eps, int silu,
                               void* ws, void* stream);
int cvar_softmax_rows(const float* s, void* p, int out_dtype, int rows, int cols, void* stream);
int cvar_transpose(const void* in, void* out, int dtype, int B, int n, int c, int64_t ld_in, int64_t ld_out , void* stream);
int cvar_nchw_to_nhwc(const float* in, void* out, int dtype, int B, int C, int HW, int Cpad, void* stream);
int cvar_nhwc_to_nchw(const void* in, int dtype, int64_t ld_in, float* out, int B, int C, int HW,
                      float lo, float hi, float mul, float add, void* stream);

int cvar_embed_rows(const int32_t* idx, const float* codebook, int V, float* out, int64_t n, int C, void* stream);
int cvar_resample_sep(const float* in, const float* wy, const float* wx, float* out, int B, int h, int w, int H, int W, int C, void* stream);

int cvar_gate_residual(float* x, const void* f, int dtype, const float* gate, int64_t ldg, int gate_rows,
                       const float* rowscale, int64_t M, int C, void* stream);
int64_t cvar_train_ws_floats(int64_t M, int R, int C);
int cvar_gated_grad(const float* dx, const void* f, int dtype, const float* gate, int64_t ldg, const float* rowscale,
                    void* df, float* dgate, int64_t ldo, int R, int l, int C, float* ws, int64_t ws_floats, void* stream);
int cvar_gelu(const void* a, void* h, int dtype, int64_t n, void* stream);
int cvar_gelu_bwd(const void* a, void* dh, int dtype, int64_t n, void* stream);
int cvar_ln_modulate_bwd(const float* x, const void* dy, int dtype, const float* scale, int64_t ld_ada, int rows_per,
                         const float* dx_in, float* dx_out, float* dscale, float* dshift, int64_t ldo,
                         int M, int C, float eps, float* ws, int64_t ws_floats, void* stream);
int64_t cvar_wordembed_grad_ws_bytes(int64_t ntok, int C);
int cvar_wordembed_grad(const float* dx, int64_t ldx, int rows_per_sample, int skip, const float* tok, int n_per_sample, int B, int C, int Cvae,
                        float* dW, float* db, float* ws, void* stream);
int cvar_colsum(const void* A, int dtype, int64_t lda, float* out, int64_t M, int N, int accumulate, float* ws, void* stream);
int cvar_rowsum(const void* A, int dtype, int64_t lda, float* out, int nrows, int ncols, int accumulate, void* stream);
int cvar_ce_fwd_bwd(const float* logits, const int32_t* target, const float* weight, float gscale, float* loss_tok,
                    void* dlogits, int out_dtype, int64_t M, int V, void* stream);
int cvar_scatter_add_rows(const float* src, int64_t ld_src, const int32_t* idx, float* dst, int n, int C, void* stream);
int cvar_silu_bwd(const float* cond, const float* dsilu, float* dcond, int64_t n, void* stream);
int cvar_adamw(float* p, const float* g, float* m, float* v, int64_t n, float lr, float beta1, float beta2, float eps,
               float weight_decay, int step, const float* gscale_dev, float gscale, void* stream);
int cvar_sumsq(const float* x, int64_t n, double* partial256, void* stream);
int cvar_clip_coef(const double* partials, int64_t count, float pre_scale, float max_norm, float* out2, void* stream);
typedef struct { float* p; const float* g; float* m; float* v; int64_t n; int32_t group; int32_t pad; uint16_t* w16; } cvar_adam_tensor;
int cvar_sumsq_multi(const void* table_dev , int n_tensors, double* partials, void* stream);
int cvar_adamw_multi(const void* table_dev, int n_tensors, const float* lr_by_group_host, const float* wd_by_group_host, int n_groups,
                     float beta1, float beta2, float eps, int step, const float* gscale_dev, float gscale, void* stream);

int cvar_lora_down(const void* x, int64_t ldx, const void* A, int64_t lda, void* u, int64_t ldu, void* x_copy, int64_t ld_copy, int M, int K,
                   int r, int dtype, float scale, float p, uint64_t seed, uint32_t tag, void* stream);
int cvar_lora_dx(void* dx, int64_t lddx, int dx_dtype, const void* du, int64_t lddu, const void* A, int64_t lda, const void* aux, int64_t ldaux,
                 int M, int K, int r, int dtype, float scale, float p, uint64_t seed, uint32_t tag, void* stream);
int64_t cvar_lora_wgrad_ws_floats(int M, int N);
int cvar_lora_wgrad(const void* Y, int64_t ldy, const void* Z, int64_t ldz, int M, int N, int r, int dtype, float scale, float p, uint64_t seed,
                    uint32_t tag, float* ws, int64_t ws_floats, float* out, int64_t os_n, int64_t os_j, void* stream);
int cvar_lora_dropout_mask(float* out, int M, int K, float p, uint64_t seed, uint32_t tag, void* stream);

int cvar_resample_u8(const void* src, int src_h, int src_w, int channels, int axis, int dst_extent,
                     const int* bounds, const int* coeffs, int ksize, void* dst, void* stream);
int cvar_crop_flip_normalize(const void* src, int src_h, int src_w, int channels, int top, int left, int out_h, int out_w,
                             int flip, float* dst, void* stream);
int cvar_ignore_mask(const float* cond, int B, int H, int W, const int* patch_nums_host, int n_scales, int first_masked_scale,
                     int image_first, float* out, int L, void* stream);
int cvar_rle_paint(const int* run_ends, const int* ann_offsets, const void* colours, int n_ann, int H, int W, void* out, void* stream);

int cvar_probe_mfma_bf16(const void* operands, int64_t operand_bytes, int iters, float* sink, void* stream);
int cvar_probe_mfma_bf16_32x32(const void* operands, int64_t operand_bytes, int iters, float* sink, void* stream);
double cvar_probe_mfma_flops(int iters);

#ifdef __cplusplus
}
#endif
#endif
```

Before: 203.7 images/s.

## Fuse GroupNorm+SiLU into the halo conv3x3 input load path in the VQVAE decoder

```diff
diff --git a/controlvar_amd/_lib.py b/controlvar_amd/_lib.py
--- a/controlvar_amd/_lib.py
+++ b/controlvar_amd/_lib.py
@@ -6,7 +6,7 @@
 
 HERE = os.path.dirname(os.path.abspath(__file__))
 LIB_PATH = os.environ.get('CVAR_LIB') or os.path.join(HERE, 'libcvar_hip.so')
-ABI_VERSION = 21
+ABI_VERSION = 22
 
 CVAR_F32, CVAR_BF16 = 0, 1
 ACT_NONE, ACT_GELU_TANH, ACT_GELU_GRAD = 0, 1, 2
@@ -34,6 +34,7 @@
         ('C_split', c_p), ('split_n', c_i), ('ld_split', c_l), ('split_alpha', c_f),
         ('ln_out', c_p), ('ln_out_dtype', c_i), ('ln_scale', c_p), ('ln_shift', c_p), ('ld_ln', c_l), ('ln_rows', c_i), ('ln_eps', c_f),
         ('gn_part', c_p),
+        ('in_gn', c_p), ('in_gn_silu', c_i),
     ]
 
 
@@ -68,6 +69,10 @@
     'cvar_split3': (c_i, [c_p, c_l, c_p, c_l, c_i, c_i, c_p]),
     'cvar_groupnorm_silu_split3': (c_i, [c_p, c_p, c_p, c_p, c_i, c_i, c_i, c_i, c_f, c_i, c_p, c_p]),
     'cvar_conv3x3_gn_partials': (c_i, [c_i, c_i, c_i, c_i, c_i, c_i, c_i, c_i, C.POINTER(c_i), C.POINTER(c_i)]),
+    'cvar_conv3x3_in_gn': (c_i, [c_i, c_i, c_i, c_i, c_i, c_i, c_i, c_i, c_i]),
+    'cvar_groupnorm_coef': (c_i, [c_p, c_i, c_p, c_p, c_p, c_i, c_i, c_i, c_i, c_f, c_p, c_p]),
+    'cvar_groupnorm_coef_partials': (c_i, [c_p, c_p, c_p, c_i, c_i, c_i, c_i, c_f, c_p, c_i, c_i, c_p]),
+    'cvar_groupnorm_apply': (c_i, [c_p, c_i, c_p, c_p, c_i, c_i, c_i, c_i, c_p]),
     'cvar_softmax_rows': (c_i, [c_p, c_p, c_i, c_i, c_i, c_p]),
     'cvar_gemm_tn': (c_i, [c_p, c_l, c_p, c_l, c_p, c_l, c_i, c_i, c_i, c_p, c_l, c_p, c_p]),
     'cvar_embed_rows': (c_i, [c_p, c_p, c_i, c_p, c_l, c_i, c_p]),
diff --git a/controlvar_amd/csrc/conv_halo.hip b/controlvar_amd/csrc/conv_halo.hip
--- a/controlvar_amd/csrc/conv_halo.hip
+++ b/controlvar_amd/csrc/conv_halo.hip
@@ -11,10 +11,12 @@
     int B, H, W, Cin, Cout, tiles_x, tiles_y, nchunk;
     int up, Hin, Win;
     float* gn_part;
+    const float* in_gn;
+    int in_gn_silu;
 };
 
 
-template <int CH_NB, typename TO, int TW = 16>
+template <int CH_NB, typename TO, bool GN = false, int TW = 16>
 __global__ __launch_bounds__(TW * 16, 2) void conv3x3_halo_bf16_kernel(const ConvHaloParams p) {
     constexpr int NW = TW / 4;
     constexpr int CH_HROW = TW + 4;
@@ -24,7 +26,8 @@
     constexpr int CH_W_BYTES = CH_NB * 2048;
     constexpr int W_PIECES = CH_NB * 2;
     constexpr int W_PER_WAVE = (W_PIECES + NW - 1) / NW;
-    __shared__ __attribute__((aligned(1024))) char smem[2 * CH_HALO_BYTES + 3 * CH_W_BYTES];
+    constexpr int CH_GN_BYTES = GN ? NW * 256 : 0;
+    __shared__ __attribute__((aligned(1024))) char smem[2 * CH_HALO_BYTES + 3 * CH_W_BYTES + CH_GN_BYTES];
     const int tid = threadIdx.x, lane = tid & 63;
     const int wave = __builtin_amdgcn_readfirstlane(tid >> 6);
     const int lrow = lane & 31, hi = lane >> 5;
@@ -56,6 +59,31 @@
         const int n = q >> 2, lc = (q & 3) ^ ((n >> 2) & 3);
         w_off[jj] = (n < 32 * CH_NB && cout0 + n < p.Cout) ? (unsigned)((n * 9 * p.Cin + lc * 8) * 2) : 0x80000000u;
     }
+    char* gn_slot = smem + 2 * CH_HALO_BYTES + 3 * CH_W_BYTES + wave * 256;
+    __amdgpu_buffer_rsrc_t gn_rsrc;
+    if constexpr (GN) gn_rsrc = __builtin_amdgcn_make_buffer_rsrc((void*)(p.in_gn + (long)b * p.Cin * 2), 0, p.Cin * 8, 0x00020000);
+    auto issue_gn = [&](int c) -> int {
+        if constexpr (GN) {
+            __builtin_amdgcn_raw_ptr_buffer_load_lds(gn_rsrc, (lptr_t)gn_slot, 4, lane * 4, c * 256, 0, 0);
+            return 1;
+        }
+        return 0;
+    };
+    auto transform = [&](char* hbuf, int jj) {
+        if constexpr (GN) {
+            const int j = wave + NW * jj;
+            if (j < CH_HALO_PIECES && h_off[jj] != 0x80000000u) {
+                const int q = j * 64 + lane;
+                const int hx = (q >> 2) % CH_HROW;
+                const int lc = (q & 3) ^ ((hx >> 2) & 3);
+                float ad[16];
+#pragma unroll
+                for (int e = 0; e < 4; ++e) *(f32x4_t*)(ad + 4 * e) = *(const f32x4_t*)(gn_slot + lc * 64 + e * 16);
+                bf16x8_t* v = (bf16x8_t*)(hbuf + j * 1024 + lane * 16);
+                *v = gn_silu_bf16x8(*v, ad, p.in_gn_silu != 0);
+            }
+        }
+    };
     auto issue_halo = [&](int c, int jj) -> int {
         const int j = wave + NW * jj;
         if (j >= CH_HALO_PIECES) return 0;
@@ -76,7 +104,8 @@
         return n;
     };
     auto wait_vm = [&](int n) {
-        if (n >= 4) asm volatile("s_waitcnt vmcnt(4)" ::: "memory");
+        if (GN && n >= 5) asm volatile("s_waitcnt vmcnt(5)" ::: "memory");
+        else if (n >= 4) asm volatile("s_waitcnt vmcnt(4)" ::: "memory");
         else if (n == 3) asm volatile("s_waitcnt vmcnt(3)" ::: "memory");
         else if (n == 2) asm volatile("s_waitcnt vmcnt(2)" ::: "memory");
         else if (n == 1) asm volatile("s_waitcnt vmcnt(1)" ::: "memory");
@@ -97,11 +126,16 @@
 #pragma unroll
             for (int r = 0; r < 16; ++r) acc[i][j][r] = 0.f;
 
+    issue_gn(0);
 #pragma unroll
     for (int jj = 0; jj < H_PER_WAVE; ++jj) issue_halo(0, jj);
     issue_w(0, 0);
     issue_w(0, 1);
     asm volatile("s_waitcnt vmcnt(0)" ::: "memory");
+    if constexpr (GN) {
+#pragma unroll
+        for (int jj = 0; jj < H_PER_WAVE; ++jj) transform(smem, jj);
+    }
     __builtin_amdgcn_s_barrier();
 
     bf16x8_t af[2][2][2];
@@ -122,6 +156,7 @@
 #pragma unroll
         for (int t = 0; t < 9; ++t) {
             int issued = 0;
+            if (t == 0 && c + 1 < p.nchunk) issued += issue_gn(c + 1);
             if (t < H_PER_WAVE && c + 1 < p.nchunk) issued += issue_halo(c + 1, t);
             {
                 const int c2 = t + 2 >= 9 ? c + 1 : c, t2 = t + 2 >= 9 ? t + 2 - 9 : t + 2;
@@ -141,6 +176,9 @@
                 for (int j = 0; j < CH_NB; ++j)
 #pragma unroll
                     for (int i = 0; i < 2; ++i) acc[i][j] = __builtin_amdgcn_mfma_f32_32x32x16_bf16(w[ks][j], af[t & 1][i][ks], acc[i][j], 0, 0, 0);
+            if constexpr (GN) {
+                if (t >= 2 && t - 2 < H_PER_WAVE && c + 1 < p.nchunk) transform((char*)hb_next, t - 2);
+            }
             wait_vm(issued);
             __builtin_amdgcn_s_barrier();
         }
@@ -324,12 +362,14 @@
 }
 
 int cvar_conv3x3_halo_bf16(const void* X, const void* Wt, const float* bias, const void* residual, void* out, int out_f32, int B, int H, int W, int Cin,
-                           int Cout, int up, float* gn_part, hipStream_t st) {
+                           int Cout, int up, float* gn_part, const float* in_gn, int in_gn_silu, hipStream_t st) {
     ConvHaloParams p;
     p.X = (const bf16_t*)X; p.Wt = (const bf16_t*)Wt; p.bias = bias; p.res = (const bf16_t*)residual; p.out = out;
     p.B = B; p.H = H; p.W = W; p.Cin = Cin; p.Cout = Cout; p.tiles_x = W / 16; p.tiles_y = H / 16; p.nchunk = Cin / 32;
     p.up = up ? 1 : 0; p.Hin = up ? H / 2 : H; p.Win = up ? W / 2 : W;
     p.gn_part = gn_part;
+    p.in_gn = in_gn; p.in_gn_silu = in_gn_silu ? 1 : 0;
+    if (in_gn && (((uintptr_t)in_gn & 3) != 0 || (Cout % 160 == 0 && out_f32))) return CVAR_EUNSUPPORTED;
     if (gn_part && !(Cout % 160 == 0 && !out_f32)) return CVAR_EUNSUPPORTED;
     const long tiles = (long)B * p.tiles_x * p.tiles_y;
     if (tiles <= 0 || tiles > 0x7fffffffL) return CVAR_EINVAL;
@@ -338,9 +378,12 @@
         hipLaunchKernelGGL((conv3x3_halo_bf16_kernel<5, float>), dim3((unsigned)tiles, Cout / 160), dim3(256), 0, st, p);
     } else if (Cout % 160 == 0 && !out_f32) {
         if ((((uintptr_t)out | (uintptr_t)residual) & 15) != 0 || (long)H * W * Cout >= 0x7fffffffL) return CVAR_EUNSUPPORTED;
-        hipLaunchKernelGGL((conv3x3_halo_bf16_kernel<5, bf16_t>), dim3((unsigned)tiles, Cout / 160), dim3(256), 0, st, p);
+        if (in_gn) hipLaunchKernelGGL((conv3x3_halo_bf16_kernel<5, bf16_t, true>), dim3((unsigned)tiles, Cout / 160), dim3(256), 0, st, p);
+        else hipLaunchKernelGGL((conv3x3_halo_bf16_kernel<5, bf16_t>), dim3((unsigned)tiles, Cout / 160), dim3(256), 0, st, p);
     } else if (Cout <= 32 && !residual) {
-        if (out_f32) hipLaunchKernelGGL((conv3x3_halo_bf16_kernel<1, float>), dim3((unsigned)tiles, 1), dim3(256), 0, st, p);
+        if (out_f32 && in_gn) hipLaunchKernelGGL((conv3x3_halo_bf16_kernel<1, float, true>), dim3((unsigned)tiles, 1), dim3(256), 0, st, p);
+        else if (out_f32) hipLaunchKernelGGL((conv3x3_halo_bf16_kernel<1, float>), dim3((unsigned)tiles, 1), dim3(256), 0, st, p);
+        else if (in_gn) hipLaunchKernelGGL((conv3x3_halo_bf16_kernel<1, bf16_t, true>), dim3((unsigned)tiles, 1), dim3(256), 0, st, p);
         else hipLaunchKernelGGL((conv3x3_halo_bf16_kernel<1, bf16_t>), dim3((unsigned)tiles, 1), dim3(256), 0, st, p);
     } else {
         return CVAR_EUNSUPPORTED;
diff --git a/controlvar_amd/csrc/cvar_common.h b/controlvar_amd/csrc/cvar_common.h
--- a/controlvar_amd/csrc/cvar_common.h
+++ b/controlvar_amd/csrc/cvar_common.h
@@ -90,9 +90,20 @@
     return sg + t * sg * (1.0f - sg) * k2 * (1.0f + 0.134145f * t * t);
 }
 
+__device__ __forceinline__ bf16x8_t gn_silu_bf16x8(const bf16x8_t v, const float* ad, bool silu) {
+    float y[8];
+#pragma unroll
+    for (int e = 0; e < 8; ++e) y[e] = bf16_to_f32((bf16_t)v[e]) * ad[2 * e] + ad[2 * e + 1];
+    if (silu) {
+#pragma unroll
+        for (int e = 0; e < 8; ++e) y[e] = y[e] * __builtin_amdgcn_rcpf(1.0f + __builtin_amdgcn_exp2f(-1.4426950408889634f * y[e]));
+    }
+    return pack_bf16x8(y);
+}
+
 static inline hipStream_t as_stream(void* s) { return (hipStream_t)s; }
 static inline int cdiv(int64_t a, int64_t b) { return (int)((a + b - 1) / b); }
 
 int cvar_conv3x3_halo_bf16(const void* X, const void* Wt, const float* bias, const void* residual, void* out, int out_f32, int B, int H, int W, int Cin,
-                           int Cout, int up, float* gn_part, hipStream_t st);
+                           int Cout, int up, float* gn_part, const float* in_gn, int in_gn_silu, hipStream_t st);
 int cvar_conv3x3_c8_bf16(const void* X, const void* Wt, const float* bias, void* out, int B, int H, int W, int Cout, float* gn_part, hipStream_t st);
diff --git a/controlvar_amd/csrc/gemm.hip b/controlvar_amd/csrc/gemm.hip
--- a/controlvar_amd/csrc/gemm.hip
+++ b/controlvar_amd/csrc/gemm.hip
@@ -1114,6 +1114,15 @@
     return 1;
 }
 
+extern "C" int cvar_conv3x3_in_gn(int dtype, int stride, int Cin, int Cout, int Hin, int Win, int Hout, int Wout, int out_dtype) {
+    const bool grid = dtype == CVAR_BF16 && stride == 1 && Cin > 0 && Cin % 32 == 0 && Cout > 0 && Hout > 0 && Wout > 0 && Hout % 16 == 0 && Wout % 16 == 0 &&
+                      (Hout == Hin || Hout == 2 * Hin) && Wout == Hout / Hin * Win && (long)Hin * Win * Cin * 2 < 0x7fffffffL;
+    if (!grid) return 0;
+    const bool wide = Cout % 160 == 0 && out_dtype == CVAR_BF16 && (long)Hout * Wout * Cout < 0x7fffffffL;
+    const bool narrow = Cout <= 32 && (out_dtype == CVAR_BF16 || out_dtype == CVAR_F32) && (long)Hout * Wout >= 65536;
+    return wide || narrow ? 1 : 0;
+}
+
 extern "C" int cvar_gemm(const cvar_gemm_desc* d, void* stream) {
     if (!d || !d->A || !d->W || !d->C) return CVAR_EINVAL;
     if (d->M <= 0 || d->N <= 0 || d->K <= 0 || d->batch < 1) return CVAR_EINVAL;
@@ -1133,6 +1142,7 @@
         return CVAR_EUNSUPPORTED;
     }
     if (d->gn_part && !d->conv) return CVAR_EINVAL;
+    if (d->in_gn && !d->conv) return CVAR_EUNSUPPORTED;
     if (d->gate && d->gate_rows <= 0) return CVAR_EINVAL;
     if (d->act == CVAR_ACT_GELU_GRAD && !d->aux) return CVAR_EINVAL;
     if (d->pre_act && d->act == CVAR_ACT_GELU_GRAD) return CVAR_EINVAL;
@@ -1241,7 +1251,7 @@
         }
     }
 #ifndef CVAR_NO_CONV_C8
-    if (d->conv && d->dtype == CVAR_BF16 && d->stride == 1 && !d->up && d->batch == 1 && (d->tile_cfg == 0 || d->tile_cfg == 6) && d->Cin == 8 && d->N % 160 == 0 &&
+    if (d->conv && d->dtype == CVAR_BF16 && d->stride == 1 && !d->up && d->batch == 1 && (d->tile_cfg == 0 || d->tile_cfg == 6) && d->Cin == 8 && d->N % 160 == 0 && !d->in_gn &&
         d->Hout % 16 == 0 && d->Wout % 16 == 0 && d->act == CVAR_ACT_NONE && !d->gate && d->alpha == 1.0f && !d->residual && !d->pre_act && !d->aux && !d->gate_scale &&
         d->remap_l == 0 && d->split_n == 0 && d->strideC == 0 && d->ldc == d->N && d->ldw == d->K && d->out_dtype == CVAR_BF16 &&
         ((((uintptr_t)d->C | (uintptr_t)d->bias) & 15) == 0) && (long)d->Hout * d->Wout * d->N < 0x7fffffffL)
@@ -1257,14 +1267,15 @@
                           (long)d->Hout * d->Wout * d->N < 0x7fffffffL;
         const bool narrow = d->N <= 32 && !d->residual && (d->out_dtype == CVAR_BF16 || d->out_dtype == CVAR_F32) && ((long)d->Hout * d->Wout >= 65536 || d->tile_cfg == 6);
         if (d->gn_part && !wide) return CVAR_EUNSUPPORTED;
+        if (d->in_gn && !(wide || narrow)) return CVAR_EUNSUPPORTED;
         const bool wide32 = d->N % 160 == 0 && d->out_dtype == CVAR_F32 && (((uintptr_t)d->C & 15) == 0) && !d->up &&
                             (!d->residual || (d->res_dtype == CVAR_F32 && d->ldr == d->N && (((uintptr_t)d->residual & 15) == 0))) &&
                             (long)d->Hout * d->Wout * d->N < 0x7fffffffL;
         if (wide || narrow || wide32)
             return cvar_conv3x3_halo_bf16(d->A, d->W, d->bias, d->residual, d->C, d->out_dtype == CVAR_F32, d->M / (d->Hout * d->Wout), d->Hout, d->Wout, d->Cin,
-                                          d->N, d->up, d->gn_part, st);
-    }
-    if (d->gn_part) return CVAR_EUNSUPPORTED;
+                                          d->N, d->up, d->gn_part, d->in_gn, d->in_gn_silu, st);
+    }
+    if (d->gn_part || d->in_gn) return CVAR_EUNSUPPORTED;
     if (d->dtype == CVAR_BF16) return d->conv ? cvar_gemm_launch_conv_bf16(p, d->batch, st) : ln_after(launch_typed<bf16_t>(p, d->batch, st));
     return ln_after(cvar_gemm_launch_f32(p, d->batch, st));
 }
diff --git a/controlvar_amd/csrc/ops.hip b/controlvar_amd/csrc/ops.hip
--- a/controlvar_amd/csrc/ops.hip
+++ b/controlvar_amd/csrc/ops.hip
@@ -368,37 +368,28 @@
     const int b = blockIdx.y, chunk = blockIdx.x;
     const int cg = threadIdx.x % ncg, pl = threadIdx.x / ncg;
     if (pl >= PL) return;
-    float a[VEC], d[VEC];
+    float a[VEC], d[VEC], ad[2 * VEC];
     {
         const float* cf = coef + ((long)b * C + cg * VEC) * 2;
 #pragma unroll
-        for (int e = 0; e < VEC; ++e) { a[e] = cf[2 * e]; d[e] = cf[2 * e + 1]; }
+        for (int e = 0; e < VEC; ++e) { a[e] = cf[2 * e]; d[e] = cf[2 * e + 1]; ad[2 * e] = a[e]; ad[2 * e + 1] = d[e]; }
     }
     const int p0 = chunk * ppb, p1 = min(HW, p0 + ppb);
     const long base = (long)b * HW * C + cg * VEC;
 #pragma unroll 4
     for (int p = p0 + pl; p < p1; p += PL) {
         const long off = base + (long)p * C;
-        float y[VEC];
         if constexpr (sizeof(T) == 2) {
-            const bf16x8_t v = *(const bf16x8_t*)(x + off);
-#pragma unroll
-            for (int e = 0; e < VEC; ++e) y[e] = bf16_to_f32((bf16_t)v[e]) * a[e] + d[e];
+            *(bf16x8_t*)(out + off) = gn_silu_bf16x8(*(const bf16x8_t*)(x + off), ad, silu != 0);
         } else {
             const f32x4_t v = *(const f32x4_t*)(x + off);
+            float y[VEC];
 #pragma unroll
             for (int e = 0; e < VEC; ++e) y[e] = v[e] * a[e] + d[e];
-        }
-        if (silu) {
-#pragma unroll
-            for (int e = 0; e < VEC; ++e) {
-                if constexpr (sizeof(T) == 2) y[e] = y[e] * __builtin_amdgcn_rcpf(1.0f + __builtin_amdgcn_exp2f(-1.4426950408889634f * y[e]));
-                else y[e] = y[e] / (1.0f + __expf(-y[e]));
+            if (silu) {
+#pragma unroll
+                for (int e = 0; e < VEC; ++e) y[e] = y[e] / (1.0f + __expf(-y[e]));
             }
-        }
-        if constexpr (sizeof(T) == 2) {
-            *(bf16x8_t*)(out + off) = pack_bf16x8(y);
-        } else {
             f32x4_t o = {y[0], y[1], y[2], y[3]};
             *(f32x4_t*)(out + off) = o;
         }
@@ -487,6 +478,50 @@
     if (dtype == CVAR_BF16) return groupnorm_typed<bf16_t>((const bf16_t*)x, weight, bias, (bf16_t*)out, B, HW, C, groups, eps, silu, ws, as_stream(stream));
     if (dtype == CVAR_F32) return groupnorm_typed<float>((const float*)x, weight, bias, (float*)out, B, HW, C, groups, eps, silu, ws, as_stream(stream));
     return CVAR_EUNSUPPORTED;
+}
+
+template <typename T>
+static int groupnorm_coef_typed(const T* x, const float* weight, const float* bias, float* coef, int B, int HW, int C, int groups, float eps, void* ws, hipStream_t st) {
+    constexpr int VEC = 16 / sizeof(T);
+    if (C % VEC || C % groups || C / VEC > 256) return CVAR_EUNSUPPORTED;
+    const int ppb = gn_pix_per_block(HW);
+    const int nchunk = cdiv(HW, ppb);
+    const int PL = 256 / (C / VEC);
+    hipLaunchKernelGGL(gn_stats_kernel<T>, dim3(nchunk, B), dim3(256), (size_t)PL * C * 2 * sizeof(float), st, x, (float*)ws, HW, C, ppb);
+    hipLaunchKernelGGL(gn_finalize_kernel<T>, dim3(groups, B), dim3(64), 0, st, (const float*)ws, nchunk, x, weight, bias, coef, HW, C, groups, eps);
+    CVAR_CHECK_LAUNCH();
+    return CVAR_OK;
+}
+
+extern "C" int cvar_groupnorm_coef(const void* x, int dtype, const float* weight, const float* bias, float* coef, int B, int HW, int C, int groups, float eps,
+                                   void* ws, void* stream) {
+    if (!x || !weight || !bias || !coef || !ws || B <= 0 || HW <= 0 || C <= 0 || groups <= 0) return CVAR_EINVAL;
+    if (dtype == CVAR_BF16) return groupnorm_coef_typed<bf16_t>((const bf16_t*)x, weight, bias, coef, B, HW, C, groups, eps, ws, as_stream(stream));
+    if (dtype == CVAR_F32) return groupnorm_coef_typed<float>((const float*)x, weight, bias, coef, B, HW, C, groups, eps, ws, as_stream(stream));
+    return CVAR_EUNSUPPORTED;
+}
+
+extern "C" int cvar_groupnorm_coef_partials(const float* weight, const float* bias, float* coef, int B, int HW, int C, int groups, float eps,
+                                            const float* gn_part, int tiles_per_image, int pixels_per_tile, void* stream) {
+    if (!weight || !bias || !coef || !gn_part || B <= 0 || HW <= 0 || C <= 0 || groups <= 0 || tiles_per_image <= 0 || pixels_per_tile <= 0) return CVAR_EINVAL;
+    if ((long)tiles_per_image * pixels_per_tile != HW) return CVAR_EINVAL;
+    if (C % groups) return CVAR_EUNSUPPORTED;
+    hipLaunchKernelGGL(gn_finalize_tiles_kernel, dim3(groups, B), dim3(64), 0, as_stream(stream), gn_part, tiles_per_image, pixels_per_tile, weight, bias, coef,
+                       HW, C, groups, eps);
+    CVAR_CHECK_LAUNCH();
+    return CVAR_OK;
+}
+
+extern "C" int cvar_groupnorm_apply(const void* x, int dtype, const float* coef, void* out, int B, int HW, int C, int silu, void* stream) {
+    if (!x || !coef || !out || B <= 0 || HW <= 0 || C <= 0) return CVAR_EINVAL;
+    const int VEC = dtype == CVAR_BF16 ? 8 : 4;
+    if ((dtype != CVAR_BF16 && dtype != CVAR_F32) || C % VEC || C / VEC > 256) return CVAR_EUNSUPPORTED;
+    const int ppb = gn_pix_per_block(HW);
+    const dim3 grid(cdiv(HW, ppb), B);
+    if (dtype == CVAR_BF16) hipLaunchKernelGGL(gn_apply_kernel<bf16_t>, grid, dim3(256), 0, as_stream(stream), (const bf16_t*)x, coef, (bf16_t*)out, HW, C, ppb, silu);
+    else hipLaunchKernelGGL(gn_apply_kernel<float>, grid, dim3(256), 0, as_stream(stream), (const float*)x, coef, (float*)out, HW, C, ppb, silu);
+    CVAR_CHECK_LAUNCH();
+    return CVAR_OK;
 }
 
 __device__ __forceinline__ void split3_store(bf16_t* __restrict__ o, const float* y, int C) {
@@ -744,7 +779,7 @@
     return CVAR_OK;
 }
 
-extern "C" int cvar_abi_version(void) { return 21; }
+extern "C" int cvar_abi_version(void) { return 22; }
 extern "C" const char* cvar_status_str(int status) {
     switch (status) {
         case CVAR_OK: return "ok";
diff --git a/controlvar_amd/models.py b/controlvar_amd/models.py
--- a/controlvar_amd/models.py
+++ b/controlvar_amd/models.py
@@ -53,6 +53,16 @@
     if isinstance(d, torch.dtype):
         return d
     return {'bf16': torch.bfloat16, 'bfloat16': torch.bfloat16, 'fp32': torch.float32, 'f32': torch.float32, 'float32': torch.float32}[d]
+
+
+class _PendingGN:
+    __slots__ = ('x', 'coef', 'silu', 'B', 'HW', 'C')
+
+    def __init__(self, x, coef, silu, B, HW, C):
+        self.x, self.coef, self.silu, self.B, self.HW, self.C = x, coef, silu, B, HW, C
+
+    def materialize(self) -> torch.Tensor:
+        return ops.groupnorm_apply(self.x, self.coef, torch.empty_like(self.x), self.B, self.HW, self.C, self.silu)
 
 
 class VQVAE(nn.Module):
@@ -164,10 +174,14 @@
         return dict(w=w3.reshape(cout, ks * ks * cin3).contiguous(), b=b, cin=cin_p, cin3=cin3, cout=cout, ks=ks)
 
     GN_FROM_CONV = True
+    GN_INTO_CONV = True
 
     def _conv(self, x, name, B, Hin, Win, *, stride=1, up=0, residual=None, out_dtype=None):
         c = self._pack()['conv'][name]
         T = c['w'].dtype
+        gn = x if isinstance(x, _PendingGN) else None
+        if gn is not None and c['ks'] == 1:
+            x = gn.materialize()
         if c['ks'] == 1:
             M = B * Hin * Win
             out = torch.empty(M, c['cout'], device=x.device, dtype=out_dtype or T)
@@ -176,16 +190,24 @@
         Hout = Hin * 2 if up else (Hin // 2 if stride == 2 else Hin)
         Wout = Win * 2 if up else (Win // 2 if stride == 2 else Win)
         M = B * Hout * Wout
-        out = torch.empty(M, c['cout'], device=x.device, dtype=out_dtype or T)
+        out = torch.empty(M, c['cout'], device=(gn.x if gn is not None else x).device, dtype=out_dtype or T)
         geo = ops.conv_gn_partials(T, stride, c['cin'], c['cout'], Hin, Win, Hout, Wout) if (self.GN_FROM_CONV and out.dtype == T) else None
-        part = torch.empty(B, geo[0], c['cout'], 3, device=x.device, dtype=torch.float32) if geo else None
+        part = torch.empty(B, geo[0], c['cout'], 3, device=out.device, dtype=torch.float32) if geo else None
+        in_gn = None
+        if gn is not None:
+            if gn.x.dtype == T and ops.conv_in_gn(T, stride, c['cin'], c['cout'], Hin, Win, Hout, Wout, out.dtype):
+                x, in_gn = gn.x, (gn.coef, gn.silu)
+            else:
+                x = gn.materialize()
         cv = dict(Hin=Hin, Win=Win, Cin=c['cin'], Hout=Hout, Wout=Wout, stride=stride, up=up)
         try:
-            ops.gemm(x, c['w'], out, M=M, N=c['cout'], K=9 * c['cin'], bias=c['b'], residual=residual, conv=cv, gn_part=part)
+            ops.gemm(x, c['w'], out, M=M, N=c['cout'], K=9 * c['cin'], bias=c['b'], residual=residual, conv=cv, gn_part=part, in_gn=in_gn)
         except CvarError as e:
-            if part is None or 'unsupported' not in str(e).lower():
+            if (part is None and in_gn is None) or 'unsupported' not in str(e).lower():
                 raise
             geo, part = None, None
+            if in_gn is not None:
+                x, in_gn = gn.materialize(), None
             ops.gemm(x, c['w'], out, M=M, N=c['cout'], K=9 * c['cin'], bias=c['b'], residual=residual, conv=cv)
         if geo:
             out._gn_part = (part, geo[0], geo[1])
@@ -193,10 +215,19 @@
 
     def _gn(self, x, name, B, HW, C, silu=True):
         w, b = self._pack()['norm'][name]
+        gp = getattr(x, '_gn_part', None)
+        from_part = gp is not None and gp[0].shape[0] == B and gp[0].shape[2] == C and gp[1] * gp[2] == HW
+        if self.GN_INTO_CONV and x.dtype == torch.bfloat16:
+            coef = torch.empty(B, C, 2, device=x.device, dtype=torch.float32)
+            if from_part:
+                ops.groupnorm_coef_partials(w, b, coef, B, HW, C, self.cfg.gn_groups, self.cfg.gn_eps, gp[0], gp[1], gp[2])
+            else:
+                ws = torch.empty(ops.groupnorm_ws_bytes(B, HW, C), device=x.device, dtype=torch.uint8)
+                ops.groupnorm_coef(x, w, b, coef, B, HW, C, self.cfg.gn_groups, self.cfg.gn_eps, ws)
+            return _PendingGN(x, coef, silu, B, HW, C)
         ws = torch.empty(ops.groupnorm_ws_bytes(B, HW, C), device=x.device, dtype=torch.uint8)
         out = torch.empty_like(x)
-        gp = getattr(x, '_gn_part', None)
-        if gp is not None and gp[0].shape[0] == B and gp[0].shape[2] == C and gp[1] * gp[2] == HW:
+        if from_part:
             return ops.groupnorm_silu_partials(x, w, b, out, B, HW, C, self.cfg.gn_groups, self.cfg.gn_eps, silu, gp[0], gp[1], gp[2], ws)
         return ops.groupnorm_silu(x, w, b, out, B, HW, C, self.cfg.gn_groups, self.cfg.gn_eps, silu, ws)
 
diff --git a/controlvar_amd/ops.py b/controlvar_amd/ops.py
--- a/controlvar_amd/ops.py
+++ b/controlvar_amd/ops.py
@@ -78,7 +78,7 @@
          conv: Optional[dict] = None, a_off: int = 0, w_off: int = 0, c_off: int = 0,
          pre_act: Optional[torch.Tensor] = None, aux: Optional[torch.Tensor] = None, gate_scale: Optional[torch.Tensor] = None,
          split: Optional[tuple] = None, split_alpha: float = 1.0, ln: Optional[tuple] = None, small_m: bool = False, split_k: bool = True,
-         gn_part: Optional[torch.Tensor] = None):
+         gn_part: Optional[torch.Tensor] = None, in_gn: Optional[tuple] = None):
     d = GemmDesc()
     d.M, d.N, d.K, d.dtype = M, N, K, dt(A)
     if W.dtype != A.dtype:
@@ -116,6 +116,8 @@
         d.ln_scale, d.ln_shift = _ptr(ada) + 4 * sc_off, _ptr(ada) + 4 * sh_off
         d.ld_ln, d.ln_rows, d.ln_eps = ld_ada, rows_per, eps
     d.gn_part = _ptr(gn_part)
+    if in_gn is not None:
+        d.in_gn, d.in_gn_silu = _ptr(in_gn[0]), int(bool(in_gn[1]))
     ws = _SPLITK_WS.get((A.device.index, _stream()))
     if ws is None:
         ws = ensure_splitk_workspace(A.device)
@@ -277,6 +279,29 @@
     return (nt.value, pp.value) if ok else None
 
 
+def conv_in_gn(dtype: torch.dtype, stride: int, Cin: int, Cout: int, Hin: int, Win: int, Hout: int, Wout: int, out_dtype: torch.dtype) -> bool:
+    if GEMM_TILE_CFG not in (0, 6) or dtype not in _DT or out_dtype not in _DT:
+        return False
+    return bool(_lib.load().cvar_conv3x3_in_gn(_DT[dtype], stride, Cin, Cout, Hin, Win, Hout, Wout, _DT[out_dtype]))
+
+
+def groupnorm_coef(x, weight, bias, coef, B, HW, Cdim, groups, eps, ws):
+    check(_lib.load().cvar_groupnorm_coef(_ptr(x), dt(x), _ptr(weight), _ptr(bias), _ptr(coef), B, HW, Cdim, groups, eps, _ptr(ws), _stream()),
+          'cvar_groupnorm_coef')
+    return coef
+
+
+def groupnorm_coef_partials(weight, bias, coef, B, HW, Cdim, groups, eps, gn_part, tiles, tile_pixels):
+    check(_lib.load().cvar_groupnorm_coef_partials(_ptr(weight), _ptr(bias), _ptr(coef), B, HW, Cdim, groups, eps, _ptr(gn_part), tiles, tile_pixels,
+                                                   _stream()), 'cvar_groupnorm_coef_partials')
+    return coef
+
+
+def groupnorm_apply(x, coef, out, B, HW, Cdim, silu):
+    check(_lib.load().cvar_groupnorm_apply(_ptr(x), dt(x), _ptr(coef), _ptr(out), B, HW, Cdim, int(silu), _stream()), 'cvar_groupnorm_apply')
+    return out
+
+
 def groupnorm_silu_partials(x, weight, bias, out, B, HW, Cdim, groups, eps, silu, gn_part, tiles, tile_pixels, ws):
     check(_lib.load().cvar_groupnorm_silu_partials(_ptr(x), dt(x), _ptr(weight), _ptr(bias), _ptr(out), B, HW, Cdim, groups, eps, int(silu),
                                                    _ptr(gn_part), tiles, tile_pixels, _ptr(ws), _stream()), 'cvar_groupnorm_silu_partials')
diff --git a/include/cvar.h b/include/cvar.h
--- a/include/cvar.h
+++ b/include/cvar.h
@@ -42,9 +42,11 @@
     void* ln_out; int ln_out_dtype;
     const float* ln_scale; const float* ln_shift; int64_t ld_ln; int ln_rows; float ln_eps;
     float* gn_part;
+    const float* in_gn; int in_gn_silu;
 } cvar_gemm_desc;
 int cvar_gemm(const cvar_gemm_desc* d, void* stream);
 int cvar_conv3x3_gn_partials(int dtype, int stride, int Cin, int Cout, int Hin, int Win, int Hout, int Wout, int* tiles_per_image, int* pixels_per_tile);
+int cvar_conv3x3_in_gn(int dtype, int stride, int Cin, int Cout, int Hin, int Win, int Hout, int Wout, int out_dtype);
 
 int cvar_gemm_tn(const void* A, int64_t lda, const void* B, int64_t ldb, float* C, int64_t ldc, int T, int Nn, int Kk,
                  float* ws, int64_t ws_bytes, float* colsum_a, void* stream);
@@ -102,6 +104,11 @@
                         int B, int HW, int C, int groups, float eps, int silu, void* ws, void* stream);
 int cvar_groupnorm_silu_partials(const void* x, int dtype, const float* weight, const float* bias, void* out, int B, int HW, int C, int groups, float eps,
                                  int silu, const float* gn_part, int tiles_per_image, int pixels_per_tile, void* ws, void* stream);
+int cvar_groupnorm_coef(const void* x, int dtype, const float* weight, const float* bias, float* coef, int B, int HW, int C, int groups, float eps,
+                        void* ws, void* stream);
+int cvar_groupnorm_coef_partials(const float* weight, const float* bias, float* coef, int B, int HW, int C, int groups, float eps,
+                                 const float* gn_part, int tiles_per_image, int pixels_per_tile, void* stream);
+int cvar_groupnorm_apply(const void* x, int dtype, const float* coef, void* out, int B, int HW, int C, int silu, void* stream);
 int cvar_split3(const float* x, int64_t ldx, void* out_bf16, int64_t M, int C, int Cpad, void* stream);
 int cvar_groupnorm_silu_split3(const float* x, const float* weight, const float* bias, void* out_bf16, int B, int HW, int C, int groups, float eps, int silu,
                                void* ws, void* stream);
```

Measured after the change: 205.8 images/s (median of 6 runs). 1.01x the previous value.
